# nka77/DAHiTra

Hardware: NVIDIA B200
Metric: image-pairs/sec (higher is better)
Workload: dtype x3 error-compensated f16 products (f16 main + scaled-remainder corrections; decoder: 3xTF32), fp32 accumulate

## Files before the change

### dahitra_b200/_lib.py

```python
from __future__ import annotations

import ctypes as C
import os
import subprocess
import threading

_HERE = os.path.dirname(os.path.abspath(__file__))
_CSRC = os.path.join(_HERE, "csrc")
LIB_PATH = os.path.join(_HERE, "libdahitra_b200.so")
SOURCES = ["conv_ffma.cu", "conv_tc.cu", "conv_tc2.cu", "conv_tc3.cu", "split.cu", "tokens.cu", "decoder.cu", "decoder_tc.cu", "stem_tc.cu", "classifier.cu", "train_decoder.cu", "train_tokens.cu", "prepare.cu", "aux.cu", "forward.cu"]
NVCC_FLAGS = ["-gencode", "arch=compute_100a,code=sm_100a", "-O3", "-lineinfo", "-std=c++17",
              "-Xcompiler", "-fPIC", "-shared"]

_lock = threading.Lock()
_lib = None


def _sources():
    return [os.path.join(_CSRC, s) for s in SOURCES if os.path.exists(os.path.join(_CSRC, s))]


STAMP_PATH = LIB_PATH + ".stamp"


def _deps():
    deps = _sources() + [os.path.join(_HERE, "..", "include", "dahitra_b200.h")]
    deps += [os.path.join(_CSRC, f) for f in sorted(os.listdir(_CSRC)) if f.endswith(".cuh")]
    return [d for d in deps if os.path.exists(d)]


def _source_hash() -> str:
    import hashlib
    h = hashlib.sha256(" ".join(NVCC_FLAGS + [os.environ.get("DAHITRA_DEBUG_BUILD", "0")]).encode())
    for d in _deps():
        h.update(os.path.basename(d).encode() + b"\0")
        with open(d, "rb") as f:
            h.update(f.read())
    return h.hexdigest()


def needs_build() -> bool:
    if not os.path.exists(LIB_PATH):
        return True
    if os.path.exists(STAMP_PATH):
        with open(STAMP_PATH) as f:
            return f.read().strip() != _source_hash()
    t = os.path.getmtime(LIB_PATH)
    if any(os.path.getmtime(d) > t for d in _deps()):
        return True
    _write_stamp()
    return False


def _write_stamp():
    try:
        with open(STAMP_PATH + ".tmp", "w") as f:
            f.write(_source_hash() + "\n")
        os.replace(STAMP_PATH + ".tmp", STAMP_PATH)
    except OSError:
        pass


def build(force: bool = False, verbose: bool = False) -> str:
    if not force and not needs_build():
        return LIB_PATH
    import tempfile
    from concurrent.futures import ThreadPoolExecutor
    nvcc = os.environ.get("NVCC", "nvcc")
    cflags = [f for f in NVCC_FLAGS if f != "-shared"]
    if os.environ.get("DAHITRA_DEBUG_BUILD") == "1":
        cflags.append("-DDH_MBAR_TIMEOUT")
    with tempfile.TemporaryDirectory(prefix="_build_", dir=_HERE) as tmp:
        def compile_one(src):
            obj = os.path.join(tmp, os.path.basename(src) + ".o")
            cmd = [nvcc] + cflags + ["-c", src, "-o", obj]
            if verbose:
                print(" ".join(cmd), flush=True)
            r = subprocess.run(cmd, capture_output=True, text=True)
            if r.returncode != 0:
                raise RuntimeError("nvcc failed on %s:\n%s%s" % (src, r.stdout, r.stderr))
            return obj
        with ThreadPoolExecutor(max_workers=min(8, os.cpu_count() or 1)) as ex:
            objs = list(ex.map(compile_one, _sources()))
        cmd = [nvcc] + NVCC_FLAGS + objs + ["-o", LIB_PATH + ".tmp"]
        if verbose:
            print(" ".join(cmd), flush=True)
        r = subprocess.run(cmd, capture_output=True, text=True)
        if r.returncode != 0:
            raise RuntimeError("nvcc link failed:\n" + r.stdout + r.stderr)
    os.replace(LIB_PATH + ".tmp", LIB_PATH)
    _write_stamp()
    return LIB_PATH


EXAMPLE_SRC = os.path.join(_HERE, "..", "examples", "dahitra_infer.c")
EXAMPLE_BIN = os.path.join(_HERE, "..", "examples", "bin", "dahitra_infer")


def build_example(force: bool = False, verbose: bool = False) -> str:
    src, out = os.path.abspath(EXAMPLE_SRC), os.path.abspath(EXAMPLE_BIN)
    deps = [src, LIB_PATH, os.path.join(_HERE, "..", "include", "dahitra_b200.h")]
    if not force and os.path.exists(out) and all(os.path.getmtime(d) <= os.path.getmtime(out) for d in deps):
        return out
    cuda = os.environ.get("CUDA_HOME", "/usr/local/cuda")
    os.makedirs(os.path.dirname(out), exist_ok=True)
    cmd = [os.environ.get("CC", "gcc"), "-std=c99", "-O2", "-Wall", "-Wextra", "-Werror", "-I", os.path.join(_HERE, "..", "include"),
           "-I", os.path.join(cuda, "include"), src, "-L", _HERE, "-ldahitra_b200", "-L", os.path.join(cuda, "lib64"),
           "-l:libcudart_static.a", "-ldl", "-lpthread", "-lrt", "-Wl,-rpath,$ORIGIN/../../dahitra_b200", "-o", out + ".tmp"]
    if verbose:
        print(" ".join(cmd), flush=True)
    r = subprocess.run(cmd, capture_output=True, text=True)
    if r.returncode != 0:
        raise RuntimeError("building examples/dahitra_infer.c failed:\n" + r.stdout + r.stderr)
    os.replace(out + ".tmp", out)
    return out


_P, _I, _LL, _SZ = C.c_void_p, C.c_int, C.c_longlong, C.c_size_t
SIGNATURES = {
    "dahitra_version": (_I, []),
    "dahitra_error_string": (C.c_char_p, [_I]),
    "dahitra_weight_slot_name": (C.c_char_p, [_I]),
    "dahitra_workspace_bytes": (_SZ, [_I, _I, _I, _I, _I, _I]),
    "dahitra_prepare_weights": (_LL, [_P, _I, _I, _I, _P, _LL, _P]),
    "dahitra_forward": (_I, [_P, _I, _P, _P, _LL, _P, _P, _P, _SZ, _I, _I, _I, _I, _I, _I, _P]),
    "dahitra_forward_profiled": (_I, [_P, _I, _P, _P, _LL, _P, _P, _P, _SZ, _I, _I, _I, _I, _I, _I, _P,
                                      _I, _P, _P, _P, _P]),
    "dahitra_conv2d": (_I, [_P, _P, _I, _I, _I, _I, _I, _I, _I, _I, _I, _I, _I, _P, _P, _P, _P, _I, _P, _I, _P]),
    "dahitra_conv2d_up2_tc": (_I, [_P, _I, _I, _I, _P, _P, _I, _P, _I, _P]),
    "dahitra_stem": (_I, [_P, _LL, _I, _I, _I, _P, _P, _P, _P]),
    "dahitra_stem_tc": (_I, [_P, _LL, _I, _I, _I, _P, _P, _P, _I, _P]),
    "dahitra_maxpool3x3s2": (_I, [_P, _I, _I, _I, _I, _P, _P]),
    "dahitra_squeeze_tokens": (_I, [_P, _I, _I, _I, _P, _P, _P, _P, _P]),
    "dahitra_token_encoder": (_I, [_P, _I, _I, _P, _I, _I, _P, _P]),
    "dahitra_decoder_tables": (_I, [_P, _I, _I, _I, _P, _I, _I, _P, _P]),
    "dahitra_pixel_decoder": (_I, [_P, _P, _P, _P, _I, _I, _I, _I, _I, _P, _I, _P, _P]),
    "dahitra_decoder_tables_tc": (_I, [_P, _I, _I, _I, _P, _I, _I, _P, _P]),
    "dahitra_pixel_decoder_tc": (_I, [_P, _P, _P, _P, _I, _I, _I, _I, _I, _P, _I, _I, _P, _P]),
    "dahitra_confusion_matrix": (_I, [_P, _P, _LL, _I, _P, _P]),
    "dahitra_prepare_input_u8": (_I, [_P, _I, _I, _I, _I, _I, _P, _P]),
    "dahitra_classifier": (_I, [_P, _I, _I, _I, _I, _P, _P, _P, _P, _P]),
    "dahitra_split_pack": (_I, [_P, _LL, _P, _P]),
    "dahitra_split_unpack": (_I, [_P, _LL, _P, _P]),
    "dahitra_maxpool3x3s2_split": (_I, [_P, _I, _I, _I, _I, _P, _P]),
    "dahitra_pixel_decoder_train_blocks": (_I, [_I]),
    "dahitra_pixel_decoder_train_fwd": (_I, [_P, _P, _P, _P, _I, _I, _I, _I, _I, _P]),
    "dahitra_pixel_decoder_train_bwd": (_I, [_P, _P, _P, _P, _P, _I, _I, _I, _I, _I, _P]),
    "dahitra_tokenizer_train_chunks": (_I, [_I]),
    "dahitra_tokenizer_train_fwd": (_I, [_P, _P, _P, _P, _P, _I, _I, _I, _P]),
    "dahitra_tokenizer_train_bwd": (_I, [_P, _P, _P, _P, _P, _P, _P, _I, _I, _I, _P]),
    "dahitra_pixel_decoder_train_fwd_ex": (_I, [_P, _P, _P, _P, _I, _I, _I, _I, _I, _I, _P]),
    "dahitra_pixel_decoder_train_bwd_ex": (_I, [_P, _P, _P, _P, _P, _I, _I, _I, _I, _I, _I, _P]),
    "dahitra_tokenizer_train_fwd_ex": (_I, [_P, _P, _P, _P, _P, _I, _I, _I, _I, _P]),
    "dahitra_tokenizer_train_bwd_ex": (_I, [_P, _P, _P, _P, _P, _P, _P, _I, _I, _I, _I, _P]),
    "dahitra_conv2d_split": (_I, [_P, _P, _I, _I, _LL, _LL, _I, _I, _I, _I, _I, _I, _P, _P, _P, _I, _I, _P, _I, _I, _P, _P, _P]),
    "dahitra_maxpool3x3s2_h16": (_I, [_P, _I, _I, _I, _I, _P, _P]),
    "dahitra_classifier_h16": (_I, [_P, _I, _I, _I, _I, _P, _P, _P, _P, _P]),
}


class DhTensor(C.Structure):
    _fields_ = [("name", C.c_char_p), ("data", C.c_void_p), ("dtype", C.c_int), ("ndim", C.c_int), ("shape", C.c_longlong * 4)]


def load():
    global _lib
    with _lock:
        if _lib is None:
            if not os.path.exists(LIB_PATH):
                raise RuntimeError(
                    f"dahitra_b200: {LIB_PATH} is missing — run `python -c 'import __graft_entry__ as g; g.build()'` "
                    "(nvcc, sm_100a). There is no fallback path.")
            lib = C.CDLL(LIB_PATH)
            for name, (res, args) in SIGNATURES.items():
                fn = getattr(lib, name)
                fn.restype, fn.argtypes = res, args
            _lib = lib
        return _lib


def check(rc: int, what: str = "dahitra"):
    if rc != 0:
        msg = load().dahitra_error_string(rc)
        raise RuntimeError(f"{what} failed with code {rc}: {msg.decode() if msg else '?'}")
```

### dahitra_b200/csrc/common.cuh

```cuda
#pragma once
#include <cuda_runtime.h>
#include <stdint.h>
#include <stddef.h>
#include "../../include/dahitra_b200.h"

#ifndef __CUDA_ARCH_LIST__
#endif

#define DH_CHECK_LAUNCH()                                   \
  do {                                                      \
    cudaError_t e__ = cudaGetLastError();                   \
    if (e__ != cudaSuccess) return (int)e__;                \
  } while (0)

#define DH_REQUIRE(cond, code) \
  do {                         \
    if (!(cond)) return (code);\
  } while (0)

static inline bool dh_aligned16(const void* p) { return (reinterpret_cast<uintptr_t>(p) & 15u) == 0; }
static inline int dh_cdiv(int a, int b) { return (a + b - 1) / b; }

__device__ __forceinline__ float4 ldg4(const float* p) { return __ldg(reinterpret_cast<const float4*>(p)); }
__device__ __forceinline__ void st4(float* p, float4 v) { *reinterpret_cast<float4*>(p) = v; }

__device__ __forceinline__ float warp_sum(float v) {
#pragma unroll
  for (int o = 16; o > 0; o >>= 1) v += __shfl_xor_sync(0xffffffffu, v, o);
  return v;
}
__device__ __forceinline__ float warp_max(float v) {
#pragma unroll
  for (int o = 16; o > 0; o >>= 1) v = fmaxf(v, __shfl_xor_sync(0xffffffffu, v, o));
  return v;
}

__device__ __forceinline__ float gelu_erf(float x) { return 0.5f * x * (1.0f + erff(x * 0.70710678118654752440f)); }

struct ConvArgs {
  const float* in0; const float* in1; int C0, C1;
  int N, inH, inW, up;
  int KH, KW, stride, pad, Cout;
  const float* w;
  const float* wt;
  const float* bias; const float* res; int relu;
  float* out;
  int ps = 0;
  int flat = 0;
};
struct Conv3Args {
  const void* in0; const void* in1; int C0, C1;
  int N, inH, inW;
  long long in0_plane = 0, in1_plane = 0;
  long long res_plane = 0, out_plane = 0;
  int K, stride, Cout;
  const void* wt16;
  long long wt_plane_bytes;
  const float* bias; const void* res; int res_split;
  int relu;
  void* out; int out_split;
  int ps = 0;
  int tok = 0;
  const float* wtok = nullptr; float* partials = nullptr;
  int force_stream = 0;
  int cg = 0;
  int h16 = 0;
};
bool dh_conv_tc3_eligible(const Conv3Args& a);
int dh_launch_conv_tc3(const Conv3Args& a, cudaStream_t s);
int dh_conv_tc3_tok_chunks(int H, int W);
int dh_launch_split_pack(const float* in, size_t n, void* out, cudaStream_t s);
int dh_launch_split_unpack(const void* in, size_t n, float* out, cudaStream_t s);
int dh_launch_maxpool_split(const void* in, int N, int H, int W, int C, void* out, cudaStream_t s);
int dh_launch_maxpool_h16(const void* in, int N, int H, int W, int C, void* out, cudaStream_t s);
int dh_pdl_attr(cudaLaunchAttribute* at);
void dh_set_pdl(int on);
template <typename... KArgs, typename... Args>
static inline int dh_launch(void (*kern)(KArgs...), dim3 grid, dim3 block, size_t smem, cudaStream_t s, Args... args) {
  cudaLaunchConfig_t cfg = {};
  cfg.gridDim = grid; cfg.blockDim = block; cfg.dynamicSmemBytes = smem; cfg.stream = s;
  cudaLaunchAttribute at[1];
  cfg.attrs = at; cfg.numAttrs = dh_pdl_attr(at);
  const cudaError_t e = cudaLaunchKernelEx(&cfg, kern, KArgs(args)...);
  if (e != cudaSuccess) return (int)e;
  DH_CHECK_LAUNCH();
  return 0;
}
#ifdef __CUDACC__
__device__ __forceinline__ void dh_pdl_wait() { asm volatile("griddepcontrol.wait;" ::: "memory"); }
__device__ __forceinline__ void dh_pdl_launch_dependents() { asm volatile("griddepcontrol.launch_dependents;" ::: "memory"); }
#endif
int dh_launch_conv_ffma(const ConvArgs& a, cudaStream_t s);
bool dh_conv_tc_eligible(const ConvArgs& a);
int dh_launch_conv_tc(const ConvArgs& a, cudaStream_t s);
bool dh_conv_tc2_eligible(const ConvArgs& a);
int dh_launch_conv_tc2(const ConvArgs& a, int xm, int cg, cudaStream_t s);
int dh_launch_stem(const float* x, long long xbs, int N, int H, int W, const float* w, const float* b, float* out, cudaStream_t s);
int dh_launch_stem_tc(const float* x, long long xbs, int N, int H, int W, const float* wtc, const float* b, float* out, int x3,
                      cudaStream_t s, long long split_plane_pitch = 0, const float* x_second = nullptr);
int dh_launch_maxpool(const float* in, int N, int H, int W, int C, float* out, cudaStream_t s);
int dh_launch_classifier(const float* in, int N, int H, int W, int nc, const float* w, const float* b,
                         float* logits, unsigned char* amax, cudaStream_t s);
int dh_launch_classifier_tma(const float* in, int N, int H, int W, int nc, const float* w, const float* b,
                             float* logits, unsigned char* amax, cudaStream_t s);
int dh_launch_classifier_h16(const void* in, int N, int H, int W, int nc, const float* w, const float* b,
                             float* logits, unsigned char* amax, cudaStream_t s);
int dh_launch_squeeze_tokens(const float* feat, int N, int npix, int Cin, const float* wsq, const float* wtok,
                             float* xs, float* partials, cudaStream_t s);
int dh_launch_token_encoder(const float* partials, int B, int nchunk, const float* enc, int heads, int add_pos,
                            float* mem, cudaStream_t s);
int dh_launch_decoder_tables(const float* mem, int B, int first_call, int ncalls, const float* dec, int heads, int depth,
                             float* tables, cudaStream_t s);
int dh_launch_decoder_tables_tc(const float* mem, int B, int first_call, int ncalls, const float* dec, int heads, int depth,
                                float* tables, cudaStream_t s);
int dh_launch_pixel_decoder_tc(const float* x, const float* pos, const float* tables, const float* pack, int nimg, int h,
                               int w, int heads, int depth, const float* skip, int skip_up, int x3, float* out,
                               cudaStream_t s);
int dh_launch_pixel_decoder(const float* x, const float* pos, const float* tables, const float* dec,
                            int nimg, int h, int w, int heads, int depth, const float* skip, int skip_up, float* out,
                            cudaStream_t s);
```

### dahitra_b200/csrc/conv_tc3.cu

```cuda
#include "tc_common.cuh"
#include <cstdlib>
#include <mutex>
#include <unordered_map>

using namespace dhtc;

namespace {

constexpr int T3_TH = 16, T3_TW = 8;
constexpr int T3_HW = T3_TW + 2, T3_HH = T3_TH + 2;
constexpr uint32_t T3_PLANE = 11776;
constexpr uint32_t T3_HALO = 2 * T3_PLANE;
constexpr int T3_MAX_HB = 4;
enum { EPI_F32 = 0, EPI_SPLIT = 1, EPI_TOK = 2 };

struct T3Args {
  const float* bias;
  const void* res; void* out;
  const float* wtok; float* partials;
  long long res_plane, out_plane;
  int OH, OW, Cout, relu, tilesX, tilesY, cchunks0, cchunks, Cin, ps, N, ncout_tiles, ntiles;
  int res_split, out_split, tiles_per_img;
  int hb;
  uint32_t halo_plane_bytes;
};

template <int NT, bool RES, int CG = 1, bool P1 = false> struct T3Cfg {
  static constexpr int TPS = NT == 128 ? 1 : 3;
  static constexpr int STAGES = RES ? 1 : (NT == 128 ? 6 : (NT == 64 ? 4 : 8)) * CG;
  static constexpr uint32_t HALO = P1 ? T3_PLANE : T3_HALO;
  static constexpr uint32_t B_TAP = (P1 ? 1u : 2u) * NT * 64u / CG;
  static constexpr uint32_t B_STAGE = B_TAP * TPS;
  static constexpr uint32_t RING_BYTES = RES ? 0u : STAGES * B_STAGE;
  static constexpr int THREADS = 352;
  static constexpr uint32_t IDESC_WIDE = umma_idesc_f16(128, 2 * NT);
  static constexpr uint32_t IDESC_NARROW = umma_idesc_f16(128 * CG, NT);
  static constexpr int ACC_COLS = P1 ? NT : 2 * NT;
  static constexpr uint32_t TMEM_COLS = 2 * ACC_COLS < 32 ? 32 : 2 * ACC_COLS;
};

template <int KS, int SD> struct Tap3 {
  static constexpr int NPH = (KS == 3 && SD == 2) ? 4 : 1;
  static constexpr int NTAPS = KS * KS;
  __host__ __device__ static constexpr int tap(int i) {
    return (KS == 3 && SD == 2) ? (int)((0x862071534ULL >> (4 * i)) & 0xF) : i;
  }
  __host__ __device__ static constexpr int first(int ph) {
    return (KS == 3 && SD == 2) ? (int)((0x95310u >> (4 * ph)) & 0xF) : (ph == 0 ? 0 : NTAPS);
  }
  __host__ __device__ static constexpr int shift_px(int t, int halo_w) {
    return KS == 1 ? 0 : (SD == 2 ? ((t / 3 != 0) ? halo_w : 0) + ((t % 3 != 0) ? 1 : 0) : (t / 3) * halo_w + t % 3);
  }
};

struct Tile3 { int n, oy0, ox0, ct; };
__device__ __forceinline__ Tile3 tile3(int tile, const T3Args& e, int CG = 1, int rank = 0) {
  Tile3 t;
  t.ct = tile % e.ncout_tiles; tile /= e.ncout_tiles;
  if (CG == 2) tile = 2 * tile + rank;
  const int tx = tile % e.tilesX; tile /= e.tilesX;
  const int ty = tile % e.tilesY;
  t.n = tile / e.tilesY; t.oy0 = ty * T3_TH; t.ox0 = tx * T3_TW;
  return t;
}

__device__ __forceinline__ void tma_load_3d_2sm(uint32_t dst, const CUtensorMap* tm, uint32_t cluster_bar, int c0, int c1, int c2) {
  asm volatile(
      "cp.async.bulk.tensor.3d.cta_group::2.shared::cluster.global.tile.mbarrier::complete_tx::bytes [%0], [%1, {%3, %4, %5}], [%2];"
      ::"r"(dst), "l"(tm), "r"(cluster_bar), "r"(c0), "r"(c1), "r"(c2) : "memory");
}
__device__ __forceinline__ void tma_load_3d(uint32_t dst, const CUtensorMap* tm, uint32_t bar, int c0, int c1, int c2) {
  asm volatile(
      "cp.async.bulk.tensor.3d.shared::cluster.global.tile.mbarrier::complete_tx::bytes [%0], [%1, {%3, %4, %5}], [%2];"
      ::"r"(dst), "l"(tm), "r"(bar), "r"(c0), "r"(c1), "r"(c2) : "memory");
}
__device__ __forceinline__ void split8(const float4& a, const float4& b, uint4& hi, uint4& lo) {
  hi.x = pack_f16x2_sat(a.x, a.y); hi.y = pack_f16x2_sat(a.z, a.w); hi.z = pack_f16x2_sat(b.x, b.y); hi.w = pack_f16x2_sat(b.z, b.w);
  lo.x = pack_f16x2_sat((a.x - f16_lo(hi.x)) * 2048.f, (a.y - f16_hi(hi.x)) * 2048.f);
  lo.y = pack_f16x2_sat((a.z - f16_lo(hi.y)) * 2048.f, (a.w - f16_hi(hi.y)) * 2048.f);
  lo.z = pack_f16x2_sat((b.x - f16_lo(hi.z)) * 2048.f, (b.y - f16_hi(hi.z)) * 2048.f);
  lo.w = pack_f16x2_sat((b.z - f16_lo(hi.w)) * 2048.f, (b.w - f16_hi(hi.w)) * 2048.f);
}
__device__ __forceinline__ void join8(const uint4& hi, const uint4& lo, float4& a, float4& b) {
  constexpr float S = 1.0f / 2048.0f;
  a = make_float4(fmaf(f16_lo(lo.x), S, f16_lo(hi.x)), fmaf(f16_hi(lo.x), S, f16_hi(hi.x)),
                  fmaf(f16_lo(lo.y), S, f16_lo(hi.y)), fmaf(f16_hi(lo.y), S, f16_hi(hi.y)));
  b = make_float4(fmaf(f16_lo(lo.z), S, f16_lo(hi.z)), fmaf(f16_hi(lo.z), S, f16_hi(hi.z)),
                  fmaf(f16_lo(lo.w), S, f16_lo(hi.w)), fmaf(f16_hi(lo.w), S, f16_hi(hi.w)));
}
__device__ __forceinline__ void half8(const uint4& h, float4& a, float4& b) {
  a = make_float4(f16_lo(h.x), f16_hi(h.x), f16_lo(h.y), f16_hi(h.y));
  b = make_float4(f16_lo(h.z), f16_hi(h.z), f16_lo(h.w), f16_hi(h.w));
}
__device__ __forceinline__ uint4 ldg16(const void* p) { return __ldg(reinterpret_cast<const uint4*>(p)); }
__device__ __forceinline__ float4 as_f4(const uint4& u) { return make_float4(__uint_as_float(u.x), __uint_as_float(u.y), __uint_as_float(u.z), __uint_as_float(u.w)); }

template <int NT, int KS, int SD, int EPI, bool RES, int CG, bool P1>
__global__ void __launch_bounds__(T3Cfg<NT, RES, CG, P1>::THREADS, 1)
conv_tc3_kernel(const __grid_constant__ CUtensorMap tmA0h, const __grid_constant__ CUtensorMap tmA0l,
                const __grid_constant__ CUtensorMap tmA1h, const __grid_constant__ CUtensorMap tmA1l,
                const __grid_constant__ CUtensorMap tmB, const T3Args e) {
  using Cfg = T3Cfg<NT, RES, CG, P1>;
  constexpr int STAGES = Cfg::STAGES;
  extern __shared__ uint8_t t3_raw[];
  __shared__ __align__(8) uint64_t halo_full[T3_MAX_HB], halo_empty[T3_MAX_HB], b_full[STAGES], b_empty[STAGES], acc_full[2], acc_empty[2];
  __shared__ uint32_t tmem_slot;

  const int warp = threadIdx.x >> 5, lane = threadIdx.x & 31;
  const uint32_t base = (smem_u32(t3_raw) + 1023u) & ~1023u;
  uint8_t* base_ptr = t3_raw + (base - smem_u32(t3_raw));
  const int HB = e.hb;
  const uint32_t b_ring = base + (uint32_t)HB * Cfg::HALO;
  const int rank = CG == 2 ? (int)cluster_ctarank() : 0;
  const int w0 = CG == 2 ? (int)(blockIdx.x >> 1) : (int)blockIdx.x;
  const int wstep = CG == 2 ? (int)(gridDim.x >> 1) : (int)gridDim.x;
  constexpr int pad = (KS == 3) ? 1 : 0;
  using Sched = Tap3<KS, SD>;
  constexpr int NPH = Sched::NPH;
  constexpr int NTAPS = KS * KS;
  constexpr int TPS = (SD == 1 && NTAPS % Cfg::TPS == 0) ? Cfg::TPS : 1;
  constexpr int HALO_W = (KS == 3) ? T3_HW : T3_TW;
  const uint32_t w_bytes = RES ? (uint32_t)(e.ncout_tiles * e.cchunks * NTAPS) * Cfg::B_TAP : Cfg::RING_BYTES;
  const uint32_t epi_off = (uint32_t)HB * Cfg::HALO + w_bytes;

  if (threadIdx.x == 0) {
    for (int i = 0; i < T3_MAX_HB; ++i) { mbar_init(smem_u32(&halo_full[i]), 1); mbar_init(smem_u32(&halo_empty[i]), 1); }
    for (int i = 0; i < 2; ++i) { mbar_init(smem_u32(&acc_full[i]), 1); mbar_init(smem_u32(&acc_empty[i]), 128 * CG); }
    for (int s = 0; s < STAGES; ++s) { mbar_init(smem_u32(&b_full[s]), 1); mbar_init(smem_u32(&b_empty[s]), 1); }
    mbar_fence_init();
    asm volatile("prefetch.tensormap [%0];" ::"l"(&tmA0h) : "memory");
    asm volatile("prefetch.tensormap [%0];" ::"l"(&tmA0l) : "memory");
    asm volatile("prefetch.tensormap [%0];" ::"l"(&tmB) : "memory");
  }
  if (warp == 1) {
    if (CG == 2) tmem_alloc_2sm(smem_u32(&tmem_slot), Cfg::TMEM_COLS);
    else         tmem_alloc(smem_u32(&tmem_slot), Cfg::TMEM_COLS);
  }
  if (EPI == EPI_TOK && threadIdx.x >= 64 && threadIdx.x < 96)
    reinterpret_cast<float4*>(base_ptr + epi_off + 8 * 4096)[threadIdx.x - 64] = __ldg(reinterpret_cast<const float4*>(e.wtok) + (threadIdx.x - 64));
  tc_fence_before();
  __syncthreads();
  if (CG == 2) cluster_sync_all();
  tc_fence_after();
  const uint32_t tmem_base = tmem_slot;
  if (RES && warp == 6 && lane == 0) {
    const uint32_t bar = smem_u32(&b_full[0]);
    if (rank == 0) mbar_expect_tx(bar, (uint32_t)CG * w_bytes);
    const uint32_t lbar = (CG == 2 && rank == 1) ? mapa_u32(bar, 0) : bar;
    uint32_t dst = b_ring;
    for (int ct = 0; ct < e.ncout_tiles; ++ct)
      for (int cc = 0; cc < e.cchunks; ++cc)
#pragma unroll
        for (int i = 0; i < NTAPS; ++i, dst += Cfg::B_TAP) {
          if (CG == 2) tma_load_3d_2sm(dst, &tmB, lbar, Sched::tap(i) * e.Cin + cc * 32, ct * NT + rank * (NT / 2), 0);
          else         tma_load_3d(dst, &tmB, bar, Sched::tap(i) * e.Cin + cc * 32, ct * NT, 0);
        }
  }
  pdl_wait();
  pdl_launch_dependents();

  if (warp == 0) {
    if (lane == 0) {
      int hb = 0;
      uint32_t ephase = 1;
      for (int tile = w0; tile < e.ntiles; tile += wstep) {
        const Tile3 t = tile3(tile, e, CG, rank);
        for (int cc = 0; cc < e.cchunks; ++cc) {
#pragma unroll
          for (int ph = 0; ph < NPH; ++ph) {
            mbar_wait(smem_u32(&halo_empty[hb]), ephase);
            const uint32_t bar = smem_u32(&halo_full[hb]);
            if (rank == 0) mbar_expect_tx(bar, (uint32_t)CG * (P1 ? 1u : 2u) * e.halo_plane_bytes);
            const uint32_t dst = base + (uint32_t)hb * Cfg::HALO;
            const int cx = SD == 1 ? t.ox0 - pad : 2 * (t.ox0 - pad) + (ph & 1);
            const int cy = SD == 1 ? t.oy0 - pad : 2 * (t.oy0 - pad) + (ph >> 1);
            const bool first = cc < e.cchunks0;
            const int c0 = (first ? cc : cc - e.cchunks0) * 32;
            if (CG == 2 && rank == 1) {
              const uint32_t lbar = mapa_u32(bar, 0);
              tma_load_4d_2sm(dst, first ? &tmA0h : &tmA1h, lbar, c0, cx, cy, t.n);
              tma_load_4d_2sm(dst + T3_PLANE, first ? &tmA0l : &tmA1l, lbar, c0, cx, cy, t.n);
            } else {
              tma_load_4d(dst, first ? &tmA0h : &tmA1h, bar, c0, cx, cy, t.n);
              if (!P1) tma_load_4d(dst + T3_PLANE, first ? &tmA0l : &tmA1l, bar, c0, cx, cy, t.n);
            }
            if (++hb == HB) { hb = 0; ephase ^= 1u; }
          }
        }
      }
    }
  } else if (warp == 6) {
    if (!RES && lane == 0) {
      int step = 0;
      for (int tile = w0; tile < e.ntiles; tile += wstep) {
        const Tile3 t = tile3(tile, e, CG, rank);
        for (int cc = 0; cc < e.cchunks; ++cc) {
#pragma unroll
          for (int i0 = 0; i0 < NTAPS; i0 += TPS, ++step) {
            const int st = step % STAGES, round = step / STAGES;
            mbar_wait(smem_u32(&b_empty[st]), (uint32_t)((round & 1) ^ 1));
            const uint32_t bar = smem_u32(&b_full[st]);
            if (rank == 0) mbar_expect_tx(bar, (uint32_t)(CG * TPS) * Cfg::B_TAP);
            const uint32_t lbar = (CG == 2 && rank == 1) ? mapa_u32(bar, 0) : bar;
#pragma unroll
            for (int tt = 0; tt < TPS; ++tt) {
              const uint32_t dst = b_ring + (uint32_t)st * Cfg::B_STAGE + (uint32_t)tt * Cfg::B_TAP;
              const int kcol = Sched::tap(i0 + tt) * e.Cin + cc * 32;
              if (CG == 2) tma_load_3d_2sm(dst, &tmB, lbar, kcol, t.ct * NT + rank * (NT / 2), 0);
              else         tma_load_3d(dst, &tmB, bar, kcol, t.ct * NT, 0);
            }
          }
        }
      }
    }
  } else if (warp == 1) {
    if (lane == 0 && rank == 0) {
      constexpr uint32_t SBO = (uint32_t)HALO_W * 64u;
      int hb = 0, st = 0, it = 0;
      uint32_t hphase = 0, bphase = 0;
      if (RES) { mbar_wait(smem_u32(&b_full[0]), 0); tc_fence_after(); }
      for (int tile = w0; tile < e.ntiles; tile += wstep, ++it) {
        const int ab = it & 1;
        if (CG == 2) mbar_wait_cluster(smem_u32(&acc_empty[ab]), (uint32_t)(((it >> 1) & 1) ^ 1));
        else         mbar_wait(smem_u32(&acc_empty[ab]), (uint32_t)(((it >> 1) & 1) ^ 1));
        tc_fence_after();
        const uint32_t d_main = tmem_base + (uint32_t)ab * Cfg::ACC_COLS, d_corr = d_main + NT;
        const uint32_t w_tile = RES ? b_ring + (uint32_t)((tile % e.ncout_tiles) * e.cchunks * NTAPS) * Cfg::B_TAP : 0u;
        for (int cc = 0; cc < e.cchunks; ++cc) {
#pragma unroll
          for (int ph = 0; ph < NPH; ++ph) {
            mbar_wait(smem_u32(&halo_full[hb]), hphase);
            tc_fence_after();
            const uint32_t h_hi = base + (uint32_t)hb * Cfg::HALO, h_lo = h_hi + T3_PLANE;
#pragma unroll
            for (int i0 = Sched::first(ph); i0 < Sched::first(ph + 1); i0 += TPS) {
              uint32_t b_stage;
              if (RES) {
                b_stage = w_tile + (uint32_t)(cc * NTAPS + i0) * Cfg::B_TAP;
              } else {
                mbar_wait(smem_u32(&b_full[st]), bphase);
                tc_fence_after();
                b_stage = b_ring + (uint32_t)st * Cfg::B_STAGE;
              }
#pragma unroll
              for (int tt = 0; tt < TPS; ++tt) {
                const int i = i0 + tt;
                const uint32_t px = (uint32_t)Sched::shift_px(Sched::tap(i), HALO_W) * 64u;
                const uint64_t a_h = umma_desc_sw64(h_hi + px, SBO), a_l = umma_desc_sw64(h_lo + px, SBO);
                const uint64_t b_w = umma_desc_sw64(b_stage + (uint32_t)tt * Cfg::B_TAP, 512u);
                if (CG == 2) {
                  const uint64_t b_l = umma_desc_sw64(b_stage + (uint32_t)tt * Cfg::B_TAP + (NT / 2) * 64u, 512u);
#pragma unroll
                  for (int k = 0; k < 2; ++k) umma_bf16_2sm(d_main, a_h + (uint64_t)(2 * k), b_w + (uint64_t)(2 * k), Cfg::IDESC_NARROW, (cc | i | k) ? 1u : 0u);
#pragma unroll
                  for (int k = 0; k < 2; ++k) umma_bf16_2sm(d_corr, a_h + (uint64_t)(2 * k), b_l + (uint64_t)(2 * k), Cfg::IDESC_NARROW, (cc | i | k) ? 1u : 0u);
#pragma unroll
                  for (int k = 0; k < 2; ++k) umma_bf16_2sm(d_corr, a_l + (uint64_t)(2 * k), b_w + (uint64_t)(2 * k), Cfg::IDESC_NARROW, 1u);
                } else if (P1) {
#pragma unroll
                  for (int k = 0; k < 2; ++k) umma_bf16(d_main, a_h + (uint64_t)(2 * k), b_w + (uint64_t)(2 * k), Cfg::IDESC_NARROW, (cc | i | k) ? 1u : 0u);
                } else {
#pragma unroll
                  for (int k = 0; k < 2; ++k) umma_bf16(d_main, a_h + (uint64_t)(2 * k), b_w + (uint64_t)(2 * k), Cfg::IDESC_WIDE, (cc | i | k) ? 1u : 0u);
#pragma unroll
                  for (int k = 0; k < 2; ++k) umma_bf16(d_corr, a_l + (uint64_t)(2 * k), b_w + (uint64_t)(2 * k), Cfg::IDESC_NARROW, 1u);
                }
              }
              if (!RES) {
                if (CG == 2) umma_commit_2sm(smem_u32(&b_empty[st])); else umma_commit(smem_u32(&b_empty[st]));
                if (++st == STAGES) { st = 0; bphase ^= 1u; }
              }
            }
            if (CG == 2) umma_commit_2sm(smem_u32(&halo_empty[hb])); else umma_commit(smem_u32(&halo_empty[hb]));
            if (++hb == HB) { hb = 0; hphase ^= 1u; }
          }
        }
        if (CG == 2) umma_commit_2sm(smem_u32(&acc_full[ab])); else umma_commit(smem_u32(&acc_full[ab]));
      }
    }
  } else {
    const int q = warp & 3, grp = warp >= 7 ? 1 : 0;
    float* stage = reinterpret_cast<float*>(base_ptr + epi_off + (size_t)(grp * 4 + q) * 4096);
    const float* wtok_s = reinterpret_cast<const float*>(base_ptr + epi_off + 8 * 4096);
    float* tokred = reinterpret_cast<float*>(base_ptr + epi_off + 8 * 4096 + 512 + grp * 2176);
    const int c4 = lane & 3, r4 = lane >> 2;
    constexpr int NSLAB = NT / 32;
    const char* resb = reinterpret_cast<const char*>(e.res);
    int it = 0;
    for (int tile = w0; tile < e.ntiles; tile += wstep, ++it) {
      if ((it & 1) != grp) continue;
      const Tile3 t = tile3(tile, e, CG, rank);
      const int n0 = t.ct * NT;
      size_t rowoff[4];
      bool ok[4];
#pragma unroll
      for (int g = 0; g < 4; ++g) {
        const int mm = q * 32 + g * 8 + r4;
        const int oy = t.oy0 + mm / T3_TW, ox = t.ox0 + mm % T3_TW;
        ok[g] = (oy < e.OH) && (ox < e.OW) && (t.n < e.N);
        rowoff[g] = e.ps ? ((size_t)(t.n * 2 * e.OH + 2 * oy) * (2 * e.OW) + 2 * ox) * 32 + c4 * 8
                         : ((size_t)(t.n * e.OH + oy) * e.OW + ox) * e.Cout + n0 + c4 * 8;
      }
      uint4 ra[4], rb[4];
      auto load_res = [&](int j) {
#pragma unroll
        for (int g = 0; g < 4; ++g) {
          ra[g] = make_uint4(0u, 0u, 0u, 0u); rb[g] = ra[g];
          if (ok[g]) {
            const size_t o = rowoff[g] + (size_t)j * 32;
            if (e.res_split) { ra[g] = ldg16(resb + o * 2); if (!P1) rb[g] = ldg16(resb + (o + (size_t)e.res_plane) * 2); }
            else             { ra[g] = ldg16(resb + o * 4); rb[g] = ldg16(resb + o * 4 + 16); }
          }
        }
      };
      if (e.res) load_res(0);
      const int ab = it & 1;
      mbar_wait(smem_u32(&acc_full[ab]), (uint32_t)((it >> 1) & 1));
      tc_fence_after();
#pragma unroll 1
      for (int j = 0; j < NSLAB; ++j) {
        float4 bia0 = make_float4(0.f, 0.f, 0.f, 0.f), bia1 = bia0;
        if (e.bias) { bia0 = ldg4(e.bias + n0 + j * 32 + c4 * 8); bia1 = ldg4(e.bias + n0 + j * 32 + c4 * 8 + 4); }
        uint32_t v[32], u[32];
        tmem_ld32(tmem_base + ((uint32_t)(q * 32) << 16) + (uint32_t)(ab * Cfg::ACC_COLS + j * 32), v);
        if (!P1) tmem_ld32(tmem_base + ((uint32_t)(q * 32) << 16) + (uint32_t)(ab * Cfg::ACC_COLS + NT + j * 32), u);
        if (j == NSLAB - 1) {
          tc_fence_before();
          if (CG == 2) mbar_arrive_cluster(mapa_u32(smem_u32(&acc_empty[ab]), 0));
          else         mbar_arrive_local(smem_u32(&acc_empty[ab]));
        }
        float tl[4] = {0.f, 0.f, 0.f, 0.f};
#pragma unroll
        for (int c = 0; c < 32; ++c) {
          float x = P1 ? __uint_as_float(v[c]) : fmaf(__uint_as_float(u[c]), 1.0f / 2048.0f, __uint_as_float(v[c]));
          if (EPI == EPI_TOK) {
            x = fmaxf(x, 0.f);
            const float4 wt = *reinterpret_cast<const float4*>(wtok_s + c * 4);
            tl[0] = fmaf(x, wt.x, tl[0]); tl[1] = fmaf(x, wt.y, tl[1]); tl[2] = fmaf(x, wt.z, tl[2]); tl[3] = fmaf(x, wt.w, tl[3]);
          }
          v[c] = __float_as_uint(x);
        }
#pragma unroll
        for (int k4 = 0; k4 < 8; ++k4)
          *reinterpret_cast<float4*>(stage + lane * 32 + ((k4 ^ (lane & 7)) << 2)) =
              make_float4(__uint_as_float(v[k4 * 4]), __uint_as_float(v[k4 * 4 + 1]), __uint_as_float(v[k4 * 4 + 2]), __uint_as_float(v[k4 * 4 + 3]));
        __syncwarp();
#pragma unroll
        for (int g = 0; g < 4; ++g) {
          const int r = g * 8 + r4;
          float4 o0 = *reinterpret_cast<const float4*>(stage + r * 32 + (((2 * c4) ^ (r & 7)) << 2));
          float4 o1 = *reinterpret_cast<const float4*>(stage + r * 32 + (((2 * c4 + 1) ^ (r & 7)) << 2));
          o0.x += bia0.x; o0.y += bia0.y; o0.z += bia0.z; o0.w += bia0.w;
          o1.x += bia1.x; o1.y += bia1.y; o1.z += bia1.z; o1.w += bia1.w;
          if (e.res) {
            float4 x0, x1;
            if (e.res_split) { if (P1) half8(ra[g], x0, x1); else join8(ra[g], rb[g], x0, x1); }
            else { x0 = as_f4(ra[g]); x1 = as_f4(rb[g]); }
            o0.x += x0.x; o0.y += x0.y; o0.z += x0.z; o0.w += x0.w;
            o1.x += x1.x; o1.y += x1.y; o1.z += x1.z; o1.w += x1.w;
          }
          if (e.relu) {
            o0.x = fmaxf(o0.x, 0.f); o0.y = fmaxf(o0.y, 0.f); o0.z = fmaxf(o0.z, 0.f); o0.w = fmaxf(o0.w, 0.f);
            o1.x = fmaxf(o1.x, 0.f); o1.y = fmaxf(o1.y, 0.f); o1.z = fmaxf(o1.z, 0.f); o1.w = fmaxf(o1.w, 0.f);
          }
          if (ok[g]) {
            if (P1 && e.out_split) {
              uint16_t* o16 = reinterpret_cast<uint16_t*>(e.out);
              const size_t off = rowoff[g] + (e.ps ? ((size_t)(j >> 1) * (2 * e.OW) + (j & 1)) * 32 : (size_t)j * 32);
              *reinterpret_cast<uint4*>(o16 + off) = make_uint4(pack_f16x2_sat(o0.x, o0.y), pack_f16x2_sat(o0.z, o0.w),
                                                                pack_f16x2_sat(o1.x, o1.y), pack_f16x2_sat(o1.z, o1.w));
            } else if (!P1 && (EPI == EPI_SPLIT || (EPI == EPI_TOK && e.out_split))) {
              uint4 h, l;
              split8(o0, o1, h, l);
              uint16_t* o16 = reinterpret_cast<uint16_t*>(e.out);
              const size_t off = rowoff[g] + (size_t)j * 32;
              *reinterpret_cast<uint4*>(o16 + off) = h;
              *reinterpret_cast<uint4*>(o16 + off + (size_t)e.out_plane) = l;
            } else {
              float* ob = reinterpret_cast<float*>(e.out);
              float* op = e.ps ? ob + rowoff[g] + ((size_t)(j >> 1) * (2 * e.OW) + (j & 1)) * 32 : ob + rowoff[g] + (size_t)j * 32;
              st4(op, o0); st4(op + 4, o1);
            }
          }
        }
        if (e.res && j + 1 < NSLAB) load_res(j + 1);
        if (EPI == EPI_TOK) {
          const int mm = q * 32 + lane;
          const bool valid = (t.oy0 + mm / T3_TW < e.OH) && (t.ox0 + mm % T3_TW < e.OW) && (t.n < e.N);
          float ew[4];
#pragma unroll
          for (int l = 0; l < 4; ++l) {
            const float a = valid ? tl[l] : -INFINITY;
            const float mx = warp_max(a);
            ew[l] = valid ? expf(a - mx) : 0.f;
            const float sw = warp_sum(ew[l]);
            if (lane == 0) { tokred[(q * 4 + l) * 34] = mx; tokred[(q * 4 + l) * 34 + 1] = sw; }
          }
          float ts[4] = {0.f, 0.f, 0.f, 0.f};
#pragma unroll 8
          for (int r = 0; r < 32; ++r) {
            const float xv = stage[r * 32 + ((((lane >> 2) ^ (r & 7)) << 2) | (lane & 3))];
#pragma unroll
            for (int l = 0; l < 4; ++l) ts[l] = fmaf(__shfl_sync(0xffffffffu, ew[l], r), xv, ts[l]);
          }
#pragma unroll
          for (int l = 0; l < 4; ++l) tokred[(q * 4 + l) * 34 + 2 + lane] = ts[l];
          asm volatile("bar.sync %0, 128;" ::"r"(1 + grp) : "memory");
          {
            const int l = q;
            float m4[4], M = -INFINITY;
#pragma unroll
            for (int w4 = 0; w4 < 4; ++w4) { m4[w4] = tokred[(w4 * 4 + l) * 34]; M = fmaxf(M, m4[w4]); }
            float S = 0.f, T = 0.f;
#pragma unroll
            for (int w4 = 0; w4 < 4; ++w4) {
              const float sc = (m4[w4] == -INFINITY) ? 0.f : expf(m4[w4] - M);
              S = fmaf(tokred[(w4 * 4 + l) * 34 + 1], sc, S);
              T = fmaf(tokred[(w4 * 4 + l) * 34 + 2 + lane], sc, T);
            }
            const int mtile = CG == 2 ? 2 * (tile / e.ncout_tiles) + rank : tile / e.ncout_tiles;
            float* pp = e.partials + (((size_t)t.n * e.tiles_per_img + mtile % e.tiles_per_img) * 4 + l) * 34;
            if (t.n < e.N) {
              if (lane == 0) { pp[0] = M; pp[1] = S; }
              pp[2 + lane] = T;
            }
          }
          asm volatile("bar.sync %0, 128;" ::"r"(1 + grp) : "memory");
        }
        __syncwarp();
      }
    }
  }
  tc_fence_before();
  __syncthreads();
  if (CG == 2) cluster_sync_all();
  if (warp == 1) {
    tc_fence_after();
    if (CG == 2) tmem_dealloc_2sm(tmem_base, Cfg::TMEM_COLS);
    else         tmem_dealloc(tmem_base, Cfg::TMEM_COLS);
  }
}

typedef CUresult (*EncodeTiledFn3)(CUtensorMap*, CUtensorMapDataType, cuuint32_t, void*, const cuuint64_t*, const cuuint64_t*,
                                   const cuuint32_t*, const cuuint32_t*, CUtensorMapInterleave, CUtensorMapSwizzle,
                                   CUtensorMapL2promotion, CUtensorMapFloatOOBfill);
EncodeTiledFn3 get_encode3() {
  static EncodeTiledFn3 fn = nullptr;
  static std::once_flag once;
  std::call_once(once, [] {
    void* p = nullptr;
    cudaDriverEntryPointQueryResult q;
    if (cudaGetDriverEntryPoint("cuTensorMapEncodeTiled", &p, cudaEnableDefault, &q) == cudaSuccess && q == cudaDriverEntryPointSuccess)
      fn = (EncodeTiledFn3)p;
  });
  return fn;
}
struct Key3 {
  const void* ptr; long long d[5];
  bool operator==(const Key3& o) const { return ptr == o.ptr && d[0] == o.d[0] && d[1] == o.d[1] && d[2] == o.d[2] && d[3] == o.d[3] && d[4] == o.d[4]; }
};
struct Key3Hash {
  size_t operator()(const Key3& k) const {
    size_t h = (size_t)k.ptr;
    for (long long v : k.d) h = h * 1000003u ^ (size_t)v;
    return h;
  }
};
std::mutex g_mu3;
std::unordered_map<Key3, CUtensorMap, Key3Hash> g_maps3;

int act_map(CUtensorMap* out, const void* ptr, int C, int W, int H, int N, int bw, int bh, int es) {
  Key3 key{ptr, {C, W, H, ((long long)N << 8) | es, ((long long)bw << 16) | bh}};
  {
    std::lock_guard<std::mutex> lk(g_mu3);
    auto it = g_maps3.find(key);
    if (it != g_maps3.end()) { *out = it->second; return 0; }
  }
  EncodeTiledFn3 enc = get_encode3();
  if (!enc) return DH_E_VARIANT;
  cuuint64_t dims[4] = {(cuuint64_t)C, (cuuint64_t)W, (cuuint64_t)H, (cuuint64_t)N};
  cuuint64_t strides[3] = {(cuuint64_t)C * 2, (cuuint64_t)C * W * 2, (cuuint64_t)C * W * H * 2};
  cuuint32_t box[4] = {32, (cuuint32_t)(bw * es), (cuuint32_t)(bh * es), 1};
  cuuint32_t estr[4] = {1, (cuuint32_t)es, (cuuint32_t)es, 1};
  CUtensorMap m;
  const CUresult r = enc(&m, CU_TENSOR_MAP_DATA_TYPE_FLOAT16, 4, const_cast<void*>(ptr), dims, strides, box, estr,
                         CU_TENSOR_MAP_INTERLEAVE_NONE, CU_TENSOR_MAP_SWIZZLE_64B, CU_TENSOR_MAP_L2_PROMOTION_L2_256B,
                         CU_TENSOR_MAP_FLOAT_OOB_FILL_NONE);
  if (r != CUDA_SUCCESS) return DH_E_SHAPE;
  {
    std::lock_guard<std::mutex> lk(g_mu3);
    if (g_maps3.size() > 4096) g_maps3.clear();
    g_maps3[key] = m;
  }
  *out = m;
  return 0;
}
int filt_map(CUtensorMap* out, const void* ptr, int K, int Cout, long long plane_bytes, int NT, int planes) {
  Key3 key{ptr, {K, Cout, plane_bytes, NT, -1 - planes}};
  {
    std::lock_guard<std::mutex> lk(g_mu3);
    auto it = g_maps3.find(key);
    if (it != g_maps3.end()) { *out = it->second; return 0; }
  }
  EncodeTiledFn3 enc = get_encode3();
  if (!enc) return DH_E_VARIANT;
  cuuint64_t dims[3] = {(cuuint64_t)K, (cuuint64_t)Cout, (cuuint64_t)planes};
  cuuint64_t strides[2] = {(cuuint64_t)K * 2, (cuuint64_t)plane_bytes};
  cuuint32_t box[3] = {32, (cuuint32_t)NT, (cuuint32_t)planes};
  cuuint32_t estr[3] = {1, 1, 1};
  CUtensorMap m;
  const CUresult r = enc(&m, CU_TENSOR_MAP_DATA_TYPE_FLOAT16, 3, const_cast<void*>(ptr), dims, strides, box, estr,
                         CU_TENSOR_MAP_INTERLEAVE_NONE, CU_TENSOR_MAP_SWIZZLE_64B, CU_TENSOR_MAP_L2_PROMOTION_L2_256B,
                         CU_TENSOR_MAP_FLOAT_OOB_FILL_NONE);
  if (r != CUDA_SUCCESS) return DH_E_SHAPE;
  {
    std::lock_guard<std::mutex> lk(g_mu3);
    g_maps3[key] = m;
  }
  *out = m;
  return 0;
}

constexpr uint32_t T3_SMEM_MAX = 232448 - 1024;

template <int NT, int KS, int SD, int EPI, bool RES, int CG, bool P1>
int launch3k(const CUtensorMap* A, const CUtensorMap& Bm, const T3Args& e, uint32_t smem, dim3 grid, cudaStream_t s) {
  using Cfg = T3Cfg<NT, RES, CG, P1>;
  auto kern = conv_tc3_kernel<NT, KS, SD, EPI, RES, CG, P1>;
  cudaError_t err = cudaFuncSetAttribute(kern, cudaFuncAttributeMaxDynamicSharedMemorySize, (int)T3_SMEM_MAX);
  if (err != cudaSuccess) return (int)err;
  cudaLaunchConfig_t cfg = {};
  cfg.gridDim = grid; cfg.blockDim = dim3(Cfg::THREADS, 1, 1); cfg.dynamicSmemBytes = smem; cfg.stream = s;
  cudaLaunchAttribute at[2];
  int na = dh_pdl_attr(at);
  if (CG == 2) {
    at[na].id = cudaLaunchAttributeClusterDimension;
    at[na].val.clusterDim.x = 2; at[na].val.clusterDim.y = 1; at[na].val.clusterDim.z = 1;
    ++na;
  }
  cfg.attrs = at; cfg.numAttrs = na;
  err = cudaLaunchKernelEx(&cfg, kern, A[0], A[1], A[2], A[3], Bm, e);
  if (err != cudaSuccess) return (int)err;
  DH_CHECK_LAUNCH();
  return 0;
}
template <int NT, bool RES, int CG, bool P1>
int launch3(const CUtensorMap* A, const CUtensorMap& Bm, const T3Args& e, int ks, int stride, int epi, uint32_t smem, dim3 grid, cudaStream_t s) {
  if (epi == EPI_TOK) {
    if constexpr (NT == 32 && CG == 1) return launch3k<32, 1, 1, EPI_TOK, RES, 1, P1>(A, Bm, e, smem, grid, s);
    return DH_E_SHAPE;
  }
  if constexpr (P1) {
    if (stride == 2) return ks == 3 ? launch3k<NT, 3, 2, EPI_SPLIT, RES, CG, true>(A, Bm, e, smem, grid, s) : launch3k<NT, 1, 2, EPI_SPLIT, RES, CG, true>(A, Bm, e, smem, grid, s);
    return ks == 3 ? launch3k<NT, 3, 1, EPI_SPLIT, RES, CG, true>(A, Bm, e, smem, grid, s) : launch3k<NT, 1, 1, EPI_SPLIT, RES, CG, true>(A, Bm, e, smem, grid, s);
  } else {
    if (stride == 2) {
      if (epi == EPI_SPLIT) return ks == 3 ? launch3k<NT, 3, 2, EPI_SPLIT, RES, CG, false>(A, Bm, e, smem, grid, s) : launch3k<NT, 1, 2, EPI_SPLIT, RES, CG, false>(A, Bm, e, smem, grid, s);
      return ks == 3 ? launch3k<NT, 3, 2, EPI_F32, RES, CG, false>(A, Bm, e, smem, grid, s) : launch3k<NT, 1, 2, EPI_F32, RES, CG, false>(A, Bm, e, smem, grid, s);
    }
    if (epi == EPI_SPLIT) return ks == 3 ? launch3k<NT, 3, 1, EPI_SPLIT, RES, CG, false>(A, Bm, e, smem, grid, s) : launch3k<NT, 1, 1, EPI_SPLIT, RES, CG, false>(A, Bm, e, smem, grid, s);
    return ks == 3 ? launch3k<NT, 3, 1, EPI_F32, RES, CG, false>(A, Bm, e, smem, grid, s) : launch3k<NT, 1, 1, EPI_F32, RES, CG, false>(A, Bm, e, smem, grid, s);
  }
}
template <bool RES, int CG, bool P1>
int launch3n(int NT, const CUtensorMap* A, const CUtensorMap& Bm, const T3Args& e, int ks, int stride, int epi, uint32_t smem, dim3 grid, cudaStream_t s) {
  switch (NT) {
    case 128: return launch3<128, RES, CG, P1>(A, Bm, e, ks, stride, epi, smem, grid, s);
    case 64: return launch3<64, RES, CG, P1>(A, Bm, e, ks, stride, epi, smem, grid, s);
    default: return launch3<32, RES, CG, P1>(A, Bm, e, ks, stride, epi, smem, grid, s);
  }
}
template <bool RES>
int launch3c(int cg, bool p1, int NT, const CUtensorMap* A, const CUtensorMap& Bm, const T3Args& e, int ks, int stride, int epi, uint32_t smem,
             dim3 grid, cudaStream_t s) {
  if (p1) return launch3n<RES, 1, true>(NT, A, Bm, e, ks, stride, epi, smem, grid, s);
  return cg == 2 ? launch3n<RES, 2, false>(NT, A, Bm, e, ks, stride, epi, smem, grid, s)
                 : launch3n<RES, 1, false>(NT, A, Bm, e, ks, stride, epi, smem, grid, s);
}
}

bool dh_conv_tc3_eligible(const Conv3Args& a) {
  const bool base = a.in0 && a.wt16 && a.out && (a.stride == 1 || (a.stride == 2 && a.inH % 2 == 0 && a.inW % 2 == 0 && !a.ps)) &&
                    (a.K == 1 || a.K == 3) && a.C0 > 0 && a.C0 % 32 == 0 && a.C1 % 32 == 0 && (a.C1 == 0 || a.in1) &&
                    (a.Cout == 32 || a.Cout == 64 || a.Cout == 128 || a.Cout == 256) && a.inH >= 1 && a.inW >= 1 && a.N >= 1;
  if (!base) return false;
  if (a.ps) return a.Cout == 128 && a.res == nullptr && (!a.out_split || a.h16) && a.K == 3;
  if (a.tok) return a.Cout == 32 && a.K == 1 && a.stride == 1 && a.wtok && a.partials && !a.res && !a.bias;
  return true;
}

int dh_conv_tc3_tok_chunks(int H, int W) { return dh_cdiv(H, T3_TH) * dh_cdiv(W, T3_TW); }

int dh_launch_conv_tc3(const Conv3Args& a, cudaStream_t s) {
  DH_REQUIRE(dh_conv_tc3_eligible(a), DH_E_SHAPE);
  DH_REQUIRE(dh_aligned16(a.in0) && dh_aligned16(a.in1) && dh_aligned16(a.wt16) && dh_aligned16(a.out) &&
             dh_aligned16(a.bias) && dh_aligned16(a.res) && dh_aligned16(a.wtok), DH_E_ALIGN);
  const int Cin = a.C0 + a.C1, K = a.K * a.K * Cin;
  int sms_ = 148, dev_ = 0;
  cudaGetDevice(&dev_);
  cudaDeviceGetAttribute(&sms_, cudaDevAttrMultiProcessorCount, dev_);
  int NT = a.Cout >= 128 ? 128 : a.Cout;
  if (NT == 128 && !a.ps) {
    const int mt = dh_cdiv(a.inW / a.stride, T3_TW) * dh_cdiv(a.inH / a.stride, T3_TH) * a.N;
    if (mt * (a.Cout / 128) < sms_) NT = 64;
  }
  const int hw = (a.K == 3) ? T3_HW : T3_TW, hh = (a.K == 3) ? T3_HH : T3_TH;
  CUtensorMap A[4], Bm;
  const size_t plane0 = a.in0_plane ? (size_t)a.in0_plane : (size_t)a.N * a.inH * a.inW * a.C0;
  const size_t plane1 = a.in1_plane ? (size_t)a.in1_plane : (size_t)a.N * a.inH * a.inW * a.C1;
  int rc = act_map(&A[0], a.in0, a.C0, a.inW, a.inH, a.N, hw, hh, a.stride);
  if (rc) return rc;
  A[1] = A[0];
  if (!a.h16) rc = act_map(&A[1], reinterpret_cast<const uint16_t*>(a.in0) + plane0, a.C0, a.inW, a.inH, a.N, hw, hh, a.stride);
  if (rc) return rc;
  if (a.C1) {
    rc = act_map(&A[2], a.in1, a.C1, a.inW, a.inH, a.N, hw, hh, a.stride);
    A[3] = A[2];
    if (!rc && !a.h16) rc = act_map(&A[3], reinterpret_cast<const uint16_t*>(a.in1) + plane1, a.C1, a.inW, a.inH, a.N, hw, hh, a.stride);
    if (rc) return rc;
  } else { A[2] = A[0]; A[3] = A[1]; }
  static const int env_cg = [] { const char* v = getenv("DAHITRA_TC3_CG"); return v ? atoi(v) : 0; }();
  static const bool env_stream = [] { const char* v = getenv("DAHITRA_TC3_STREAM"); return v && v[0] == '1'; }();
  const int mtiles = dh_cdiv(a.inW / a.stride, T3_TW) * dh_cdiv(a.inH / a.stride, T3_TH) * a.N;
  int cg = a.tok ? 1 : (a.cg ? a.cg : (env_cg == 2 ? 2 : (env_cg == 1 && (NT == 128 || (a.Cout == 32 && K >= 1152)) ? 2 : 1)));
  DH_REQUIRE(!(a.h16 && cg == 2), DH_E_VARIANT);
  if (mtiles < 2) cg = 1;
  rc = filt_map(&Bm, a.wt16, K, a.Cout, a.wt_plane_bytes, NT / cg, a.h16 ? 1 : 2);
  if (rc) return rc;
  T3Args e;
  e.bias = a.bias; e.res = a.res; e.out = a.out; e.wtok = a.wtok; e.partials = a.partials;
  e.OH = a.inH / a.stride; e.OW = a.inW / a.stride; e.Cout = a.Cout; e.relu = a.relu;
  e.tilesX = dh_cdiv(e.OW, T3_TW); e.tilesY = dh_cdiv(e.OH, T3_TH);
  e.cchunks0 = a.C0 / 32; e.cchunks = Cin / 32; e.Cin = Cin; e.ps = a.ps; e.N = a.N;
  e.ncout_tiles = a.Cout / NT;
  e.tiles_per_img = e.tilesX * e.tilesY;
  e.ntiles = (cg == 2 ? (mtiles + 1) / 2 : mtiles) * e.ncout_tiles;
  e.res_split = a.res_split; e.out_split = a.out_split;
  e.res_plane = a.res_plane ? a.res_plane : (long long)a.N * e.OH * e.OW * a.Cout;
  e.out_plane = a.out_plane ? a.out_plane : (long long)a.N * e.OH * e.OW * a.Cout;
  e.halo_plane_bytes = (uint32_t)(hw * hh * 64);
  const int epi = a.tok ? EPI_TOK : ((a.out_split || a.h16) ? EPI_SPLIT : EPI_F32);
  int dev = 0, sms = 148;
  cudaGetDevice(&dev);
  cudaDeviceGetAttribute(&sms, cudaDevAttrMultiProcessorCount, dev);
  const int slots = sms / cg;
  const int nwork = e.ntiles < slots ? e.ntiles : slots;
  dim3 grid((unsigned)(nwork * cg), 1, 1);
  const uint32_t w_bytes = (uint32_t)K * (uint32_t)a.Cout * (a.h16 ? 2u : 4u) / (uint32_t)cg;
  const uint32_t halo = a.h16 ? T3_PLANE : T3_HALO;
  const uint32_t fixed = 8 * 4096 + 1024 + (a.tok ? 512 + 2 * 2176 : 0);
  const bool res_ok = w_bytes + 2 * halo + fixed <= T3_SMEM_MAX && !a.force_stream && !env_stream && e.ntiles >= 2 * nwork;
  if (res_ok) {
    int hb = (int)((T3_SMEM_MAX - fixed - w_bytes) / halo);
    e.hb = hb > T3_MAX_HB ? T3_MAX_HB : hb;
    const uint32_t smem = (uint32_t)e.hb * halo + w_bytes + fixed;
    return launch3c<true>(cg, a.h16, NT, A, Bm, e, a.K, a.stride, epi, smem, grid, s);
  }
  e.hb = T3_MAX_HB;
  const uint32_t ring = a.h16 ? (NT == 128 ? T3Cfg<128, false, 1, true>::RING_BYTES : (NT == 64 ? T3Cfg<64, false, 1, true>::RING_BYTES : T3Cfg<32, false, 1, true>::RING_BYTES))
                              : (NT == 128 ? T3Cfg<128, false>::RING_BYTES : (NT == 64 ? T3Cfg<64, false>::RING_BYTES : T3Cfg<32, false>::RING_BYTES));
  const uint32_t smem = T3_MAX_HB * halo + ring + fixed;
  return launch3c<false>(cg, a.h16, NT, A, Bm, e, a.K, a.stride, epi, smem, grid, s);
}
```

### dahitra_b200/csrc/forward.cu

```cuda
#include "common.cuh"
#include <string.h>

namespace {

struct Level {
  int cin, heads, depth, h, w;
  size_t xs, xd, dx, out, part, mem, tab;
  int nchunk, nchunk3;
};

struct Plan {
  int B, H, W, nc, variant;
  size_t f2, p2, t4a, t4b, f4, t8a, t8b, t8c, f8, p8, t16a, t16b, t16c, f16;
  Level lv[3];
  size_t c4, c3, y20, o2, c2;
  size_t total_floats;
};

struct Bump {
  size_t off = 0;
  size_t take(size_t nfloats) {
    const size_t o = off;
    off += (nfloats + 63) & ~(size_t)63;
    return o;
  }
};

bool make_plan(Plan& p, int variant, int B, int H, int W, int nc, int flags) {
  if (B < 1 || H < 32 || W < 32 || (H % 32) || (W % 32) || nc < 1 || nc > 8) return false;
  if (variant != DH_VARIANT_LEVIR && variant != DH_VARIANT_XBD) return false;
  p.B = B; p.H = H; p.W = W; p.nc = nc; p.variant = variant;
  const size_t N2 = 2 * (size_t)B;
  const size_t s2 = (size_t)(H / 2) * (W / 2), s4 = s2 / 4, s8 = s4 / 4, s16 = s8 / 4;
  Bump b;
  p.f2 = b.take(N2 * s2 * 64);
  p.p2 = b.take(N2 * s4 * 64);
  p.t4a = b.take(N2 * s4 * 64); p.t4b = b.take(N2 * s4 * 64); p.f4 = b.take(N2 * s4 * 64);
  p.t8a = b.take(N2 * s8 * 128); p.t8b = b.take(N2 * s8 * 128); p.t8c = b.take(N2 * s8 * 128); p.f8 = b.take(N2 * s8 * 128);
  p.p8 = b.take(N2 * s16 * 128);
  p.t16a = b.take(N2 * s16 * 256); p.t16b = b.take(N2 * s16 * 256); p.t16c = b.take(N2 * s16 * 256); p.f16 = b.take(N2 * s16 * 256);
  const int cins[3] = {256, 128, 64}, heads[3] = {4, 4, 8}, depths[3] = {4, 4, 8}, div[3] = {16, 8, 4};
  for (int i = 0; i < 3; ++i) {
    Level& L = p.lv[i];
    L.cin = cins[i]; L.heads = heads[i]; L.depth = depths[i]; L.h = H / div[i]; L.w = W / div[i];
    const size_t n = (size_t)L.h * L.w;
    L.nchunk = (int)((n + 255) / 256);
    L.nchunk3 = dh_conv_tc3_tok_chunks(L.h, L.w);
    L.xs = b.take(N2 * n * 32);
    L.xd = b.take(N2 * n * 32);
    L.dx = b.take((size_t)B * n * 32);
    L.out = b.take((size_t)B * n * 32);
    L.part = b.take(N2 * (size_t)(L.nchunk3 > L.nchunk ? L.nchunk3 : L.nchunk) * 4 * 34);
    L.mem = b.take((size_t)B * 3 * 128);
    L.tab = b.take((size_t)3 * B * L.depth * (DH_TAB_FLOATS(L.heads) > DH_TABTC_FLOATS ? DH_TAB_FLOATS(L.heads) : DH_TABTC_FLOATS));
  }
  p.c4 = b.take((size_t)B * s4 * 32);
  const size_t n_c3 = (size_t)B * s2 * 32, n_y20 = (size_t)B * s2 * 128, n_c2 = (size_t)B * H * W * 32;
  const bool early_head = (flags & DH_FLAG_EARLY_HEAD) != 0;
  p.c3 = (p.t8c - p.t8a >= n_c3) ? p.t8a : b.take(n_c3);
  p.o2 = (p.p8 - p.t8c >= n_c3) ? p.t8c : b.take(n_c3);
  p.y20 = (!early_head && p.t8a - p.p2 >= n_y20) ? p.p2 : b.take(n_y20);
  p.c2 = (p.p2 - p.f2 >= n_c2) ? p.f2 : b.take(n_c2);
  p.total_floats = b.off;
  return true;
}

const char* kSlotNames[DH_W_COUNT] = {
  "DH_W_STEM_W", "DH_W_STEM_B",
  "DH_W_L1_0_C1_W", "DH_W_L1_0_C1_B", "DH_W_L1_0_C2_W", "DH_W_L1_0_C2_B",
  "DH_W_L1_1_C1_W", "DH_W_L1_1_C1_B", "DH_W_L1_1_C2_W", "DH_W_L1_1_C2_B",
  "DH_W_L2_0_C1_W", "DH_W_L2_0_C1_B", "DH_W_L2_0_C2_W", "DH_W_L2_0_C2_B", "DH_W_L2_0_DS_W", "DH_W_L2_0_DS_B",
  "DH_W_L2_1_C1_W", "DH_W_L2_1_C1_B", "DH_W_L2_1_C2_W", "DH_W_L2_1_C2_B",
  "DH_W_L3_0_C1_W", "DH_W_L3_0_C1_B", "DH_W_L3_0_C2_W", "DH_W_L3_0_C2_B", "DH_W_L3_0_DS_W", "DH_W_L3_0_DS_B",
  "DH_W_L3_1_C1_W", "DH_W_L3_1_C1_B", "DH_W_L3_1_C2_W", "DH_W_L3_1_C2_B",
  "DH_W_LV5_SQ", "DH_W_LV5_TOK", "DH_W_LV5_ENC", "DH_W_LV5_DEC", "DH_W_LV5_POS", "DH_W_LV5_DECODE",
  "DH_W_LV4_SQ", "DH_W_LV4_TOK", "DH_W_LV4_ENC", "DH_W_LV4_DEC", "DH_W_LV4_POS", "DH_W_LV4_DECODE",
  "DH_W_LV3_SQ", "DH_W_LV3_TOK", "DH_W_LV3_ENC", "DH_W_LV3_DEC", "DH_W_LV3_POS", "DH_W_LV3_DECODE",
  "DH_W_CL4_W", "DH_W_CL4_B", "DH_W_CL3_W", "DH_W_CL3_B", "DH_W_CL2_W", "DH_W_CL2_B",
  "DH_W_CL20A_W", "DH_W_CL20A_B", "DH_W_CL20B_W", "DH_W_CL20B_B", "DH_W_CLS_W", "DH_W_CLS_B",
  "DH_W_L1_0_C1_WT", "DH_W_L1_0_C2_WT", "DH_W_L1_1_C1_WT", "DH_W_L1_1_C2_WT",
  "DH_W_L2_0_C2_WT", "DH_W_L2_1_C1_WT", "DH_W_L2_1_C2_WT",
  "DH_W_L3_0_C1_WT", "DH_W_L3_0_C2_WT", "DH_W_L3_0_DS_WT", "DH_W_L3_1_C1_WT", "DH_W_L3_1_C2_WT",
  "DH_W_LV5_DECODE_WT", "DH_W_LV4_DECODE_WT", "DH_W_LV3_DECODE_WT", "DH_W_CL20A_WT", "DH_W_CL20B_WT",
  "DH_W_L2_0_C1_WT", "DH_W_L2_0_DS_WT",
  "DH_W_CL4_PSWT", "DH_W_CL4_PSB", "DH_W_CL3_PSWT", "DH_W_CL3_PSB", "DH_W_CL2_PSWT", "DH_W_CL2_PSB",
  "DH_W_LV5_DECTC", "DH_W_LV4_DECTC", "DH_W_LV3_DECTC", "DH_W_STEM_WTC",
  "DH_W_LV5_SQ_WT", "DH_W_LV4_SQ_WT", "DH_W_LV3_SQ_WT"};

int wt_slot_of(int wslot) {
  switch (wslot) {
    case DH_W_L1_0_C1_W: return DH_W_L1_0_C1_WT; case DH_W_L1_0_C2_W: return DH_W_L1_0_C2_WT;
    case DH_W_L1_1_C1_W: return DH_W_L1_1_C1_WT; case DH_W_L1_1_C2_W: return DH_W_L1_1_C2_WT;
    case DH_W_L2_0_C2_W: return DH_W_L2_0_C2_WT; case DH_W_L2_1_C1_W: return DH_W_L2_1_C1_WT;
    case DH_W_L2_1_C2_W: return DH_W_L2_1_C2_WT;
    case DH_W_L3_0_C1_W: return DH_W_L3_0_C1_WT; case DH_W_L3_0_C2_W: return DH_W_L3_0_C2_WT;
    case DH_W_L3_0_DS_W: return DH_W_L3_0_DS_WT; case DH_W_L3_1_C1_W: return DH_W_L3_1_C1_WT;
    case DH_W_L3_1_C2_W: return DH_W_L3_1_C2_WT;
    case DH_W_LV5_DECODE: return DH_W_LV5_DECODE_WT; case DH_W_LV4_DECODE: return DH_W_LV4_DECODE_WT;
    case DH_W_LV3_DECODE: return DH_W_LV3_DECODE_WT;
    case DH_W_CL20A_W: return DH_W_CL20A_WT; case DH_W_CL20B_W: return DH_W_CL20B_WT;
    case DH_W_L2_0_C1_W: return DH_W_L2_0_C1_WT; case DH_W_L2_0_DS_W: return DH_W_L2_0_DS_WT;
    default: return -1;
  }
}

}

extern "C" int dahitra_version(void) { return DAHITRA_ABI_VERSION; }

extern "C" const char* dahitra_error_string(int code) {
  switch (code) {
    case 0: return "ok";
    case DH_E_NULL: return "dahitra: required pointer is NULL";
    case DH_E_SHAPE: return "dahitra: unsupported shape";
    case DH_E_ALIGN: return "dahitra: pointer not 16-byte aligned";
    case DH_E_WORKSPACE: return "dahitra: workspace too small";
    case DH_E_VARIANT: return "dahitra: unknown variant or flags";
    case DH_E_WEIGHTS: return "dahitra: malformed weight table";
    default: return code > 0 ? cudaGetErrorString((cudaError_t)code) : "dahitra: unknown error";
  }
}

extern "C" const char* dahitra_weight_slot_name(int slot) {
  return (slot >= 0 && slot < DH_W_COUNT) ? kSlotNames[slot] : nullptr;
}

extern "C" size_t dahitra_workspace_bytes(int variant, int B, int H, int W, int output_nc, int flags) {
  Plan p;
  if (!make_plan(p, variant, B, H, W, output_nc, flags)) return 0;
  return p.total_floats * sizeof(float);
}

static int conv_dispatch(const ConvArgs& a, int flags, cudaStream_t s) {
  if (flags & DH_FLAG_CONV_TC) {
    const bool stride_ok = a.stride == 1 || (flags & DH_FLAG_TC_STRIDE2);
    if (stride_ok && !(flags & DH_FLAG_CONV_TC_V1) && dh_conv_tc2_eligible(a))
      return dh_launch_conv_tc2(a, (flags & DH_FLAG_TC_BF16) ? 3 : (flags & DH_FLAG_TC_3XTF32) ? ((flags & DH_FLAG_TC_MAIN_F16) ? ((flags & DH_FLAG_TC_FOLD) ? 6 : 4) : (flags & DH_FLAG_TC_X3_BF16) ? 2 : 1)
                                                            : ((flags & DH_FLAG_TC_MAIN_F16) ? 5 : 0),
                                (flags & DH_FLAG_CONV_TC_2CTA) ? 2 : 1, s);
    if (stride_ok && dh_conv_tc_eligible(a)) return dh_launch_conv_tc(a, s);
  }
  return dh_launch_conv_ffma(a, s);
}

extern "C" int dahitra_conv2d(const float* in0, const float* in1, int C0, int C1, int N, int inH, int inW, int up,
                              int KH, int KW, int stride, int pad, int Cout, const float* w, const float* wt,
                              const float* bias, const float* res, int relu, float* out, int flags, void* stream) {
  ConvArgs a{in0, in1, C0, C1, N, inH, inW, up, KH, KW, stride, pad, Cout, w, wt, bias, res, relu, out};
  return conv_dispatch(a, flags, (cudaStream_t)stream);
}
extern "C" int dahitra_conv2d_up2_tc(const float* in, int N, int inH, int inW, const float* pswt, const float* psb,
                                     int relu, float* out, int flags, void* stream) {
  ConvArgs a{in, nullptr, 32, 0, N, inH, inW, 1, 3, 3, 1, 1, 128, nullptr, pswt, psb, nullptr, relu, out};
  a.ps = 1;
  DH_REQUIRE(dh_conv_tc_eligible(a), DH_E_SHAPE);
  return conv_dispatch(a, flags | DH_FLAG_CONV_TC, (cudaStream_t)stream);
}
extern "C" int dahitra_stem(const float* x, long long xbs, int N, int H, int W, const float* w, const float* bias,
                            float* out, void* stream) {
  return dh_launch_stem(x, xbs, N, H, W, w, bias, out, (cudaStream_t)stream);
}
extern "C" int dahitra_stem_tc(const float* x, long long xbs, int N, int H, int W, const float* wtc, const float* bias,
                               float* out, int x3, void* stream) {
  return dh_launch_stem_tc(x, xbs, N, H, W, wtc, bias, out, x3, (cudaStream_t)stream);
}
extern "C" int dahitra_maxpool3x3s2(const float* in, int N, int H, int W, int C, float* out, void* stream) {
  return dh_launch_maxpool(in, N, H, W, C, out, (cudaStream_t)stream);
}
extern "C" int dahitra_squeeze_tokens(const float* feat, int N, int npix, int Cin, const float* w_sq, const float* w_tok,
                                      float* xs, float* partials, void* stream) {
  return dh_launch_squeeze_tokens(feat, N, npix, Cin, w_sq, w_tok, xs, partials, (cudaStream_t)stream);
}
extern "C" int dahitra_token_encoder(const float* partials, int B, int nchunk, const float* enc_pack, int heads,
                                     int add_pos, float* mem, void* stream) {
  return dh_launch_token_encoder(partials, B, nchunk, enc_pack, heads, add_pos, mem, (cudaStream_t)stream);
}
extern "C" int dahitra_decoder_tables(const float* mem, int B, int first_call, int ncalls, const float* dec_pack,
                                      int heads, int depth, float* tables, void* stream) {
  return dh_launch_decoder_tables(mem, B, first_call, ncalls, dec_pack, heads, depth, tables, (cudaStream_t)stream);
}
extern "C" int dahitra_pixel_decoder(const float* x, const float* pos, const float* tables, const float* dec_pack,
                                     int nimg, int h, int w, int heads, int depth, const float* skip, int skip_up,
                                     float* out, void* stream) {
  return dh_launch_pixel_decoder(x, pos, tables, dec_pack, nimg, h, w, heads, depth, skip, skip_up, out,
                                 (cudaStream_t)stream);
}
extern "C" int dahitra_decoder_tables_tc(const float* mem, int B, int first_call, int ncalls, const float* dec_pack,
                                         int heads, int depth, float* tables, void* stream) {
  return dh_launch_decoder_tables_tc(mem, B, first_call, ncalls, dec_pack, heads, depth, tables, (cudaStream_t)stream);
}
extern "C" int dahitra_pixel_decoder_tc(const float* x, const float* pos, const float* tables, const float* dectc_pack,
                                        int nimg, int h, int w, int heads, int depth, const float* skip, int skip_up,
                                        int x3, float* out, void* stream) {
  return dh_launch_pixel_decoder_tc(x, pos, tables, dectc_pack, nimg, h, w, heads, depth, skip, skip_up, x3, out,
                                    (cudaStream_t)stream);
}
extern "C" int dahitra_split_pack(const float* in, long long n, void* out, void* stream) {
  return dh_launch_split_pack(in, (size_t)n, out, (cudaStream_t)stream);
}
extern "C" int dahitra_split_unpack(const void* in, long long n, float* out, void* stream) {
  return dh_launch_split_unpack(in, (size_t)n, out, (cudaStream_t)stream);
}
extern "C" int dahitra_maxpool3x3s2_split(const void* in, int N, int H, int W, int C, void* out, void* stream) {
  return dh_launch_maxpool_split(in, N, H, W, C, out, (cudaStream_t)stream);
}
extern "C" int dahitra_conv2d_split(const void* in0, const void* in1, int C0, int C1, long long in0_plane, long long in1_plane,
                                    int N, int inH, int inW, int K, int stride, int Cout, const float* wt, const float* bias,
                                    const void* res, int res_split, int relu, void* out, int out_split, int mode,
                                    const float* w_tok, float* partials, void* stream) {
  DH_REQUIRE(wt, DH_E_NULL);
  const int h16 = (mode & 128) ? 1 : 0;
  const int sched = mode & ~(3 | 128);
  mode &= 3;
  DH_REQUIRE(mode <= 2 && !(sched & ~(16 | 32 | 64)), DH_E_VARIANT);
  Conv3Args a{};
  a.h16 = h16;
  a.cg = (sched & 32) ? 2 : ((sched & 16) ? 1 : 0);
  a.force_stream = (sched & 64) ? 1 : 0;
  a.in0 = in0; a.in1 = in1; a.C0 = C0; a.C1 = C1; a.N = N; a.inH = inH; a.inW = inW; a.in0_plane = in0_plane; a.in1_plane = in1_plane;
  a.K = K; a.stride = stride; a.Cout = Cout;
  const size_t plane = (size_t)Cout * K * K * (C0 + C1);
  a.wt16 = wt + 3 * plane; a.wt_plane_bytes = (long long)plane * 4;
  a.bias = bias; a.res = res; a.res_split = res_split; a.relu = relu; a.out = out; a.out_split = out_split;
  a.ps = mode == 1; a.tok = mode == 2; a.wtok = w_tok; a.partials = partials;
  return dh_launch_conv_tc3(a, (cudaStream_t)stream);
}
extern "C" int dahitra_classifier(const float* in, int N, int H, int W, int nc, const float* w, const float* bias,
                                  float* logits, unsigned char* argmax_u8, void* stream) {
  return dh_launch_classifier(in, N, H, W, nc, w, bias, logits, argmax_u8, (cudaStream_t)stream);
}
extern "C" int dahitra_maxpool3x3s2_h16(const void* in, int N, int H, int W, int C, void* out, void* stream) {
  return dh_launch_maxpool_h16(in, N, H, W, C, out, (cudaStream_t)stream);
}
extern "C" int dahitra_classifier_h16(const void* in, int N, int H, int W, int nc, const float* w, const float* bias,
                                      float* logits, unsigned char* argmax_u8, void* stream) {
  return dh_launch_classifier_h16(in, N, H, W, nc, w, bias, logits, argmax_u8, (cudaStream_t)stream);
}

namespace { thread_local int g_pdl = 0; }
void dh_set_pdl(int on) { g_pdl = on; }
int dh_pdl_attr(cudaLaunchAttribute* at) {
  if (!g_pdl) return 0;
  at[0].id = cudaLaunchAttributeProgrammaticStreamSerialization;
  at[0].val.programmaticStreamSerializationAllowed = 1;
  return 1;
}

namespace {
constexpr int PROF_MAX = 160;
struct ProfRec { const char* name; double flops, bytes; };
struct Profiler {
  bool on = false, created = false;
  int n = 0;
  cudaEvent_t ev[PROF_MAX + 1];
  ProfRec rec[PROF_MAX];
};
thread_local Profiler g_prof;

inline void prof_mark(cudaStream_t s, const char* name, double flops, double bytes) {
  if (!g_prof.on || g_prof.n >= PROF_MAX) return;
  g_prof.rec[g_prof.n] = {name, flops, bytes};
  ++g_prof.n;
  cudaEventRecord(g_prof.ev[g_prof.n], s);
}
}

namespace {
struct AuxStreams {
  bool ok = false;
  cudaStream_t st[2], low;
  cudaEvent_t fork, join[2], fork_low, join_low;
};
AuxStreams* aux_streams() {
  thread_local AuxStreams per_dev[16];
  int dev = 0;
  if (cudaGetDevice(&dev) != cudaSuccess || dev < 0 || dev >= 16) return nullptr;
  AuxStreams& a = per_dev[dev];
  if (!a.ok) {
    bool good = cudaEventCreateWithFlags(&a.fork, cudaEventDisableTiming) == cudaSuccess;
    for (int i = 0; i < 2 && good; ++i)
      good = cudaStreamCreateWithFlags(&a.st[i], cudaStreamNonBlocking) == cudaSuccess &&
             cudaEventCreateWithFlags(&a.join[i], cudaEventDisableTiming) == cudaSuccess;
    if (good) {
      int lo = 0, hi = 0;
      cudaDeviceGetStreamPriorityRange(&lo, &hi);
      good = cudaStreamCreateWithPriority(&a.low, cudaStreamNonBlocking, lo) == cudaSuccess &&
             cudaEventCreateWithFlags(&a.fork_low, cudaEventDisableTiming) == cudaSuccess &&
             cudaEventCreateWithFlags(&a.join_low, cudaEventDisableTiming) == cudaSuccess;
    }
    if (!good) { cudaGetLastError(); return nullptr; }
    a.ok = true;
  }
  return &a;
}
}

#define DH_STEP(name, fl, by, expr)        \
  do {                                     \
    const int rc__ = (expr);               \
    if (rc__ != 0) return rc__;            \
    prof_mark(s, name, (fl), (by));        \
  } while (0)

namespace {
int forward_split(const Plan& p, const void* const* weights, const float* x1, const float* x2, long long x_batch_stride,
                  float* logits, unsigned char* argmax_u8, float* ws, int variant, int B, int H, int W, int output_nc, int flags,
                  cudaStream_t s_main) {
  cudaStream_t s = s_main;
  auto Wt = [&](int slot) { return (const float*)weights[slot]; };
  const int N2 = 2 * B;
  const int h2 = H / 2, w2 = W / 2, h4 = H / 4, w4 = W / 4, h8 = H / 8, w8 = W / 8, h16 = H / 16, w16 = W / 16;
  const bool one = (flags & DH_FLAG_ACT_H16) != 0;
  const double eb = one ? 2.0 : 4.0;
  auto conv3 = [&](const char* name, const float* in0, const float* in1, int C0, int C1, long long in_plane, int N, int inH, int inW,
                   int K, int stride, int Cout, int wts, int bslot, const float* res, int res_split, int relu, float* out,
                   int out_split, int ps) -> int {
    Conv3Args a{};
    a.in0 = in0; a.in1 = in1; a.C0 = C0; a.C1 = C1; a.N = N; a.inH = inH; a.inW = inW; a.in0_plane = in_plane; a.in1_plane = in_plane;
    a.K = K; a.stride = stride; a.Cout = Cout;
    const size_t plane = (size_t)Cout * K * K * (C0 + C1);
    a.wt16 = Wt(wts) + 3 * plane; a.wt_plane_bytes = (long long)plane * 4;
    a.bias = bslot >= 0 ? Wt(bslot) : nullptr; a.res = res; a.res_split = one ? 1 : res_split; a.relu = relu; a.out = out;
    a.out_split = one ? 1 : out_split;
    a.ps = ps; a.h16 = one;
    const int rc = dh_launch_conv_tc3(a, s);
    if (rc != 0) return rc;
    const double OH = (double)inH / stride, OW = (double)inW / stride, Cin = C0 + C1;
    const double cout_alg = ps ? 32.0 : Cout, up = ps ? 2.0 : 1.0;
    const double fl = 2.0 * N * OH * up * OW * up * cout_alg * K * K * Cin;
    const double by = eb * ((double)N * inH * inW * Cin + (double)N * OH * up * OW * up * cout_alg * (res ? 2 : 1) + (double)K * K * Cin * cout_alg);
    prof_mark(s, name, fl, by);
    return 0;
  };
#define DH_CONV3(...)                     \
  do {                                    \
    const int rc__ = conv3(__VA_ARGS__);  \
    if (rc__ != 0) return rc__;           \
  } while (0)

  auto H16 = [](float* p) { return reinterpret_cast<uint16_t*>(p); };
  float* F2 = ws + p.f2;
  const size_t f2_half = (size_t)B * h2 * w2 * 64;
  const long long f2_plane = (long long)N2 * h2 * w2 * 64;
  float* F2post = reinterpret_cast<float*>(H16(F2) + f2_half);
  const double stem_fl = 2.0 * B * h2 * w2 * 64 * 147;
  const double stem_by = one ? B * (4.0 * 3 * H * W + 2.0 * h2 * w2 * 64) : 4.0 * B * ((double)3 * H * W + (double)h2 * w2 * 64);
  const int stem_mode = one ? 3 | 512 : ((flags & DH_FLAG_TC_3XTF32) ? 2 : 3) | 256;
  DH_STEP("stem", 2.0 * stem_fl, 2.0 * stem_by,
          dh_launch_stem_tc(x1, x_batch_stride, B, H, W, Wt(DH_W_STEM_WTC), Wt(DH_W_STEM_B), F2, stem_mode, s, f2_plane, x2));
  float* P2 = ws + p.p2;
  auto maxpool = [&](const float* in, int hh, int ww, int C, float* out) {
    return one ? dh_launch_maxpool_h16(in, N2, hh, ww, C, out, s) : dh_launch_maxpool_split(in, N2, hh, ww, C, out, s);
  };
  DH_STEP("maxpool_2", 0.0, eb * N2 * 64 * ((double)h2 * w2 + (double)h4 * w4), maxpool(F2, h2, w2, 64, P2));
  float *T4a = ws + p.t4a, *T4b = ws + p.t4b, *F4 = ws + p.f4;
  DH_CONV3("layer1.0.conv1", P2, nullptr, 64, 0, 0, N2, h4, w4, 3, 1, 64, DH_W_L1_0_C1_WT, DH_W_L1_0_C1_B, nullptr, 0, 1, T4a, 1, 0);
  DH_CONV3("layer1.0.conv2", T4a, nullptr, 64, 0, 0, N2, h4, w4, 3, 1, 64, DH_W_L1_0_C2_WT, DH_W_L1_0_C2_B, P2, 1, 1, T4b, 1, 0);
  DH_CONV3("layer1.1.conv1", T4b, nullptr, 64, 0, 0, N2, h4, w4, 3, 1, 64, DH_W_L1_1_C1_WT, DH_W_L1_1_C1_B, nullptr, 0, 1, T4a, 1, 0);
  DH_CONV3("layer1.1.conv2", T4a, nullptr, 64, 0, 0, N2, h4, w4, 3, 1, 64, DH_W_L1_1_C2_WT, DH_W_L1_1_C2_B, T4b, 1, 1, F4, 1, 0);
  float *T8a = ws + p.t8a, *T8b = ws + p.t8b, *T8c = ws + p.t8c, *F8 = ws + p.f8;
  DH_CONV3("layer2.0.conv1", F4, nullptr, 64, 0, 0, N2, h4, w4, 3, 2, 128, DH_W_L2_0_C1_WT, DH_W_L2_0_C1_B, nullptr, 0, 1, T8a, 1, 0);
  DH_CONV3("layer2.0.down", F4, nullptr, 64, 0, 0, N2, h4, w4, 1, 2, 128, DH_W_L2_0_DS_WT, DH_W_L2_0_DS_B, nullptr, 0, 0, T8b, 1, 0);
  DH_CONV3("layer2.0.conv2", T8a, nullptr, 128, 0, 0, N2, h8, w8, 3, 1, 128, DH_W_L2_0_C2_WT, DH_W_L2_0_C2_B, T8b, 1, 1, T8c, 1, 0);
  DH_CONV3("layer2.1.conv1", T8c, nullptr, 128, 0, 0, N2, h8, w8, 3, 1, 128, DH_W_L2_1_C1_WT, DH_W_L2_1_C1_B, nullptr, 0, 1, T8a, 1, 0);
  DH_CONV3("layer2.1.conv2", T8a, nullptr, 128, 0, 0, N2, h8, w8, 3, 1, 128, DH_W_L2_1_C2_WT, DH_W_L2_1_C2_B, T8c, 1, 1, F8, 1, 0);
  float* P8 = ws + p.p8;
  DH_STEP("maxpool_8", 0.0, eb * N2 * 128 * ((double)h8 * w8 + (double)h16 * w16), maxpool(F8, h8, w8, 128, P8));
  float *T16a = ws + p.t16a, *T16b = ws + p.t16b, *T16c = ws + p.t16c, *F16 = ws + p.f16;
  DH_CONV3("layer3.0.conv1", P8, nullptr, 128, 0, 0, N2, h16, w16, 3, 1, 256, DH_W_L3_0_C1_WT, DH_W_L3_0_C1_B, nullptr, 0, 1, T16a, 1, 0);
  DH_CONV3("layer3.0.down", P8, nullptr, 128, 0, 0, N2, h16, w16, 1, 1, 256, DH_W_L3_0_DS_WT, DH_W_L3_0_DS_B, nullptr, 0, 0, T16b, 1, 0);
  DH_CONV3("layer3.0.conv2", T16a, nullptr, 256, 0, 0, N2, h16, w16, 3, 1, 256, DH_W_L3_0_C2_WT, DH_W_L3_0_C2_B, T16b, 1, 1, T16c, 1, 0);
  DH_CONV3("layer3.1.conv1", T16c, nullptr, 256, 0, 0, N2, h16, w16, 3, 1, 256, DH_W_L3_1_C1_WT, DH_W_L3_1_C1_B, nullptr, 0, 1, T16a, 1, 0);
  DH_CONV3("layer3.1.conv2", T16a, nullptr, 256, 0, 0, N2, h16, w16, 3, 1, 256, DH_W_L3_1_C2_WT, DH_W_L3_1_C2_B, T16c, 1, 1, F16, 1, 0);

  float* feats[3] = {F16, F8, F4};
  const int base[3] = {DH_W_LV5_SQ, DH_W_LV4_SQ, DH_W_LV3_SQ};
  static const char* const nm[3][7] = {
      {"squeeze_tok_5", "token_enc_5", "dec_tables_5", "decoder_5_x12", "conv_decode_5", "decoder_5_diff", "conv_layer4"},
      {"squeeze_tok_4", "token_enc_4", "dec_tables_4", "decoder_4_x12", "conv_decode_4", "decoder_4_diff", "conv_layer4"},
      {"squeeze_tok_3", "token_enc_3", "dec_tables_3", "decoder_3_x12", "conv_decode_3", "decoder_3_diff", "conv_layer4"}};
  float* C4 = ws + p.c4;
  const int x3 = (flags & DH_FLAG_DEC_TC_X3) ? 1 : 0;
  auto dec_bytes_px = [&](const float* pos) { return one ? 32.0 * (2 + 2 + (pos ? 4 : 0)) : 4.0 * 32 * (pos ? 3 : 2); };
  auto level_pre = [&](int i) -> int {
    const Level& L = p.lv[i];
    const int npix = L.h * L.w;
    const float *wtok = Wt(base[i] + 1), *enc = Wt(base[i] + 2), *dec = Wt(base[i] + 3), *pos = Wt(base[i] + 4);
    float *XS = ws + L.xs, *XD = ws + L.xd, *DX = ws + L.dx, *PART = ws + L.part, *MEM = ws + L.mem, *TAB = ws + L.tab;
    const double inner = 64.0 * L.heads;
    const double dec_fl_px = L.depth * 2.0 * (32 * inner + 4 * inner + 4 * inner + inner * 32 + 2 * 32 * 32);
    const double dec_by_px = dec_bytes_px(pos);
    const bool levir = variant == DH_VARIANT_LEVIR;
    {
      Conv3Args a{};
      a.in0 = feats[i]; a.C0 = L.cin; a.N = N2; a.inH = L.h; a.inW = L.w; a.K = 1; a.stride = 1; a.Cout = 32;
      const size_t plane = (size_t)32 * L.cin;
      a.wt16 = Wt(DH_W_LV5_SQ_WT + i) + 3 * plane; a.wt_plane_bytes = (long long)plane * 4;
      a.out = XS; a.out_split = (levir && !one) ? 0 : 1; a.tok = 1; a.wtok = wtok; a.partials = PART; a.h16 = one;
      DH_STEP(nm[i][0], 2.0 * N2 * npix * 32 * (L.cin + 4 + 4), eb * N2 * npix * (L.cin + 32.0), dh_launch_conv_tc3(a, s));
    }
    const int add_tok_pos = levir ? 1 : (i == 0 ? 1 : 0);
    DH_STEP(nm[i][1], 0.0, 4.0 * N2 * L.nchunk3 * 136.0, dh_launch_token_encoder(PART, B, L.nchunk3, enc, L.heads, add_tok_pos, MEM, s));
    const size_t half = (size_t)B * npix * 32;
    const long long plane2 = (long long)N2 * npix * 32;
    const float* dectc = Wt(DH_W_LV5_DECTC + i);
    if (levir) {
      DH_STEP(nm[i][2], 0.0, 4.0 * 3 * B * L.depth * (double)DH_TABTC_FLOATS, dh_launch_decoder_tables_tc(MEM, B, 0, 3, dec, L.heads, L.depth, TAB, s));
      DH_STEP(nm[i][3], dec_fl_px * N2 * npix, dec_by_px * N2 * npix,
              dh_launch_pixel_decoder_tc(XS, pos, TAB, dectc, N2, L.h, L.w, L.heads, L.depth, nullptr, 1, x3 | (one ? 512 : 256), XD, s));
      DH_CONV3(nm[i][4], XD, reinterpret_cast<float*>(H16(XD) + half), 32, 32, plane2, B, L.h, L.w, 3, 1, 32, DH_W_LV5_DECODE_WT + i, -1,
               nullptr, 0, 0, DX, 0, 0);
    } else {
      DH_STEP(nm[i][2], 0.0, 4.0 * B * L.depth * (double)DH_TABTC_FLOATS, dh_launch_decoder_tables_tc(MEM, B, 2, 1, dec, L.heads, L.depth, TAB, s));
      DH_CONV3(nm[i][4], XS, reinterpret_cast<float*>(H16(XS) + half), 32, 32, plane2, B, L.h, L.w, 3, 1, 32, DH_W_LV5_DECODE_WT + i, -1,
               nullptr, 0, 0, DX, 0, 0);
    }
    return 0;
  };
  auto level_post = [&](int i) -> int {
    const Level& L = p.lv[i];
    const int npix = L.h * L.w;
    const float* pos = Wt(base[i] + 4);
    float *DX = ws + L.dx, *OUT = ws + L.out, *TAB = ws + L.tab;
    const float* skip = (i == 0) ? nullptr : (i == 1 ? ws + p.lv[0].out : C4);
    const int skip_up = (i == 1) ? 2 : 1;
    const double inner = 64.0 * L.heads;
    const double dec_fl_px = L.depth * 2.0 * (32 * inner + 4 * inner + 4 * inner + inner * 32 + 2 * 32 * 32);
    const double dec_by_px = dec_bytes_px(pos);
    const float* dectc = Wt(DH_W_LV5_DECTC + i);
    const float* tab2 = (variant == DH_VARIANT_LEVIR) ? TAB + (size_t)2 * B * L.depth * DH_TABTC_FLOATS : TAB;
    const int out_split = one ? 512 : (i == 0 ? 0 : 256);
    DH_STEP(nm[i][5], dec_fl_px * B * npix, (dec_by_px + (skip ? 32.0 * eb / (skip_up * skip_up) : 0.0)) * B * npix,
            dh_launch_pixel_decoder_tc(DX, pos, tab2, dectc, B, L.h, L.w, L.heads, L.depth, skip, skip_up, x3 | out_split, OUT, s));
    if (i == 1)
      DH_CONV3(nm[i][6], OUT, nullptr, 32, 0, 0, B, L.h, L.w, 3, 1, 128, DH_W_CL4_PSWT, DH_W_CL4_PSB, nullptr, 0, 1, C4, 0, 1);
    return 0;
  };
  AuxStreams* aux = (g_prof.on || (flags & DH_FLAG_SERIAL)) ? nullptr : aux_streams();
  if (aux) {
    if (cudaEventRecord(aux->fork, s_main) != cudaSuccess) return (int)cudaGetLastError();
    for (int i = 1; i <= 2; ++i) {
      s = aux->st[i - 1];
      if (cudaStreamWaitEvent(s, aux->fork, 0) != cudaSuccess) return (int)cudaGetLastError();
      const int rc = level_pre(i);
      if (rc == 0 && cudaEventRecord(aux->join[i - 1], s) != cudaSuccess) { s = s_main; return (int)cudaGetLastError(); }
      s = s_main;
      if (rc != 0) return rc;
    }
  }
  for (int i = 0; i < 3; ++i) {
    int rc = 0;
    if (i == 0 || !aux) rc = level_pre(i);
    else if (cudaStreamWaitEvent(s_main, aux->join[i - 1], 0) != cudaSuccess) rc = (int)cudaGetLastError();
    if (rc == 0) rc = level_post(i);
    if (rc != 0) return rc;
  }
  float *C3 = ws + p.c3, *Y20 = ws + p.y20, *O2 = ws + p.o2, *C2 = ws + p.c2;
  float* OUT3 = ws + p.lv[2].out;
  DH_CONV3("conv_layer3", OUT3, nullptr, 32, 0, 0, B, h4, w4, 3, 1, 128, DH_W_CL3_PSWT, DH_W_CL3_PSB, nullptr, 0, 1, C3, 0, 1);
  DH_CONV3("conv_layer2_0.0", F2, F2post, 64, 64, f2_plane, B, h2, w2, 3, 1, 128, DH_W_CL20A_WT, DH_W_CL20A_B, nullptr, 0, 1, Y20, 1, 0);
  DH_CONV3("conv_layer2_0.3", Y20, nullptr, 128, 0, 0, B, h2, w2, 3, 1, 32, DH_W_CL20B_WT, DH_W_CL20B_B, C3, 0, 0, O2, 1, 0);
  DH_CONV3("conv_layer2", O2, nullptr, 32, 0, 0, B, h2, w2, 3, 1, 128, DH_W_CL2_PSWT, DH_W_CL2_PSB, nullptr, 0, 1, C2, 0, 1);
  DH_STEP("classifier", 2.0 * B * H * W * 9 * 32 * output_nc,
          (one ? B * H * W * (2.0 * 32 + 4.0 * output_nc) : 4.0 * B * H * W * (32.0 + output_nc)) + (argmax_u8 ? (double)B * H * W : 0.0),
          one ? dh_launch_classifier_h16(C2, B, H, W, output_nc, Wt(DH_W_CLS_W), Wt(DH_W_CLS_B), logits, argmax_u8, s)
              : dh_launch_classifier(C2, B, H, W, output_nc, Wt(DH_W_CLS_W), Wt(DH_W_CLS_B), logits, argmax_u8, s));
  return 0;
}
}


extern "C" int dahitra_forward(const void* const* weights, int n_weights, const float* x1, const float* x2,
                               long long x_batch_stride, float* logits, unsigned char* argmax_u8, void* workspace,
                               size_t workspace_bytes, int variant, int B, int H, int W, int output_nc, int flags,
                               void* stream) {
  DH_REQUIRE(weights && x1 && x2 && logits && workspace, DH_E_NULL);
  DH_REQUIRE(n_weights == DH_W_COUNT, DH_E_WEIGHTS);
  Plan p;
  DH_REQUIRE(variant == DH_VARIANT_LEVIR || variant == DH_VARIANT_XBD, DH_E_VARIANT);
  if (flags & DH_FLAG_ACT_H16) {
    constexpr int need = DH_FLAG_CONV_TC | DH_FLAG_TC_MAIN_F16 | DH_FLAG_TC_STRIDE2 | DH_FLAG_STEM_TC | DH_FLAG_DEC_TC;
    DH_REQUIRE((flags & need) == need &&
               !(flags & (DH_FLAG_ACT_SPLIT | DH_FLAG_TC_3XTF32 | DH_FLAG_TC_BF16 | DH_FLAG_CONV_TC_V1)), DH_E_VARIANT);
  }
  DH_REQUIRE(make_plan(p, variant, B, H, W, output_nc, flags), DH_E_SHAPE);
  DH_REQUIRE(workspace_bytes >= p.total_floats * sizeof(float), DH_E_WORKSPACE);
  DH_REQUIRE(dh_aligned16(workspace), DH_E_ALIGN);
  for (int i = 0; i < DH_W_COUNT; ++i) {
    const bool optional = (i == DH_W_LV5_POS || i == DH_W_LV4_POS || i == DH_W_LV3_POS);
    DH_REQUIRE(weights[i] || optional, DH_E_WEIGHTS);
    DH_REQUIRE(dh_aligned16(weights[i]), DH_E_ALIGN);
  }
  const cudaStream_t s_main = (cudaStream_t)stream;
  cudaStream_t s = s_main;
  float* ws = (float*)workspace;
  dh_set_pdl((flags & DH_FLAG_PDL) ? 1 : 0);
  if (flags & DH_FLAG_ACT_SPLIT) {
    constexpr int need = DH_FLAG_CONV_TC | DH_FLAG_TC_MAIN_F16 | DH_FLAG_TC_STRIDE2 | DH_FLAG_STEM_TC | DH_FLAG_DEC_TC;
    DH_REQUIRE((flags & need) == need && !(flags & (DH_FLAG_TC_BF16 | DH_FLAG_CONV_TC_V1)), DH_E_VARIANT);
    return forward_split(p, weights, x1, x2, x_batch_stride, logits, argmax_u8, ws, variant, B, H, W, output_nc, flags, s_main);
  }
  if (flags & DH_FLAG_ACT_H16)
    return forward_split(p, weights, x1, x2, x_batch_stride, logits, argmax_u8, ws, variant, B, H, W, output_nc, flags, s_main);
  auto Wt = [&](int slot) { return (const float*)weights[slot]; };
  const int N2 = 2 * B;
  const int h2 = H / 2, w2 = W / 2, h4 = H / 4, w4 = W / 4, h8 = H / 8, w8 = W / 8, h16 = H / 16, w16 = W / 16;

  int conv_flat = 0;
  auto conv = [&](const char* name, const float* in0, const float* in1, int C0, int C1, int N, int inH, int inW, int up,
                  int K, int stride, int Cout, int wslot, int bslot, const float* res, int relu, float* out) -> int {
    const int wts = wt_slot_of(wslot);
    ConvArgs a{in0, in1, C0, C1, N, inH, inW, up, K, K, stride, K / 2, Cout, Wt(wslot), wts >= 0 ? Wt(wts) : nullptr,
               bslot >= 0 ? Wt(bslot) : nullptr, res, relu, out};
    const int psw = (wslot == DH_W_CL4_W) ? DH_W_CL4_PSWT : (wslot == DH_W_CL3_W) ? DH_W_CL3_PSWT
                  : (wslot == DH_W_CL2_W) ? DH_W_CL2_PSWT : -1;
    a.flat = conv_flat;
    if (up == 2 && psw >= 0 && (flags & DH_FLAG_CONV_TC)) {
      a.up = 1; a.Cout = 128; a.w = nullptr; a.wt = Wt(psw); a.bias = Wt(psw + 1); a.ps = 1;
    }
    const int rc = conv_dispatch(a, flags, s);
    if (rc != 0) return rc;
    const double OH = (double)(inH * up) / stride, OW = (double)(inW * up) / stride, Cin = C0 + C1;
    const double fl = 2.0 * N * OH * OW * Cout * K * K * Cin;
    const double by = 4.0 * ((double)N * inH * inW * Cin + (double)N * OH * OW * Cout * (res ? 2 : 1) + (double)K * K * Cin * Cout);
    prof_mark(s, name, fl, by);
    return 0;
  };
#define DH_CONV(...)                     \
  do {                                   \
    const int rc__ = conv(__VA_ARGS__);  \
    if (rc__ != 0) return rc__;          \
  } while (0)

  float* F2 = ws + p.f2;
  const double stem_fl = 2.0 * B * h2 * w2 * 64 * 147, stem_by = 4.0 * B * ((double)3 * H * W + (double)h2 * w2 * 64);
  const int stem_mode = !(flags & DH_FLAG_TC_3XTF32)
                            ? ((flags & (DH_FLAG_TC_MAIN_F16 | DH_FLAG_TC_BF16)) ? 3 : 0)
                            : ((flags & DH_FLAG_TC_FOLD) && (flags & DH_FLAG_TC_MAIN_F16) && (flags & DH_FLAG_TC_X3_BF16)) ? 2 : 1;
  auto stem = [&](const float* xin, float* o) -> int {
    return (flags & DH_FLAG_STEM_TC) ? dh_launch_stem_tc(xin, x_batch_stride, B, H, W, Wt(DH_W_STEM_WTC), Wt(DH_W_STEM_B), o,
                                                         stem_mode, s)
                                     : dh_launch_stem(xin, x_batch_stride, B, H, W, Wt(DH_W_STEM_W), Wt(DH_W_STEM_B), o, s);
  };
  DH_STEP("stem_pre", stem_fl, stem_by, stem(x1, F2));
  DH_STEP("stem_post", stem_fl, stem_by, stem(x2, F2 + (size_t)B * h2 * w2 * 64));
  AuxStreams* aux_head = (!g_prof.on && !(flags & DH_FLAG_SERIAL) && (flags & DH_FLAG_EARLY_HEAD) && (flags & DH_FLAG_CONV_TC))
                             ? aux_streams() : nullptr;
  float* Y20 = ws + p.y20;
  if (aux_head) {
    if (cudaEventRecord(aux_head->fork_low, s_main) != cudaSuccess ||
        cudaStreamWaitEvent(aux_head->low, aux_head->fork_low, 0) != cudaSuccess) return (int)cudaGetLastError();
    s = aux_head->low; conv_flat = 1;
    const int rc = conv("conv_layer2_0.0", F2, F2 + (size_t)B * h2 * w2 * 64, 64, 64, B, h2, w2, 1, 3, 1, 128, DH_W_CL20A_W, DH_W_CL20A_B,
                        nullptr, 1, Y20);
    conv_flat = 0;
    const bool ok = rc == 0 && cudaEventRecord(aux_head->join_low, s) == cudaSuccess;
    s = s_main;
    if (!ok) return rc != 0 ? rc : (int)cudaGetLastError();
  }
  float* P2 = ws + p.p2;
  DH_STEP("maxpool_2", 0.0, 4.0 * N2 * 64 * ((double)h2 * w2 + (double)h4 * w4), dh_launch_maxpool(F2, N2, h2, w2, 64, P2, s));
  float *T4a = ws + p.t4a, *T4b = ws + p.t4b, *F4 = ws + p.f4;
  DH_CONV("layer1.0.conv1", P2, nullptr, 64, 0, N2, h4, w4, 1, 3, 1, 64, DH_W_L1_0_C1_W, DH_W_L1_0_C1_B, nullptr, 1, T4a);
  DH_CONV("layer1.0.conv2", T4a, nullptr, 64, 0, N2, h4, w4, 1, 3, 1, 64, DH_W_L1_0_C2_W, DH_W_L1_0_C2_B, P2, 1, T4b);
  DH_CONV("layer1.1.conv1", T4b, nullptr, 64, 0, N2, h4, w4, 1, 3, 1, 64, DH_W_L1_1_C1_W, DH_W_L1_1_C1_B, nullptr, 1, T4a);
  DH_CONV("layer1.1.conv2", T4a, nullptr, 64, 0, N2, h4, w4, 1, 3, 1, 64, DH_W_L1_1_C2_W, DH_W_L1_1_C2_B, T4b, 1, F4);
  float *T8a = ws + p.t8a, *T8b = ws + p.t8b, *T8c = ws + p.t8c, *F8 = ws + p.f8;
  DH_CONV("layer2.0.conv1", F4, nullptr, 64, 0, N2, h4, w4, 1, 3, 2, 128, DH_W_L2_0_C1_W, DH_W_L2_0_C1_B, nullptr, 1, T8a);
  DH_CONV("layer2.0.down", F4, nullptr, 64, 0, N2, h4, w4, 1, 1, 2, 128, DH_W_L2_0_DS_W, DH_W_L2_0_DS_B, nullptr, 0, T8b);
  DH_CONV("layer2.0.conv2", T8a, nullptr, 128, 0, N2, h8, w8, 1, 3, 1, 128, DH_W_L2_0_C2_W, DH_W_L2_0_C2_B, T8b, 1, T8c);
  DH_CONV("layer2.1.conv1", T8c, nullptr, 128, 0, N2, h8, w8, 1, 3, 1, 128, DH_W_L2_1_C1_W, DH_W_L2_1_C1_B, nullptr, 1, T8a);
  DH_CONV("layer2.1.conv2", T8a, nullptr, 128, 0, N2, h8, w8, 1, 3, 1, 128, DH_W_L2_1_C2_W, DH_W_L2_1_C2_B, T8c, 1, F8);
  float* P8 = ws + p.p8;
  DH_STEP("maxpool_8", 0.0, 4.0 * N2 * 128 * ((double)h8 * w8 + (double)h16 * w16), dh_launch_maxpool(F8, N2, h8, w8, 128, P8, s));
  float *T16a = ws + p.t16a, *T16b = ws + p.t16b, *T16c = ws + p.t16c, *F16 = ws + p.f16;
  DH_CONV("layer3.0.conv1", P8, nullptr, 128, 0, N2, h16, w16, 1, 3, 1, 256, DH_W_L3_0_C1_W, DH_W_L3_0_C1_B, nullptr, 1, T16a);
  DH_CONV("layer3.0.down", P8, nullptr, 128, 0, N2, h16, w16, 1, 1, 1, 256, DH_W_L3_0_DS_W, DH_W_L3_0_DS_B, nullptr, 0, T16b);
  DH_CONV("layer3.0.conv2", T16a, nullptr, 256, 0, N2, h16, w16, 1, 3, 1, 256, DH_W_L3_0_C2_W, DH_W_L3_0_C2_B, T16b, 1, T16c);
  DH_CONV("layer3.1.conv1", T16c, nullptr, 256, 0, N2, h16, w16, 1, 3, 1, 256, DH_W_L3_1_C1_W, DH_W_L3_1_C1_B, nullptr, 1, T16a);
  DH_CONV("layer3.1.conv2", T16a, nullptr, 256, 0, N2, h16, w16, 1, 3, 1, 256, DH_W_L3_1_C2_W, DH_W_L3_1_C2_B, T16c, 1, F16);

  const float* feats[3] = {F16, F8, F4};
  const int base[3] = {DH_W_LV5_SQ, DH_W_LV4_SQ, DH_W_LV3_SQ};
  static const char* const nm[3][7] = {
      {"squeeze_tok_5", "token_enc_5", "dec_tables_5", "decoder_5_x12", "conv_decode_5", "decoder_5_diff", "conv_layer4"},
      {"squeeze_tok_4", "token_enc_4", "dec_tables_4", "decoder_4_x12", "conv_decode_4", "decoder_4_diff", "conv_layer4"},
      {"squeeze_tok_3", "token_enc_3", "dec_tables_3", "decoder_3_x12", "conv_decode_3", "decoder_3_diff", "conv_layer4"}};
  float* C4 = ws + p.c4;
  auto level_pre = [&](int i) -> int {
    const Level& L = p.lv[i];
    const int npix = L.h * L.w;
    const float *wsq = Wt(base[i] + 0), *wtok = Wt(base[i] + 1), *enc = Wt(base[i] + 2), *dec = Wt(base[i] + 3),
                *pos = Wt(base[i] + 4);
    float *XS = ws + L.xs, *XD = ws + L.xd, *DX = ws + L.dx, *PART = ws + L.part, *MEM = ws + L.mem, *TAB = ws + L.tab;
    const double inner = 64.0 * L.heads;
    const double dec_fl_px = L.depth * 2.0 * (32 * inner + 4 * inner + 4 * inner + inner * 32 + 2 * 32 * 32);
    const double dec_by_px = 4.0 * 32 * (pos ? 3 : 2);
    DH_STEP(nm[i][0], 2.0 * N2 * npix * 32 * (L.cin + 4 + 4), 4.0 * N2 * npix * (L.cin + 32.0),
            dh_launch_squeeze_tokens(feats[i], N2, npix, L.cin, wsq, wtok, XS, PART, s));
    const int add_tok_pos = (variant == DH_VARIANT_LEVIR) ? 1 : (i == 0 ? 1 : 0);
    DH_STEP(nm[i][1], 0.0, 4.0 * N2 * L.nchunk * 136.0, dh_launch_token_encoder(PART, B, L.nchunk, enc, L.heads, add_tok_pos, MEM, s));
    const size_t half = (size_t)B * npix * 32;
    const bool dtc = (flags & DH_FLAG_DEC_TC) != 0;
    const float* dectc = Wt(DH_W_LV5_DECTC + i);
    const size_t tabf = dtc ? (size_t)DH_TABTC_FLOATS : (size_t)DH_TAB_FLOATS(L.heads);
    auto tables = [&](int first, int ncalls) -> int {
      return dtc ? dh_launch_decoder_tables_tc(MEM, B, first, ncalls, dec, L.heads, L.depth, TAB, s)
                 : dh_launch_decoder_tables(MEM, B, first, ncalls, dec, L.heads, L.depth, TAB, s);
    };
    if (variant == DH_VARIANT_LEVIR) {
      DH_STEP(nm[i][2], 0.0, 4.0 * 3 * B * L.depth * tabf, tables(0, 3));
      DH_STEP(nm[i][3], dec_fl_px * N2 * npix, dec_by_px * N2 * npix,
              (dtc ? dh_launch_pixel_decoder_tc(XS, pos, TAB, dectc, N2, L.h, L.w, L.heads, L.depth, nullptr, 1,
                                                (flags & DH_FLAG_DEC_TC_X3) ? 1 : 0, XD, s)
                   : dh_launch_pixel_decoder(XS, pos, TAB, dec, N2, L.h, L.w, L.heads, L.depth, nullptr, 1, XD, s)));
      DH_CONV(nm[i][4], XD, XD + half, 32, 32, B, L.h, L.w, 1, 3, 1, 32, base[i] + 5, -1, nullptr, 0, DX);
    } else {
      DH_STEP(nm[i][2], 0.0, 4.0 * B * L.depth * tabf, tables(2, 1));
      DH_CONV(nm[i][4], XS, XS + half, 32, 32, B, L.h, L.w, 1, 3, 1, 32, base[i] + 5, -1, nullptr, 0, DX);
    }
    return 0;
  };
  auto level_post = [&](int i) -> int {
    const Level& L = p.lv[i];
    const int npix = L.h * L.w;
    const float *dec = Wt(base[i] + 3), *pos = Wt(base[i] + 4);
    float *DX = ws + L.dx, *OUT = ws + L.out, *TAB = ws + L.tab;
    const float* skip = (i == 0) ? nullptr : (i == 1 ? ws + p.lv[0].out : C4);
    const int skip_up = (i == 1) ? 2 : 1;
    const double inner = 64.0 * L.heads;
    const double dec_fl_px = L.depth * 2.0 * (32 * inner + 4 * inner + 4 * inner + inner * 32 + 2 * 32 * 32);
    const double dec_by_px = 4.0 * 32 * (pos ? 3 : 2);
    const bool dtc = (flags & DH_FLAG_DEC_TC) != 0;
    const float* dectc = Wt(DH_W_LV5_DECTC + i);
    const size_t tabf = dtc ? (size_t)DH_TABTC_FLOATS : (size_t)DH_TAB_FLOATS(L.heads);
    const float* tab2 = (variant == DH_VARIANT_LEVIR) ? TAB + (size_t)2 * B * L.depth * tabf : TAB;
    DH_STEP(nm[i][5], dec_fl_px * B * npix, (dec_by_px + (skip ? 128.0 / (skip_up * skip_up) : 0.0)) * B * npix,
            (dtc ? dh_launch_pixel_decoder_tc(DX, pos, tab2, dectc, B, L.h, L.w, L.heads, L.depth, skip, skip_up,
                                              (flags & DH_FLAG_DEC_TC_X3) ? 1 : 0, OUT, s)
                 : dh_launch_pixel_decoder(DX, pos, tab2, dec, B, L.h, L.w, L.heads, L.depth, skip, skip_up, OUT, s)));
    if (i == 1)
      DH_CONV(nm[i][6], OUT, nullptr, 32, 0, B, L.h, L.w, 2, 3, 1, 32, DH_W_CL4_W, DH_W_CL4_B, nullptr, 1, C4);
    return 0;
  };
  AuxStreams* aux = (g_prof.on || (flags & DH_FLAG_SERIAL)) ? nullptr : aux_streams();
  if (aux) {
    if (cudaEventRecord(aux->fork, s_main) != cudaSuccess) return (int)cudaGetLastError();
    for (int i = 1; i <= 2; ++i) {
      s = aux->st[i - 1];
      if (cudaStreamWaitEvent(s, aux->fork, 0) != cudaSuccess) return (int)cudaGetLastError();
      const int rc = level_pre(i);
      if (rc == 0 && cudaEventRecord(aux->join[i - 1], s) != cudaSuccess) { s = s_main; return (int)cudaGetLastError(); }
      s = s_main;
      if (rc != 0) return rc;
    }
  }
  for (int i = 0; i < 3; ++i) {
    int rc = 0;
    if (i == 0 || !aux) rc = level_pre(i);
    else if (cudaStreamWaitEvent(s_main, aux->join[i - 1], 0) != cudaSuccess) rc = (int)cudaGetLastError();
    if (rc == 0) rc = level_post(i);
    if (rc != 0) return rc;
  }
  float *C3 = ws + p.c3, *O2 = ws + p.o2, *C2 = ws + p.c2;
  const float* OUT3 = ws + p.lv[2].out;
  DH_CONV("conv_layer3", OUT3, nullptr, 32, 0, B, h4, w4, 2, 3, 1, 32, DH_W_CL3_W, DH_W_CL3_B, nullptr, 1, C3);
  const float* A128 = F2;
  const float* B128 = F2 + (size_t)B * h2 * w2 * 64;
  if (aux_head) {
    if (cudaStreamWaitEvent(s_main, aux_head->join_low, 0) != cudaSuccess) return (int)cudaGetLastError();
  } else {
    DH_CONV("conv_layer2_0.0", A128, B128, 64, 64, B, h2, w2, 1, 3, 1, 128, DH_W_CL20A_W, DH_W_CL20A_B, nullptr, 1, Y20);
  }
  DH_CONV("conv_layer2_0.3", Y20, nullptr, 128, 0, B, h2, w2, 1, 3, 1, 32, DH_W_CL20B_W, DH_W_CL20B_B, C3, 0, O2);
  DH_CONV("conv_layer2", O2, nullptr, 32, 0, B, h2, w2, 2, 3, 1, 32, DH_W_CL2_W, DH_W_CL2_B, nullptr, 1, C2);
  DH_STEP("classifier", 2.0 * B * H * W * 9 * 32 * output_nc, 4.0 * B * H * W * (32.0 + output_nc) + (argmax_u8 ? (double)B * H * W : 0.0),
          dh_launch_classifier(C2, B, H, W, output_nc, Wt(DH_W_CLS_W), Wt(DH_W_CLS_B), logits, argmax_u8, s));
  return 0;
}

extern "C" int dahitra_forward_profiled(const void* const* weights, int n_weights, const float* x1, const float* x2,
                                        long long x_batch_stride, float* logits, unsigned char* argmax_u8,
                                        void* workspace, size_t workspace_bytes, int variant, int B, int H, int W,
                                        int output_nc, int flags, void* stream, int cap, float* ms, double* flops,
                                        double* bytes, const char** names) {
  DH_REQUIRE(ms && flops && bytes && names && cap > 0, DH_E_NULL);
  cudaStream_t s = (cudaStream_t)stream;
  if (!g_prof.created) {
    for (int i = 0; i <= PROF_MAX; ++i)
      if (cudaEventCreate(&g_prof.ev[i]) != cudaSuccess) return -(int)cudaGetLastError() - 1000;
    g_prof.created = true;
  }
  g_prof.n = 0;
  g_prof.on = true;
  cudaEventRecord(g_prof.ev[0], s);
  const int rc = dahitra_forward(weights, n_weights, x1, x2, x_batch_stride, logits, argmax_u8, workspace, workspace_bytes,
                                 variant, B, H, W, output_nc, flags, stream);
  g_prof.on = false;
  if (rc != 0) return rc > 0 ? -rc - 1000 : rc;
  const cudaError_t e = cudaStreamSynchronize(s);
  if (e != cudaSuccess) return -(int)e - 1000;
  const int n = g_prof.n < cap ? g_prof.n : cap;
  for (int i = 0; i < n; ++i) {
    cudaEventElapsedTime(&ms[i], g_prof.ev[i], g_prof.ev[i + 1]);
    flops[i] = g_prof.rec[i].flops;
    bytes[i] = g_prof.rec[i].bytes;
    names[i] = g_prof.rec[i].name;
  }
  return n;
}
```

### dahitra_b200/csrc/split.cu

```cuda
#include "tc_common.cuh"
#include <cuda_fp16.h>

using namespace dhtc;

namespace {

__device__ __forceinline__ void sp_split8(const float (&v)[8], uint4& hi, uint4& lo) {
  hi.x = pack_f16x2_sat(v[0], v[1]); hi.y = pack_f16x2_sat(v[2], v[3]); hi.z = pack_f16x2_sat(v[4], v[5]); hi.w = pack_f16x2_sat(v[6], v[7]);
  lo.x = pack_f16x2_sat((v[0] - f16_lo(hi.x)) * 2048.f, (v[1] - f16_hi(hi.x)) * 2048.f);
  lo.y = pack_f16x2_sat((v[2] - f16_lo(hi.y)) * 2048.f, (v[3] - f16_hi(hi.y)) * 2048.f);
  lo.z = pack_f16x2_sat((v[4] - f16_lo(hi.z)) * 2048.f, (v[5] - f16_hi(hi.z)) * 2048.f);
  lo.w = pack_f16x2_sat((v[6] - f16_lo(hi.w)) * 2048.f, (v[7] - f16_hi(hi.w)) * 2048.f);
}
__device__ __forceinline__ void sp_join8(uint4 hi, uint4 lo, float (&v)[8]) {
  constexpr float S = 1.0f / 2048.0f;
  v[0] = fmaf(f16_lo(lo.x), S, f16_lo(hi.x)); v[1] = fmaf(f16_hi(lo.x), S, f16_hi(hi.x));
  v[2] = fmaf(f16_lo(lo.y), S, f16_lo(hi.y)); v[3] = fmaf(f16_hi(lo.y), S, f16_hi(hi.y));
  v[4] = fmaf(f16_lo(lo.z), S, f16_lo(hi.z)); v[5] = fmaf(f16_hi(lo.z), S, f16_hi(hi.z));
  v[6] = fmaf(f16_lo(lo.w), S, f16_lo(hi.w)); v[7] = fmaf(f16_hi(lo.w), S, f16_hi(hi.w));
}

__global__ void __launch_bounds__(256) split_pack_kernel(const float* __restrict__ in, size_t n8, size_t n, uint16_t* __restrict__ out) {
  for (size_t i = (size_t)blockIdx.x * blockDim.x + threadIdx.x; i < n8; i += (size_t)gridDim.x * blockDim.x) {
    const float4 a = ldg4(in + i * 8), b = ldg4(in + i * 8 + 4);
    const float v[8] = {a.x, a.y, a.z, a.w, b.x, b.y, b.z, b.w};
    uint4 hi, lo;
    sp_split8(v, hi, lo);
    *reinterpret_cast<uint4*>(out + i * 8) = hi;
    *reinterpret_cast<uint4*>(out + n + i * 8) = lo;
  }
}
__global__ void __launch_bounds__(256) split_unpack_kernel(const uint16_t* __restrict__ in, size_t n8, size_t n, float* __restrict__ out) {
  for (size_t i = (size_t)blockIdx.x * blockDim.x + threadIdx.x; i < n8; i += (size_t)gridDim.x * blockDim.x) {
    const uint4 hi = __ldg(reinterpret_cast<const uint4*>(in + i * 8)), lo = __ldg(reinterpret_cast<const uint4*>(in + n + i * 8));
    float v[8];
    sp_join8(hi, lo, v);
    st4(out + i * 8, make_float4(v[0], v[1], v[2], v[3]));
    st4(out + i * 8 + 4, make_float4(v[4], v[5], v[6], v[7]));
  }
}

__device__ __forceinline__ void lexmax2(uint32_t& mh, uint32_t& ml, uint32_t h, uint32_t l) {
  const __half2 a = *reinterpret_cast<const __half2*>(&h), m = *reinterpret_cast<const __half2*>(&mh);
  const uint32_t gt = __hgt2_mask(a, m), eq = __heq2_mask(a, m);
  const __half2 lm = __hmax2(*reinterpret_cast<const __half2*>(&l), *reinterpret_cast<const __half2*>(&ml));
  ml = (gt & l) | (eq & *reinterpret_cast<const uint32_t*>(&lm)) | (~(gt | eq) & ml);
  mh = (gt & h) | (~gt & mh);
}

__global__ void __launch_bounds__(256)
maxpool_split_kernel(const uint16_t* __restrict__ in, int N, int H, int W, int C, uint16_t* __restrict__ out) {
  const int OH = H / 2, OW = W / 2, C8 = C / 8;
  const size_t total = (size_t)N * OH * OW * C8, plane_in = (size_t)N * H * W * C, plane_out = (size_t)N * OH * OW * C;
  pdl_wait();
  pdl_launch_dependents();
  const size_t i = (size_t)blockIdx.x * blockDim.x + threadIdx.x;
  if (i >= total) return;
  const int c8 = (int)(i % C8);
  size_t p = i / C8;
  const int ox = (int)(p % OW); p /= OW;
  const int oy = (int)(p % OH);
  const int n = (int)(p / OH);
  uint4 mh = make_uint4(0xFC00FC00u, 0xFC00FC00u, 0xFC00FC00u, 0xFC00FC00u), ml = mh;
#pragma unroll
  for (int dy = -1; dy <= 1; ++dy) {
    const int iy = 2 * oy + dy;
    if (iy < 0 || iy >= H) continue;
#pragma unroll
    for (int dx = -1; dx <= 1; ++dx) {
      const int ix = 2 * ox + dx;
      if (ix < 0 || ix >= W) continue;
      const size_t o = (((size_t)n * H + iy) * W + ix) * C + c8 * 8;
      const uint4 hi = __ldg(reinterpret_cast<const uint4*>(in + o)), lo = __ldg(reinterpret_cast<const uint4*>(in + plane_in + o));
      lexmax2(mh.x, ml.x, hi.x, lo.x); lexmax2(mh.y, ml.y, hi.y, lo.y); lexmax2(mh.z, ml.z, hi.z, lo.z); lexmax2(mh.w, ml.w, hi.w, lo.w);
    }
  }
  const size_t o = (((size_t)n * OH + oy) * OW + ox) * C + c8 * 8;
  *reinterpret_cast<uint4*>(out + o) = mh;
  *reinterpret_cast<uint4*>(out + plane_out + o) = ml;
}

__global__ void __launch_bounds__(256)
maxpool_h16_kernel(const uint16_t* __restrict__ in, int N, int H, int W, int C, uint16_t* __restrict__ out) {
  const int OH = H / 2, OW = W / 2, C8 = C / 8;
  const size_t total = (size_t)N * OH * OW * C8;
  pdl_wait();
  pdl_launch_dependents();
  const size_t i = (size_t)blockIdx.x * blockDim.x + threadIdx.x;
  if (i >= total) return;
  const int c8 = (int)(i % C8);
  size_t p = i / C8;
  const int ox = (int)(p % OW); p /= OW;
  const int oy = (int)(p % OH);
  const int n = (int)(p / OH);
  __half2 m[4];
#pragma unroll
  for (int k = 0; k < 4; ++k) m[k] = __half2half2(__ushort_as_half((unsigned short)0xFC00u));
#pragma unroll
  for (int dy = -1; dy <= 1; ++dy) {
    const int iy = 2 * oy + dy;
    if (iy < 0 || iy >= H) continue;
#pragma unroll
    for (int dx = -1; dx <= 1; ++dx) {
      const int ix = 2 * ox + dx;
      if (ix < 0 || ix >= W) continue;
      const uint4 v = __ldg(reinterpret_cast<const uint4*>(in + (((size_t)n * H + iy) * W + ix) * C + c8 * 8));
      const __half2* h = reinterpret_cast<const __half2*>(&v);
#pragma unroll
      for (int k = 0; k < 4; ++k) m[k] = __hmax2(m[k], h[k]);
    }
  }
  *reinterpret_cast<uint4*>(out + (((size_t)n * OH + oy) * OW + ox) * C + c8 * 8) = *reinterpret_cast<const uint4*>(m);
}

int grid_for(size_t items) {
  int dev = 0, sms = 148;
  cudaGetDevice(&dev);
  cudaDeviceGetAttribute(&sms, cudaDevAttrMultiProcessorCount, dev);
  const size_t want = (items + 255) / 256, cap = (size_t)sms * 8;
  return (int)(want < cap ? (want ? want : 1) : cap);
}
}

int dh_launch_split_pack(const float* in, size_t n, void* out, cudaStream_t s) {
  DH_REQUIRE(in && out, DH_E_NULL);
  DH_REQUIRE(n % 8 == 0 && n > 0, DH_E_SHAPE);
  DH_REQUIRE(dh_aligned16(in) && dh_aligned16(out), DH_E_ALIGN);
  split_pack_kernel<<<grid_for(n / 8), 256, 0, s>>>(in, n / 8, n, reinterpret_cast<uint16_t*>(out));
  DH_CHECK_LAUNCH();
  return 0;
}
int dh_launch_split_unpack(const void* in, size_t n, float* out, cudaStream_t s) {
  DH_REQUIRE(in && out, DH_E_NULL);
  DH_REQUIRE(n % 8 == 0 && n > 0, DH_E_SHAPE);
  DH_REQUIRE(dh_aligned16(in) && dh_aligned16(out), DH_E_ALIGN);
  split_unpack_kernel<<<grid_for(n / 8), 256, 0, s>>>(reinterpret_cast<const uint16_t*>(in), n / 8, n, out);
  DH_CHECK_LAUNCH();
  return 0;
}
int dh_launch_maxpool_split(const void* in, int N, int H, int W, int C, void* out, cudaStream_t s) {
  DH_REQUIRE(in && out, DH_E_NULL);
  DH_REQUIRE(N > 0 && H >= 2 && W >= 2 && H % 2 == 0 && W % 2 == 0 && C % 8 == 0, DH_E_SHAPE);
  DH_REQUIRE(dh_aligned16(in) && dh_aligned16(out), DH_E_ALIGN);
  const size_t items = (size_t)N * (H / 2) * (W / 2) * (C / 8);
  cudaLaunchConfig_t cfg = {};
  cfg.gridDim = dim3((unsigned)((items + 255) / 256)); cfg.blockDim = dim3(256); cfg.stream = s;
  cudaLaunchAttribute at[1];
  cfg.attrs = at; cfg.numAttrs = dh_pdl_attr(at);
  const cudaError_t e = cudaLaunchKernelEx(&cfg, maxpool_split_kernel, reinterpret_cast<const uint16_t*>(in), N, H, W, C,
                                           reinterpret_cast<uint16_t*>(out));
  if (e != cudaSuccess) return (int)e;
  DH_CHECK_LAUNCH();
  return 0;
}
int dh_launch_maxpool_h16(const void* in, int N, int H, int W, int C, void* out, cudaStream_t s) {
  DH_REQUIRE(in && out, DH_E_NULL);
  DH_REQUIRE(N > 0 && H >= 2 && W >= 2 && H % 2 == 0 && W % 2 == 0 && C % 8 == 0, DH_E_SHAPE);
  DH_REQUIRE(dh_aligned16(in) && dh_aligned16(out), DH_E_ALIGN);
  const size_t items = (size_t)N * (H / 2) * (W / 2) * (C / 8);
  return dh_launch(maxpool_h16_kernel, dim3((unsigned)((items + 255) / 256)), dim3(256), 0, s,
                   reinterpret_cast<const uint16_t*>(in), N, H, W, C, reinterpret_cast<uint16_t*>(out));
}
```

### dahitra_b200/csrc/tc_common.cuh

```cuda
#pragma once
#include "common.cuh"
#include <cuda.h>
#include <cstdio>

int dh_encode_tiled_f32(CUtensorMap* out, const void* ptr, int rank, const unsigned long long* dims,
                        const unsigned long long* strides, const unsigned* box, bool swizzle128);
int dh_encode_tiled_f32_sw(CUtensorMap* out, const void* ptr, int rank, const unsigned long long* dims,
                           const unsigned long long* strides, const unsigned* box, int swizzle_bytes);
int dh_encode_tiled_f16_sw(CUtensorMap* out, const void* ptr, int rank, const unsigned long long* dims,
                           const unsigned long long* strides, const unsigned* box, int swizzle_bytes);

namespace dhtc {

__device__ __forceinline__ uint32_t smem_u32(const void* p) { return (uint32_t)__cvta_generic_to_shared(p); }

__device__ __forceinline__ void mbar_init(uint32_t bar, uint32_t count) {
  asm volatile("mbarrier.init.shared::cta.b64 [%0], %1;" ::"r"(bar), "r"(count) : "memory");
}
__device__ __forceinline__ void mbar_fence_init() { asm volatile("fence.mbarrier_init.release.cluster;" ::: "memory"); }
__device__ __forceinline__ void mbar_expect_tx(uint32_t bar, uint32_t bytes) {
  asm volatile("mbarrier.arrive.expect_tx.shared::cta.b64 _, [%0], %1;" ::"r"(bar), "r"(bytes) : "memory");
}
__device__ __forceinline__ void pdl_wait() { asm volatile("griddepcontrol.wait;" ::: "memory"); }
__device__ __forceinline__ void pdl_launch_dependents() { asm volatile("griddepcontrol.launch_dependents;" ::: "memory"); }

__device__ __forceinline__ void mbar_wait(uint32_t bar, uint32_t parity) {
  uint32_t done;
#ifdef DH_MBAR_TIMEOUT
  uint32_t spins = 0;
#endif
  do {
    asm volatile(
        "{\n\t.reg .pred p;\n\t"
        "mbarrier.try_wait.parity.shared::cta.b64 p, [%1], %2, %3;\n\t"
        "selp.u32 %0, 1, 0, p;\n\t}"
        : "=r"(done) : "r"(bar), "r"(parity), "r"(10000u) : "memory");
#ifdef DH_MBAR_TIMEOUT
    if (!done && ++spins > (1u << 19)) {
      printf("[mbar timeout] block %d thread %d bar smem+0x%x parity %u\n", blockIdx.x, threadIdx.x, bar, parity);
      __trap();
    }
#endif
  } while (!done);
}
__device__ __forceinline__ uint32_t cluster_ctarank() { uint32_t r; asm volatile("mov.u32 %0, %%cluster_ctarank;" : "=r"(r)); return r; }
__device__ __forceinline__ void cluster_sync_all() {
  asm volatile("barrier.cluster.arrive.release.aligned;" ::: "memory");
  asm volatile("barrier.cluster.wait.acquire.aligned;" ::: "memory");
}
__device__ __forceinline__ uint32_t mapa_u32(uint32_t smem_addr, uint32_t rank) {
  uint32_t r;
  asm volatile("mapa.shared::cluster.u32 %0, %1, %2;" : "=r"(r) : "r"(smem_addr), "r"(rank));
  return r;
}
__device__ __forceinline__ void mbar_arrive_local(uint32_t bar) {
  asm volatile("mbarrier.arrive.shared::cta.b64 _, [%0];" ::"r"(bar) : "memory");
}
__device__ __forceinline__ void mbar_arrive_cluster(uint32_t cluster_bar) {
  asm volatile("mbarrier.arrive.release.cluster.shared::cluster.b64 _, [%0];" ::"r"(cluster_bar) : "memory");
}
__device__ __forceinline__ void mbar_wait_cluster(uint32_t bar, uint32_t parity) {
  uint32_t done;
#ifdef DH_MBAR_TIMEOUT
  uint32_t spins = 0;
#endif
  do {
    asm volatile(
        "{\n\t.reg .pred p;\n\t"
        "mbarrier.try_wait.parity.acquire.cluster.shared::cta.b64 p, [%1], %2, %3;\n\t"
        "selp.u32 %0, 1, 0, p;\n\t}"
        : "=r"(done) : "r"(bar), "r"(parity), "r"(10000u) : "memory");
#ifdef DH_MBAR_TIMEOUT
    if (!done && ++spins > (1u << 19)) __trap();
#endif
  } while (!done);
}
__device__ __forceinline__ void tma_load_4d_2sm(uint32_t dst, const CUtensorMap* tm, uint32_t cluster_bar, int c0, int c1, int c2, int c3) {
  asm volatile(
      "cp.async.bulk.tensor.4d.cta_group::2.shared::cluster.global.tile.mbarrier::complete_tx::bytes [%0], [%1, {%3, %4, %5, %6}], [%2];"
      ::"r"(dst), "l"(tm), "r"(cluster_bar), "r"(c0), "r"(c1), "r"(c2), "r"(c3) : "memory");
}
__device__ __forceinline__ void tma_load_2d_2sm(uint32_t dst, const CUtensorMap* tm, uint32_t cluster_bar, int c0, int c1) {
  asm volatile(
      "cp.async.bulk.tensor.2d.cta_group::2.shared::cluster.global.tile.mbarrier::complete_tx::bytes [%0], [%1, {%3, %4}], [%2];"
      ::"r"(dst), "l"(tm), "r"(cluster_bar), "r"(c0), "r"(c1) : "memory");
}
__device__ __forceinline__ float tf32_round(float v) {
  return __uint_as_float((__float_as_uint(v) + 0x1000u) & 0xFFFFE000u);
}
__device__ __forceinline__ void tma_load_4d(uint32_t dst, const CUtensorMap* tm, uint32_t bar, int c0, int c1, int c2, int c3) {
  asm volatile(
      "cp.async.bulk.tensor.4d.shared::cluster.global.tile.mbarrier::complete_tx::bytes [%0], [%1, {%3, %4, %5, %6}], [%2];"
      ::"r"(dst), "l"(tm), "r"(bar), "r"(c0), "r"(c1), "r"(c2), "r"(c3) : "memory");
}
__device__ __forceinline__ void tma_load_2d(uint32_t dst, const CUtensorMap* tm, uint32_t bar, int c0, int c1) {
  asm volatile(
      "cp.async.bulk.tensor.2d.shared::cluster.global.tile.mbarrier::complete_tx::bytes [%0], [%1, {%3, %4}], [%2];"
      ::"r"(dst), "l"(tm), "r"(bar), "r"(c0), "r"(c1) : "memory");
}
__device__ __forceinline__ void bulk_load_1d(uint32_t dst, const void* src, uint32_t bytes, uint32_t bar) {
  asm volatile("cp.async.bulk.shared::cluster.global.mbarrier::complete_tx::bytes [%0], [%1], %2, [%3];"
               ::"r"(dst), "l"(src), "r"(bytes), "r"(bar) : "memory");
}
__device__ __forceinline__ void fence_async_smem() { asm volatile("fence.proxy.async.shared::cta;" ::: "memory"); }
__device__ __forceinline__ void tc_fence_before() { asm volatile("tcgen05.fence::before_thread_sync;" ::: "memory"); }
__device__ __forceinline__ void tc_fence_after() { asm volatile("tcgen05.fence::after_thread_sync;" ::: "memory"); }

__device__ __forceinline__ uint64_t umma_desc_sw128(uint32_t smem_addr) {
  return (uint64_t)((smem_addr & 0x3FFFF) >> 4) | ((uint64_t)1 << 16) | ((uint64_t)(1024 >> 4) << 32) |
         ((uint64_t)1 << 46) | ((uint64_t)2 << 61);
}
__host__ __device__ constexpr uint32_t umma_idesc_tf32(int M, int N) {
  return (1u << 4) | (2u << 7) | (2u << 10) | ((uint32_t)(N >> 3) << 17) | ((uint32_t)(M >> 4) << 24);
}
__device__ __forceinline__ void umma_tf32(uint32_t tmem_d, uint64_t adesc, uint64_t bdesc, uint32_t idesc, uint32_t accumulate) {
  asm volatile(
      "{\n\t.reg .pred p;\n\t"
      "setp.ne.b32 p, %4, 0;\n\t"
      "tcgen05.mma.cta_group::1.kind::tf32 [%0], %1, %2, %3, p;\n\t}"
      ::"r"(tmem_d), "l"(adesc), "l"(bdesc), "r"(idesc), "r"(accumulate) : "memory");
}
__device__ __forceinline__ uint64_t umma_desc_sw64(uint32_t smem_addr, uint32_t sbo_bytes) {
  return (uint64_t)((smem_addr & 0x3FFFF) >> 4) | ((uint64_t)1 << 16) | ((uint64_t)(sbo_bytes >> 4) << 32) |
         ((uint64_t)1 << 46) | ((uint64_t)4 << 61);
}
__host__ __device__ constexpr uint32_t umma_idesc_bf16(int M, int N) {
  return (1u << 4) | (1u << 7) | (1u << 10) | ((uint32_t)(N >> 3) << 17) | ((uint32_t)(M >> 4) << 24);
}
__device__ __forceinline__ void umma_bf16(uint32_t tmem_d, uint64_t adesc, uint64_t bdesc, uint32_t idesc, uint32_t accumulate) {
  asm volatile(
      "{\n\t.reg .pred p;\n\t"
      "setp.ne.b32 p, %4, 0;\n\t"
      "tcgen05.mma.cta_group::1.kind::f16 [%0], %1, %2, %3, p;\n\t}"
      ::"r"(tmem_d), "l"(adesc), "l"(bdesc), "r"(idesc), "r"(accumulate) : "memory");
}
__host__ __device__ constexpr uint32_t umma_idesc_f16(int M, int N) {
  return (1u << 4) | ((uint32_t)(N >> 3) << 17) | ((uint32_t)(M >> 4) << 24);
}
__device__ __forceinline__ uint32_t pack_f16x2_sat(float lo, float hi) {
  uint32_t r;
  asm("cvt.rn.satfinite.f16x2.f32 %0, %1, %2;" : "=r"(r) : "f"(hi), "f"(lo));
  return r;
}
__device__ __forceinline__ float f16_lo(uint32_t p) { float f; asm("{ .reg .b16 l, h; mov.b32 {l, h}, %1; cvt.f32.f16 %0, l; }" : "=f"(f) : "r"(p)); return f; }
__device__ __forceinline__ float f16_hi(uint32_t p) { float f; asm("{ .reg .b16 l, h; mov.b32 {l, h}, %1; cvt.f32.f16 %0, h; }" : "=f"(f) : "r"(p)); return f; }
__device__ __forceinline__ uint32_t pack_bf16x2(float lo, float hi) {
  uint32_t r;
  asm("cvt.rn.bf16x2.f32 %0, %1, %2;" : "=r"(r) : "f"(hi), "f"(lo));
  return r;
}
__device__ __forceinline__ void umma_tf32_ts(uint32_t tmem_d, uint32_t tmem_a, uint64_t bdesc, uint32_t idesc, uint32_t accumulate) {
  asm volatile(
      "{\n\t.reg .pred p;\n\t"
      "setp.ne.b32 p, %4, 0;\n\t"
      "tcgen05.mma.cta_group::1.kind::tf32 [%0], [%1], %2, %3, p;\n\t}"
      ::"r"(tmem_d), "r"(tmem_a), "l"(bdesc), "r"(idesc), "r"(accumulate) : "memory");
}
__device__ __forceinline__ void umma_tf32_2sm(uint32_t tmem_d, uint64_t adesc, uint64_t bdesc, uint32_t idesc, uint32_t accumulate) {
  asm volatile(
      "{\n\t.reg .pred p;\n\t"
      "setp.ne.b32 p, %4, 0;\n\t"
      "tcgen05.mma.cta_group::2.kind::tf32 [%0], %1, %2, %3, p;\n\t}"
      ::"r"(tmem_d), "l"(adesc), "l"(bdesc), "r"(idesc), "r"(accumulate) : "memory");
}
__device__ __forceinline__ void umma_bf16_2sm(uint32_t tmem_d, uint64_t adesc, uint64_t bdesc, uint32_t idesc, uint32_t accumulate) {
  asm volatile(
      "{\n\t.reg .pred p;\n\t"
      "setp.ne.b32 p, %4, 0;\n\t"
      "tcgen05.mma.cta_group::2.kind::f16 [%0], %1, %2, %3, p;\n\t}"
      ::"r"(tmem_d), "l"(adesc), "l"(bdesc), "r"(idesc), "r"(accumulate) : "memory");
}
__device__ __forceinline__ void umma_commit_2sm(uint32_t bar) {
  asm volatile("tcgen05.commit.cta_group::2.mbarrier::arrive::one.shared::cluster.multicast::cluster.b64 [%0], %1;"
               ::"r"(bar), "h"((uint16_t)3) : "memory");
}
__device__ __forceinline__ void tmem_alloc_2sm(uint32_t slot_smem_addr, uint32_t ncols) {
  asm volatile("tcgen05.alloc.cta_group::2.sync.aligned.shared::cta.b32 [%0], %1;" ::"r"(slot_smem_addr), "r"(ncols) : "memory");
  asm volatile("tcgen05.relinquish_alloc_permit.cta_group::2.sync.aligned;" ::: "memory");
}
__device__ __forceinline__ void tmem_dealloc_2sm(uint32_t taddr, uint32_t ncols) {
  asm volatile("tcgen05.dealloc.cta_group::2.sync.aligned.b32 %0, %1;" ::"r"(taddr), "r"(ncols) : "memory");
}
__device__ __forceinline__ void umma_commit(uint32_t bar) {
  asm volatile("tcgen05.commit.cta_group::1.mbarrier::arrive::one.shared::cluster.b64 [%0];" ::"r"(bar) : "memory");
}
__device__ __forceinline__ void tmem_alloc(uint32_t slot_smem_addr, uint32_t ncols) {
  asm volatile("tcgen05.alloc.cta_group::1.sync.aligned.shared::cta.b32 [%0], %1;" ::"r"(slot_smem_addr), "r"(ncols) : "memory");
  asm volatile("tcgen05.relinquish_alloc_permit.cta_group::1.sync.aligned;" ::: "memory");
}
__device__ __forceinline__ void tmem_dealloc(uint32_t taddr, uint32_t ncols) {
  asm volatile("tcgen05.dealloc.cta_group::1.sync.aligned.b32 %0, %1;" ::"r"(taddr), "r"(ncols) : "memory");
}
__device__ __forceinline__ void tmem_ld32(uint32_t taddr, uint32_t (&v)[32]) {
  asm volatile(
      "tcgen05.ld.sync.aligned.32x32b.x32.b32 "
      "{%0, %1, %2, %3, %4, %5, %6, %7, %8, %9, %10, %11, %12, %13, %14, %15, "
      "%16, %17, %18, %19, %20, %21, %22, %23, %24, %25, %26, %27, %28, %29, %30, %31}, [%32];"
      : "=r"(v[0]), "=r"(v[1]), "=r"(v[2]), "=r"(v[3]), "=r"(v[4]), "=r"(v[5]), "=r"(v[6]), "=r"(v[7]),
        "=r"(v[8]), "=r"(v[9]), "=r"(v[10]), "=r"(v[11]), "=r"(v[12]), "=r"(v[13]), "=r"(v[14]), "=r"(v[15]),
        "=r"(v[16]), "=r"(v[17]), "=r"(v[18]), "=r"(v[19]), "=r"(v[20]), "=r"(v[21]), "=r"(v[22]), "=r"(v[23]),
        "=r"(v[24]), "=r"(v[25]), "=r"(v[26]), "=r"(v[27]), "=r"(v[28]), "=r"(v[29]), "=r"(v[30]), "=r"(v[31])
      : "r"(taddr) : "memory");
  asm volatile("tcgen05.wait::ld.sync.aligned;" ::: "memory");
}
__device__ __forceinline__ void tmem_ld16(uint32_t taddr, uint32_t (&v)[16]) {
  asm volatile(
      "tcgen05.ld.sync.aligned.32x32b.x16.b32 "
      "{%0, %1, %2, %3, %4, %5, %6, %7, %8, %9, %10, %11, %12, %13, %14, %15}, [%16];"
      : "=r"(v[0]), "=r"(v[1]), "=r"(v[2]), "=r"(v[3]), "=r"(v[4]), "=r"(v[5]), "=r"(v[6]), "=r"(v[7]),
        "=r"(v[8]), "=r"(v[9]), "=r"(v[10]), "=r"(v[11]), "=r"(v[12]), "=r"(v[13]), "=r"(v[14]), "=r"(v[15])
      : "r"(taddr) : "memory");
  asm volatile("tcgen05.wait::ld.sync.aligned;" ::: "memory");
}
__device__ __forceinline__ void tmem_st32(uint32_t taddr, const uint32_t (&v)[32]) {
  asm volatile(
      "tcgen05.st.sync.aligned.32x32b.x32.b32 [%0], "
      "{%1, %2, %3, %4, %5, %6, %7, %8, %9, %10, %11, %12, %13, %14, %15, %16, "
      "%17, %18, %19, %20, %21, %22, %23, %24, %25, %26, %27, %28, %29, %30, %31, %32};"
      ::"r"(taddr), "r"(v[0]), "r"(v[1]), "r"(v[2]), "r"(v[3]), "r"(v[4]), "r"(v[5]), "r"(v[6]), "r"(v[7]),
        "r"(v[8]), "r"(v[9]), "r"(v[10]), "r"(v[11]), "r"(v[12]), "r"(v[13]), "r"(v[14]), "r"(v[15]),
        "r"(v[16]), "r"(v[17]), "r"(v[18]), "r"(v[19]), "r"(v[20]), "r"(v[21]), "r"(v[22]), "r"(v[23]),
        "r"(v[24]), "r"(v[25]), "r"(v[26]), "r"(v[27]), "r"(v[28]), "r"(v[29]), "r"(v[30]), "r"(v[31])
      : "memory");
  asm volatile("tcgen05.wait::st.sync.aligned;" ::: "memory");
}

__device__ __forceinline__ unsigned long long f2_pack(float2 a) { unsigned long long r; asm("mov.b64 %0, {%1, %2};" : "=l"(r) : "f"(a.x), "f"(a.y)); return r; }
__device__ __forceinline__ float2 f2_unpack(unsigned long long r) { float2 d; asm("mov.b64 {%0, %1}, %2;" : "=f"(d.x), "=f"(d.y) : "l"(r)); return d; }
__device__ __forceinline__ float2 ffma2(float2 a, float2 b, float2 c) {
  unsigned long long d; asm("fma.rn.f32x2 %0, %1, %2, %3;" : "=l"(d) : "l"(f2_pack(a)), "l"(f2_pack(b)), "l"(f2_pack(c))); return f2_unpack(d);
}
__device__ __forceinline__ float2 fadd2(float2 a, float2 b) { unsigned long long d; asm("add.rn.f32x2 %0, %1, %2;" : "=l"(d) : "l"(f2_pack(a)), "l"(f2_pack(b))); return f2_unpack(d); }
__device__ __forceinline__ float2 fsub2(float2 a, float2 b) { unsigned long long d; asm("sub.rn.f32x2 %0, %1, %2;" : "=l"(d) : "l"(f2_pack(a)), "l"(f2_pack(b))); return f2_unpack(d); }
__device__ __forceinline__ float2 fmul2(float2 a, float2 b) { unsigned long long d; asm("mul.rn.f32x2 %0, %1, %2;" : "=l"(d) : "l"(f2_pack(a)), "l"(f2_pack(b))); return f2_unpack(d); }
__device__ __forceinline__ float2 f2_bcast(float s) { return make_float2(s, s); }

__host__ __device__ __forceinline__ int sw128_idx(int r, int k) { return r * 32 + ((((k >> 2) ^ (r & 7)) << 2) | (k & 3)); }

}
```

### dahitra_b200/engine.py

```python
from __future__ import annotations

import ctypes as C
import os

import torch

from . import _lib

BN_EPS = 1e-5
SCALE = 32 ** -0.5
LEVELS = ((5, 256, 4, 4), (4, 128, 4, 4), (3, 64, 8, 8))

DH_VARIANT_LEVIR, DH_VARIANT_XBD = 0, 1
DH_FLAG_CONV_TC, DH_FLAG_TC_3XTF32, DH_FLAG_TC_STRIDE2, DH_FLAG_DEC_TC, DH_FLAG_STEM_TC, DH_FLAG_DEC_TC_X3 = 1, 2, 4, 8, 16, 32
DH_FLAG_CONV_TC_V1, DH_FLAG_CONV_TC_2CTA, DH_FLAG_SERIAL, DH_FLAG_TC_X3_BF16, DH_FLAG_TC_BF16 = 64, 128, 256, 512, 1024
DH_FLAG_TC_MAIN_F16, DH_FLAG_TC_FOLD, DH_FLAG_EARLY_HEAD, DH_FLAG_ACT_SPLIT, DH_FLAG_PDL = 2048, 4096, 8192, 16384, 32768
DH_FLAG_ACT_H16 = 65536
MODES = {
    "fp32": 0,
    "fp32_tcdec": DH_FLAG_DEC_TC | DH_FLAG_DEC_TC_X3,
    "tf32x3": DH_FLAG_CONV_TC | DH_FLAG_TC_3XTF32 | DH_FLAG_TC_X3_BF16 | DH_FLAG_TC_MAIN_F16 | DH_FLAG_TC_FOLD | DH_FLAG_TC_STRIDE2
              | DH_FLAG_STEM_TC | DH_FLAG_DEC_TC | DH_FLAG_DEC_TC_X3 | DH_FLAG_ACT_SPLIT | DH_FLAG_PDL,
    "tf32x3_fp32act": DH_FLAG_CONV_TC | DH_FLAG_TC_3XTF32 | DH_FLAG_TC_X3_BF16 | DH_FLAG_TC_MAIN_F16 | DH_FLAG_TC_FOLD | DH_FLAG_TC_STRIDE2
                      | DH_FLAG_STEM_TC | DH_FLAG_DEC_TC | DH_FLAG_DEC_TC_X3,
    "tf32x3_unfolded": DH_FLAG_CONV_TC | DH_FLAG_TC_3XTF32 | DH_FLAG_TC_X3_BF16 | DH_FLAG_TC_MAIN_F16 | DH_FLAG_TC_STRIDE2 | DH_FLAG_STEM_TC
                       | DH_FLAG_DEC_TC | DH_FLAG_DEC_TC_X3,
    "tf32x3_tf32main": DH_FLAG_CONV_TC | DH_FLAG_TC_3XTF32 | DH_FLAG_TC_X3_BF16 | DH_FLAG_TC_STRIDE2 | DH_FLAG_STEM_TC | DH_FLAG_DEC_TC
                       | DH_FLAG_DEC_TC_X3,
    "tf32x3_pure": DH_FLAG_CONV_TC | DH_FLAG_TC_3XTF32 | DH_FLAG_TC_STRIDE2 | DH_FLAG_STEM_TC | DH_FLAG_DEC_TC | DH_FLAG_DEC_TC_X3,
    "tf32": DH_FLAG_CONV_TC | DH_FLAG_TC_STRIDE2 | DH_FLAG_STEM_TC | DH_FLAG_DEC_TC | DH_FLAG_DEC_TC_X3,
    "f16": DH_FLAG_CONV_TC | DH_FLAG_TC_MAIN_F16 | DH_FLAG_TC_STRIDE2 | DH_FLAG_STEM_TC | DH_FLAG_DEC_TC | DH_FLAG_DEC_TC_X3,
    "bf16": DH_FLAG_CONV_TC | DH_FLAG_TC_BF16 | DH_FLAG_TC_STRIDE2 | DH_FLAG_STEM_TC | DH_FLAG_DEC_TC | DH_FLAG_DEC_TC_X3,
    "h16": DH_FLAG_CONV_TC | DH_FLAG_TC_MAIN_F16 | DH_FLAG_TC_STRIDE2 | DH_FLAG_STEM_TC | DH_FLAG_DEC_TC | DH_FLAG_DEC_TC_X3
           | DH_FLAG_ACT_H16 | DH_FLAG_PDL,
    "tf32_fast": DH_FLAG_CONV_TC | DH_FLAG_TC_STRIDE2 | DH_FLAG_STEM_TC | DH_FLAG_DEC_TC,
}

DEFAULT_MODE = "tf32x3"


def resolve_mode(mode):
    if isinstance(mode, int):
        return mode
    if mode not in MODES:
        raise ValueError(f"dahitra_b200: unknown precision mode {mode!r}; choose from {sorted(MODES)}")
    return MODES[mode]


def slot_names():
    lib = _lib.load()
    out, i = [], 0
    while True:
        s = lib.dahitra_weight_slot_name(i)
        if s is None:
            return out
        out.append(s.decode())
        i += 1


def _fold_conv_bn(sd, conv, bn):
    w = sd[conv + ".weight"].double()
    if bn is None:
        return w, (sd[conv + ".bias"].double() if (conv + ".bias") in sd else None)
    g, b = sd[bn + ".weight"].double(), sd[bn + ".bias"].double()
    mu, var = sd[bn + ".running_mean"].double(), sd[bn + ".running_var"].double()
    k = g / torch.sqrt(var + BN_EPS)
    return w * k[:, None, None, None], b - mu * k


def _khwc(w):
    o, i, kh, kw = w.shape
    return w.permute(2, 3, 1, 0).reshape(kh * kw * i, o)


def upsample_phase_filter(w, b):
    cout, cin = w.shape[:2]
    rows = {0: {-1: [0], 0: [1, 2]}, 1: {0: [0, 1], 1: [2]}}
    W3 = torch.zeros(4, cout, 3, 3, cin, dtype=w.dtype)
    for py in (0, 1):
        for px in (0, 1):
            for u, rs in rows[py].items():
                for v, ss in rows[px].items():
                    acc = torch.zeros(cout, cin, dtype=w.dtype)
                    for r in rs:
                        for s in ss:
                            acc += w[:, :, r, s]
                    W3[py * 2 + px, :, u + 1, v + 1, :] = acc
    return W3.reshape(4 * cout, 9 * cin), b.repeat(4)


def tf32_round(x):
    b = x.to(torch.float32).contiguous().view(torch.int32)
    return ((b + 0x1000) & ~0x1FFF).view(torch.float32)


def tf32_split(x):
    hi = tf32_round(x).double()
    lo = tf32_round(x - hi).double()
    return hi, lo


def kmajor_split(wt):
    wt = wt.contiguous().double()
    hi, lo = tf32_split(wt)
    b16 = torch.stack([wt, wt - hi]).to(torch.float32).to(torch.bfloat16).contiguous()
    packed = b16.view(torch.int16).reshape(-1).view(torch.float32).reshape(wt.shape)
    h16 = wt.clamp(-65504.0, 65504.0).to(torch.float32).to(torch.float16)
    r16 = (wt - h16.double()).to(torch.float32).to(torch.bfloat16)
    packed_f = torch.cat([h16.contiguous().view(torch.int16).reshape(-1), r16.contiguous().view(torch.int16).reshape(-1)]) \
        .view(torch.float32).reshape(wt.shape)
    s16 = ((wt - h16.double()) * 2048.0).clamp(-65504.0, 65504.0).to(torch.float32).to(torch.float16)
    packed_s = torch.cat([s16.contiguous().view(torch.int16).reshape(-1), torch.zeros(s16.numel(), dtype=torch.int16)]) \
        .view(torch.float32).reshape(wt.shape)
    return torch.cat([torch.stack([hi, lo]).to(torch.float32), packed[None], packed_f[None], packed_s[None]])


def stem_tc_image(w147):
    w = w147.double().reshape(7, 7, 3, 64)
    wk = torch.zeros(24, 8, 64, dtype=torch.float64)
    wk[:21, 1:8] = w.permute(2, 0, 1, 3).reshape(21, 7, 64)
    wk = wk.reshape(192, 64)
    hi, lo = tf32_split(wk)
    img = lambda m: torch.cat([swizzle128(m[kt * 32:(kt + 1) * 32].T.contiguous()) for kt in range(6)])
    h16 = wk.clamp(-65504.0, 65504.0).to(torch.float32).to(torch.float16)
    s16 = ((wk - h16.double()) * 2048.0).clamp(-65504.0, 65504.0).to(torch.float32).to(torch.float16)
    main = torch.cat([h16, s16], dim=1).view(torch.int16)
    corr = wk.to(torch.float32).to(torch.bfloat16).view(torch.int16)
    img16 = lambda m: torch.cat([swizzle128_16(m[kt * 64:(kt + 1) * 64].T.contiguous()) for kt in range(3)]).view(torch.float32)
    return torch.cat([img(hi).to(torch.float32), img(lo).to(torch.float32), img16(main), img16(corr)])


def swizzle128_16(m):
    rows = m.shape[0]
    n = torch.arange(rows)[:, None].expand(rows, 64)
    k = torch.arange(64)[None, :].expand(rows, 64)
    idx = n * 64 + ((((k >> 3) ^ (n & 7)) << 3) | (k & 7))
    out = torch.empty(rows * 64, dtype=m.dtype)
    out[idx.reshape(-1)] = m.reshape(-1)
    return out


def swizzle128(m):
    rows = m.shape[0]
    n = torch.arange(rows)[:, None].expand(rows, 32)
    k = torch.arange(32)[None, :].expand(rows, 32)
    idx = n * 32 + ((((k >> 2) ^ (n & 7)) << 2) | (k & 3))
    out = torch.empty(rows * 32, dtype=m.dtype)
    out[idx.reshape(-1)] = m.reshape(-1)
    return out


def _heads(w, h):
    return w.reshape(h, -1, w.shape[-1])


def prepare_weights(sd: dict, variant: int, out_nc: int) -> dict:
    sd = {k: v.detach().cpu() for k, v in sd.items()}
    P = {}

    tc_slots = {"DH_W_L1_0_C1", "DH_W_L1_0_C2", "DH_W_L1_1_C1", "DH_W_L1_1_C2", "DH_W_L2_0_C2", "DH_W_L2_1_C1",
                "DH_W_L2_1_C2", "DH_W_L3_0_C1", "DH_W_L3_0_C2", "DH_W_L3_0_DS", "DH_W_L3_1_C1", "DH_W_L3_1_C2",
                "DH_W_CL20A", "DH_W_CL20B", "DH_W_L2_0_C1", "DH_W_L2_0_DS"}

    def put_conv(slot, conv, bn):
        w, b = _fold_conv_bn(sd, conv, bn)
        P[slot + "_W"] = _khwc(w)
        P[slot + "_B"] = b
        if slot in tc_slots:
            P[slot + "_WT"] = kmajor_split(_khwc(w).T)

    put_conv("DH_W_STEM", "resnet.conv1", "resnet.bn1")
    P["DH_W_STEM_WTC"] = stem_tc_image(P["DH_W_STEM_W"])
    for li in (1, 2, 3):
        for bi in (0, 1):
            p = f"resnet.layer{li}.{bi}"
            put_conv(f"DH_W_L{li}_{bi}_C1", p + ".conv1", p + ".bn1")
            put_conv(f"DH_W_L{li}_{bi}_C2", p + ".conv2", p + ".bn2")
            if (p + ".downsample.0.weight") in sd:
                put_conv(f"DH_W_L{li}_{bi}_DS", p + ".downsample.0", p + ".downsample.1")
    for k, cin, heads, depth in LEVELS:
        s = f"DH_W_LV{k}_"
        P[s + "SQ"] = sd[f"conv_squeeze_{k}.0.weight"].double()[:, :, 0, 0].T
        P[s + "TOK"] = sd[f"conv_token_{k}.weight"].double()[:, :, 0, 0].T
        P[s + "SQ_WT"] = kmajor_split(P[s + "SQ"].T)
        P[s + "DECODE"] = _khwc(sd[f"conv_decode_{k}.weight"].double())
        P[s + "DECODE_WT"] = kmajor_split(P[s + "DECODE"].T)
        t = f"transformer_{k}.layers.0"
        if variant == DH_VARIANT_LEVIR:
            pos = sd[f"pos_embedding_{k}"].double().reshape(-1) if f"pos_embedding_{k}" in sd \
                else torch.zeros(256, dtype=torch.float64)
        else:
            pos = sd["pos_embedding_3"].double().reshape(-1) if (k == 5 and "pos_embedding_3" in sd) \
                else torch.zeros(256, dtype=torch.float64)
        wqkv = sd[t + ".0.fn.fn.to_qkv.weight"].double()
        inner = heads * 64
        wq, wk, wv = (_heads(wqkv[i * inner:(i + 1) * inner], heads) for i in range(3))
        wo = sd[t + ".0.fn.fn.to_out.0.weight"].double().reshape(32, heads, 64).permute(1, 0, 2)
        mqk = SCALE * torch.einsum("hdc,hde->hce", wq, wk)
        mvoT = torch.einsum("hcd,hde->hec", wo, wv)
        P[s + "ENC"] = torch.cat([
            pos, sd[t + ".0.fn.norm.weight"].double(), sd[t + ".0.fn.norm.bias"].double(),
            mqk.reshape(-1), mvoT.reshape(-1), sd[t + ".0.fn.fn.to_out.0.bias"].double(),
            sd[t + ".1.fn.norm.weight"].double(), sd[t + ".1.fn.norm.bias"].double(),
            sd[t + ".1.fn.fn.net.0.weight"].double().T.reshape(-1), sd[t + ".1.fn.fn.net.0.bias"].double(),
            sd[t + ".1.fn.fn.net.3.weight"].double().T.reshape(-1), sd[t + ".1.fn.fn.net.3.bias"].double()])
        layers = []
        for l in range(depth):
            d = f"transformer_decoder_{k}.layers.{l}"
            wq = _heads(sd[d + ".0.fn.fn.to_q.weight"].double(), heads)
            wk = _heads(sd[d + ".0.fn.fn.to_k.weight"].double(), heads)
            wv = _heads(sd[d + ".0.fn.fn.to_v.weight"].double(), heads)
            wo = sd[d + ".0.fn.fn.to_out.0.weight"].double().reshape(32, heads, 64).permute(1, 0, 2)
            mqkT = SCALE * torch.einsum("hdc,hde->hec", wq, wk)
            movT = torch.einsum("hcd,hde->hec", wo, wv)
            g2, b2n = sd[d + ".1.fn.norm.weight"].double(), sd[d + ".1.fn.norm.bias"].double()
            w1, b1 = sd[d + ".1.fn.fn.net.0.weight"].double(), sd[d + ".1.fn.fn.net.0.bias"].double()
            w2, b2 = sd[d + ".1.fn.fn.net.3.weight"].double(), sd[d + ".1.fn.fn.net.3.bias"].double()
            layers += [sd[d + ".0.fn.norm.weight"].double(), sd[d + ".0.fn.norm.bias"].double(),
                       mqkT.reshape(-1), movT.reshape(-1), sd[d + ".0.fn.fn.to_out.0.bias"].double(),
                       (w1 * g2[None, :]).T.reshape(-1), b1 + w1 @ b2n, w2.T.reshape(-1), b2]
        P[s + "DEC"] = torch.cat(layers)
        tc_layers, cum = [], torch.zeros(32, dtype=torch.float64)
        for l in range(depth):
            d = f"transformer_decoder_{k}.layers.{l}"
            g2, b2n = sd[d + ".1.fn.norm.weight"].double(), sd[d + ".1.fn.norm.bias"].double()
            w1, b1 = sd[d + ".1.fn.fn.net.0.weight"].double(), sd[d + ".1.fn.fn.net.0.bias"].double()
            w2, b2 = sd[d + ".1.fn.fn.net.3.weight"].double(), sd[d + ".1.fn.fn.net.3.bias"].double()
            cba = cum + sd[d + ".0.fn.fn.to_out.0.bias"].double()
            cum = cba + b2
            w1h, w1l = tf32_split(w1 * g2[None, :])
            w2h, w2l = tf32_split(w2)
            tc_layers += [swizzle128(w1h), swizzle128(w2h), b1 + w1 @ b2n, cba, cum.clone(), swizzle128(w1l), swizzle128(w2l)]
        P[s + "DECTC"] = torch.cat(tc_layers)
        if variant == DH_VARIANT_LEVIR:
            pe = sd.get(f"pos_embedding_decoder_{k}")
        else:
            pe = sd.get("pos_embedding_decoder_3") if k == 5 else None
        P[s + "POS"] = None if pe is None else pe.double()[0].permute(1, 2, 0).reshape(-1, 32)
    for name, key in (("DH_W_CL4", "conv_layer4.0"), ("DH_W_CL3", "conv_layer3.0"), ("DH_W_CL2", "conv_layer2.0")):
        put_conv(name, key, None)
        pw, pb = upsample_phase_filter(sd[key + ".weight"].double(), sd[key + ".bias"].double())
        P[name + "_PSWT"], P[name + "_PSB"] = kmajor_split(pw), pb
    put_conv("DH_W_CL20A", "conv_layer2_0.0", "conv_layer2_0.1")
    put_conv("DH_W_CL20B", "conv_layer2_0.3", None)
    wc = sd["classifier.weight"].double()
    assert wc.shape[0] == out_nc
    P["DH_W_CLS_W"] = wc.permute(2, 3, 0, 1).reshape(9, out_nc, 32)
    P["DH_W_CLS_B"] = sd["classifier.bias"].double()
    return {k: (None if v is None else v.to(torch.float32).contiguous()) for k, v in P.items()}


def prepare_weights_c(sd: dict, variant: int, out_nc: int):
    lib = _lib.load()
    keep, recs = [], []
    for k, v in sd.items():
        if not torch.is_tensor(v) or not v.dtype.is_floating_point or v.dim() > 4:
            continue
        t = v.detach().cpu().contiguous()
        if t.dtype not in (torch.float32, torch.float64):
            t = t.float()
        keep.append((k.encode(), t))
    arr = (_lib.DhTensor * len(keep))()
    for i, (name, t) in enumerate(keep):
        arr[i].name, arr[i].data = name, t.data_ptr()
        arr[i].dtype, arr[i].ndim = (0 if t.dtype == torch.float32 else 1), t.dim()
        for j, d in enumerate(t.shape):
            arr[i].shape[j] = d
    n = lib.dahitra_prepare_weights(arr, len(keep), variant, out_nc, None, 0, None)
    if n <= 0:
        _lib.check(int(n), "dahitra_prepare_weights")
    flat = torch.zeros(n, dtype=torch.float32)
    offs = (C.c_longlong * len(slot_names()))()
    n2 = lib.dahitra_prepare_weights(arr, len(keep), variant, out_nc, flat.data_ptr(), n, offs)
    if n2 != n:
        _lib.check(int(n2) if n2 < 0 else -6, "dahitra_prepare_weights")
    return flat, list(offs)


F16_MAX = 65504.0


def _filter_absmax(flat: torch.Tensor, offs: dict):
    import bisect
    ends = sorted(offs.values()) + [flat.numel()]
    worst, where = 0.0, None
    for name, o in offs.items():
        if name.endswith(("_W", "_DECODE", "_SQ")):
            seg = flat[o:ends[bisect.bisect_right(ends, o)]]
            m = float(seg.abs().max()) if seg.numel() else 0.0
            if not m <= worst:
                worst, where = m, name
                if m != m:
                    break
    return worst, where


class PreparedWeights:

    def __init__(self, sd, variant, out_nc, device):
        names = slot_names()
        if os.environ.get("DAHITRA_PREPARE", "c") == "py":
            host = prepare_weights(sd, variant, out_nc)
            missing = [n for n in names if n not in host]
            if missing:
                raise RuntimeError(f"weight preparation does not produce slots {missing}")
            offs, total = {}, 0
            for n in names:
                if host[n] is not None:
                    offs[n] = total
                    total += (host[n].numel() + 63) // 64 * 64
            flat = torch.zeros(total, dtype=torch.float32)
            for n, o in offs.items():
                flat[o:o + host[n].numel()] = host[n].reshape(-1)
        else:
            flat, off_list = prepare_weights_c(sd, variant, out_nc)
            offs = {n: o for n, o in zip(names, off_list) if o >= 0}
        self.filter_absmax = _filter_absmax(flat, offs)
        if not (self.filter_absmax[0] <= F16_MAX):
            import warnings
            warnings.warn(f"dahitra_b200: folded filter {self.filter_absmax[1]} has max |w| = {self.filter_absmax[0]:.4g}, outside the FP16 "
                          "operand range of the default mode (values saturate at 65504); use net.set_mode('tf32x3_tf32main') or 'fp32' "
                          "for this checkpoint (DESIGN.md, 'FP16 operand caveat')", RuntimeWarning, stacklevel=3)
        self.flat = flat.to(device)
        base = self.flat.data_ptr()
        self.table = (C.c_void_p * len(names))(*[(base + 4 * offs[n]) if n in offs else None for n in names])
        self.n = len(names)
        self.names = names
        self.offs = offs
        self.pos_positions = {}
        for k in (5, 4, 3):
            key = f"pos_embedding_decoder_{k}" if variant == DH_VARIANT_LEVIR else ("pos_embedding_decoder_3" if k == 5 else None)
            if key is not None and key in sd and f"DH_W_LV{k}_POS" in offs:
                self.pos_positions[f"DH_W_LV{k}_POS"] = int(sd[key].shape[2] * sd[key].shape[3])

    def ptr(self, name):
        return self.flat.data_ptr() + 4 * self.offs[name] if name in self.offs else None


class NativeEngine:
    def __init__(self):
        self._preps = {}
        self._tensors = None
        self._fingerprint = None
        self._ws = {}
        if "DAHITRA_FLAGS" in os.environ:
            self.flags = int(os.environ["DAHITRA_FLAGS"])
        else:
            self.flags = resolve_mode(os.environ.get("DAHITRA_MODE", DEFAULT_MODE))
        self.last_argmax = None

    def __deepcopy__(self, memo):
        e = NativeEngine.__new__(NativeEngine)
        e.__setstate__(self.__getstate__())
        return e

    def __getstate__(self):
        return {"flags": self.flags}

    def __setstate__(self, st):
        self._preps, self._tensors, self._fingerprint, self._ws, self.last_argmax = {}, None, None, {}, None
        self.flags = st.get("flags", MODES[DEFAULT_MODE])

    def set_mode(self, mode):
        self.flags = resolve_mode(mode)

    @property
    def mode(self):
        return next((k for k, v in MODES.items() if v == self.flags), f"flags{self.flags}")

    def invalidate(self):
        self._preps = {}
        self._tensors = None
        self._fingerprint = None

    def release_workspaces(self):
        self._ws = {}

    def _live_fingerprint(self, module):
        ts = self._tensors
        if ts is None:
            ts = self._tensors = [t for t in list(module.parameters()) + list(module.buffers())]
        return (tuple(t._version for t in ts), ts[0].data_ptr() if ts else 0, len(ts))

    def _prepared(self, module, device):
        fp = self._live_fingerprint(module)
        if fp != self._fingerprint:
            self._preps = {}
            self._fingerprint = fp
        key = (str(device), module.VARIANT)
        prep = self._preps.get(key)
        if prep is None:
            variant = DH_VARIANT_LEVIR if module.VARIANT == "levir" else DH_VARIANT_XBD
            prep = self._preps[key] = PreparedWeights(module.state_dict(), variant, module.output_nc, device)
        return prep

    def _workspace(self, lib, device, variant, B, H, W, nc):
        stream = torch.cuda.current_stream(device)
        capturing = torch.cuda.is_current_stream_capturing()
        nbytes = lib.dahitra_workspace_bytes(variant, B, H, W, nc, self.flags)
        if nbytes == 0:
            raise RuntimeError(f"dahitra_b200: unsupported shape B={B} H={H} W={W} (H, W must be multiples of 32)")
        key = (str(device), "capture" if capturing else stream.cuda_stream, variant, B, H, W, nc, nbytes)
        ws = self._ws.get(key)
        if ws is None:
            ws = torch.empty(nbytes, dtype=torch.uint8, device=device)
            self._ws[key] = ws
        return ws

    def run(self, module, x1, x2, batch_stride, B, H, W, want_argmax=False):
        lib = _lib.load()
        dev = x1.device
        variant = DH_VARIANT_LEVIR if module.VARIANT == "levir" else DH_VARIANT_XBD
        prep = self._prepared(module, dev)
        for name, hw in module.pos_shapes(H, W).items():
            have = prep.pos_positions.get(name)
            if have is not None and have != hw:
                raise RuntimeError(
                    f"dahitra_b200: decoder positional embedding {name} has {have} positions but the input needs {hw} "
                    f"(the {module.VARIANT} variant only runs at the resolution its embeddings were built for, like the reference)")
        nc = module.output_nc
        ws = self._workspace(lib, dev, variant, B, H, W, nc)
        logits = torch.empty((B, nc, H, W), dtype=torch.float32, device=dev)
        amax = torch.empty((B, H, W), dtype=torch.uint8, device=dev) if want_argmax else None
        stream = torch.cuda.current_stream(dev).cuda_stream
        with torch.cuda.device(dev):
            rc = lib.dahitra_forward(prep.table, prep.n, x1.data_ptr(), x2.data_ptr(), batch_stride,
                                     logits.data_ptr(), amax.data_ptr() if amax is not None else None,
                                     ws.data_ptr(), ws.numel(), variant, B, H, W, nc, self.flags, stream)
        _lib.check(rc, "dahitra_forward")
        self.last_argmax = amax
        return logits

    def profile_pair(self, module, x1, x2):
        lib = _lib.load()
        x1 = x1.float().contiguous()
        x2 = x2.float().contiguous()
        B, _, H, W = x1.shape
        dev = x1.device
        variant = DH_VARIANT_LEVIR if module.VARIANT == "levir" else DH_VARIANT_XBD
        prep = self._prepared(module, dev)
        nc = module.output_nc
        ws = self._workspace(lib, dev, variant, B, H, W, nc)
        logits = torch.empty((B, nc, H, W), dtype=torch.float32, device=dev)
        cap = 160
        ms, fl, by = (C.c_float * cap)(), (C.c_double * cap)(), (C.c_double * cap)()
        names = (C.c_char_p * cap)()
        stream = torch.cuda.current_stream(dev).cuda_stream
        with torch.cuda.device(dev):
            n = lib.dahitra_forward_profiled(prep.table, prep.n, x1.data_ptr(), x2.data_ptr(), 3 * H * W, logits.data_ptr(),
                                             None, ws.data_ptr(), ws.numel(), variant, B, H, W, nc, self.flags, stream,
                                             cap, ms, fl, by, names)
        if n <= 0:
            _lib.check(n if n > -1000 else -(n + 1000), "dahitra_forward_profiled")
        return [dict(name=names[i].decode(), ms=float(ms[i]), flops=float(fl[i]), bytes=float(by[i])) for i in range(n)]

    def forward_pair(self, module, x1, x2, want_argmax=False):
        if x1.shape != x2.shape or x1.dim() != 4 or x1.shape[1] != 3:
            raise RuntimeError(f"dahitra_b200: expected two (B,3,H,W) tensors, got {tuple(x1.shape)} and {tuple(x2.shape)}")
        x1 = x1.float().contiguous()
        x2 = x2.float().contiguous()
        B, _, H, W = x1.shape
        return self.run(module, x1, x2, 3 * H * W, B, H, W, want_argmax)

    def forward_stacked(self, module, x, want_argmax=False):
        if x.dim() != 4 or x.shape[1] != 6:
            raise RuntimeError(f"dahitra_b200: expected a (B,6,H,W) tensor, got {tuple(x.shape)}")
        x = x.float().contiguous()
        B, _, H, W = x.shape
        return self.run(module, x, x[:, 3:], 6 * H * W, B, H, W, want_argmax)
```

### include/dahitra_b200.h

```cpp
#ifndef DAHITRA_B200_H
#define DAHITRA_B200_H

#include <stddef.h>
#include <stdint.h>

#ifdef __cplusplus
extern "C" {
#endif

#define DAHITRA_ABI_VERSION 2

#define DH_E_NULL      (-1)
#define DH_E_SHAPE     (-2)
#define DH_E_ALIGN     (-3)
#define DH_E_WORKSPACE (-4)
#define DH_E_VARIANT   (-5)
#define DH_E_WEIGHTS   (-6)

#define DH_VARIANT_LEVIR 0
#define DH_VARIANT_XBD   1

#define DH_FLAG_NONE        0
#define DH_FLAG_CONV_TC     1
#define DH_FLAG_TC_3XTF32   2
#define DH_FLAG_TC_STRIDE2  4
#define DH_FLAG_DEC_TC      8
#define DH_FLAG_STEM_TC     16
#define DH_FLAG_DEC_TC_X3   32
#define DH_FLAG_CONV_TC_V1  64
#define DH_FLAG_CONV_TC_2CTA 128
#define DH_FLAG_SERIAL      256
#define DH_FLAG_TC_X3_BF16  512
#define DH_FLAG_TC_BF16     1024
#define DH_FLAG_TC_MAIN_F16 2048
#define DH_FLAG_TC_FOLD     4096
#define DH_FLAG_EARLY_HEAD  8192
#define DH_FLAG_ACT_SPLIT   16384
#define DH_FLAG_PDL         32768
#define DH_FLAG_ACT_H16     65536
#define DH_FLAGS_TF32X3     (DH_FLAG_CONV_TC | DH_FLAG_TC_3XTF32 | DH_FLAG_TC_X3_BF16 | DH_FLAG_TC_MAIN_F16 | DH_FLAG_TC_FOLD | DH_FLAG_TC_STRIDE2 | \
                             DH_FLAG_STEM_TC | DH_FLAG_DEC_TC | DH_FLAG_DEC_TC_X3 | DH_FLAG_ACT_SPLIT | DH_FLAG_PDL)
#define DH_FLAGS_TF32       (DH_FLAG_CONV_TC | DH_FLAG_TC_STRIDE2 | DH_FLAG_STEM_TC | DH_FLAG_DEC_TC | DH_FLAG_DEC_TC_X3)
#define DH_FLAGS_F16        (DH_FLAGS_TF32 | DH_FLAG_TC_MAIN_F16)
#define DH_FLAGS_BF16       (DH_FLAGS_TF32 | DH_FLAG_TC_BF16)
#define DH_FLAGS_H16        (DH_FLAGS_F16 | DH_FLAG_ACT_H16 | DH_FLAG_PDL)

enum dh_weight_slot {
  DH_W_STEM_W = 0, DH_W_STEM_B,
  DH_W_L1_0_C1_W, DH_W_L1_0_C1_B, DH_W_L1_0_C2_W, DH_W_L1_0_C2_B,
  DH_W_L1_1_C1_W, DH_W_L1_1_C1_B, DH_W_L1_1_C2_W, DH_W_L1_1_C2_B,
  DH_W_L2_0_C1_W, DH_W_L2_0_C1_B, DH_W_L2_0_C2_W, DH_W_L2_0_C2_B, DH_W_L2_0_DS_W, DH_W_L2_0_DS_B,
  DH_W_L2_1_C1_W, DH_W_L2_1_C1_B, DH_W_L2_1_C2_W, DH_W_L2_1_C2_B,
  DH_W_L3_0_C1_W, DH_W_L3_0_C1_B, DH_W_L3_0_C2_W, DH_W_L3_0_C2_B, DH_W_L3_0_DS_W, DH_W_L3_0_DS_B,
  DH_W_L3_1_C1_W, DH_W_L3_1_C1_B, DH_W_L3_1_C2_W, DH_W_L3_1_C2_B,
  DH_W_LV5_SQ, DH_W_LV5_TOK, DH_W_LV5_ENC, DH_W_LV5_DEC, DH_W_LV5_POS, DH_W_LV5_DECODE,
  DH_W_LV4_SQ, DH_W_LV4_TOK, DH_W_LV4_ENC, DH_W_LV4_DEC, DH_W_LV4_POS, DH_W_LV4_DECODE,
  DH_W_LV3_SQ, DH_W_LV3_TOK, DH_W_LV3_ENC, DH_W_LV3_DEC, DH_W_LV3_POS, DH_W_LV3_DECODE,
  DH_W_CL4_W, DH_W_CL4_B, DH_W_CL3_W, DH_W_CL3_B, DH_W_CL2_W, DH_W_CL2_B,
  DH_W_CL20A_W, DH_W_CL20A_B,
  DH_W_CL20B_W, DH_W_CL20B_B,
  DH_W_CLS_W, DH_W_CLS_B,
  DH_W_L1_0_C1_WT, DH_W_L1_0_C2_WT, DH_W_L1_1_C1_WT, DH_W_L1_1_C2_WT,
  DH_W_L2_0_C2_WT, DH_W_L2_1_C1_WT, DH_W_L2_1_C2_WT,
  DH_W_L3_0_C1_WT, DH_W_L3_0_C2_WT, DH_W_L3_0_DS_WT, DH_W_L3_1_C1_WT, DH_W_L3_1_C2_WT,
  DH_W_LV5_DECODE_WT, DH_W_LV4_DECODE_WT, DH_W_LV3_DECODE_WT,
  DH_W_CL20A_WT, DH_W_CL20B_WT,
  DH_W_L2_0_C1_WT, DH_W_L2_0_DS_WT,
  DH_W_CL4_PSWT, DH_W_CL4_PSB, DH_W_CL3_PSWT, DH_W_CL3_PSB, DH_W_CL2_PSWT, DH_W_CL2_PSB,
  DH_W_LV5_DECTC, DH_W_LV4_DECTC, DH_W_LV3_DECTC,
  DH_W_STEM_WTC,
  DH_W_LV5_SQ_WT, DH_W_LV4_SQ_WT, DH_W_LV3_SQ_WT,
  DH_W_COUNT
};

#define DH_ENC_FLOATS(H)       (8*32 + 64 + 2*(H)*1024 + 32 + 64 + 1024 + 32 + 1024 + 32)
#define DH_DEC_LAYER_FLOATS(H) (64 + 2*(H)*1024 + 32 + 1024 + 32 + 1024 + 32)

int         dahitra_version(void);
const char* dahitra_error_string(int code);
const char* dahitra_weight_slot_name(int slot);

#define DH_DTYPE_F32 0
#define DH_DTYPE_F64 1
typedef struct dh_tensor { const char* name; const void* data; int dtype; int ndim; long long shape[4]; } dh_tensor;
long long dahitra_prepare_weights(const dh_tensor* tensors, int n_tensors, int variant, int output_nc,
                                  float* out, long long out_floats, long long* slot_offsets);

size_t dahitra_workspace_bytes(int variant, int B, int H, int W, int output_nc, int flags);

int dahitra_forward(const void* const* weights, int n_weights,
                    const float* x1, const float* x2, long long x_batch_stride,
                    float* logits, unsigned char* argmax_u8,
                    void* workspace, size_t workspace_bytes,
                    int variant, int B, int H, int W, int output_nc, int flags, void* stream);

int dahitra_forward_profiled(const void* const* weights, int n_weights,
                             const float* x1, const float* x2, long long x_batch_stride,
                             float* logits, unsigned char* argmax_u8,
                             void* workspace, size_t workspace_bytes,
                             int variant, int B, int H, int W, int output_nc, int flags, void* stream,
                             int cap, float* ms, double* flops, double* bytes, const char** names);


int dahitra_conv2d(const float* in0, const float* in1, int C0, int C1, int N, int inH, int inW, int up,
                   int KH, int KW, int stride, int pad, int Cout,
                   const float* w, const float* wt, const float* bias, const float* res, int relu,
                   float* out, int flags, void* stream);

int dahitra_conv2d_up2_tc(const float* in, int N, int inH, int inW, const float* pswt, const float* psb,
                          int relu, float* out, int flags, void* stream);

int dahitra_stem(const float* x, long long x_batch_stride, int N, int H, int W,
                 const float* w, const float* bias, float* out, void* stream);

int dahitra_stem_tc(const float* x, long long x_batch_stride, int N, int H, int W,
                    const float* wtc, const float* bias, float* out, int x3, void* stream);

int dahitra_maxpool3x3s2(const float* in, int N, int H, int W, int C, float* out, void* stream);

int dahitra_squeeze_tokens(const float* feat, int N, int npix, int Cin, const float* w_sq, const float* w_tok,
                           float* xs, float* partials, void* stream);

int dahitra_token_encoder(const float* partials, int B, int nchunk, const float* enc_pack, int heads, int add_pos,
                          float* mem, void* stream);

#define DH_TAB_FLOATS(H) (32*4*(H) + 4*(H) + 4*(H)*32 + 32)
int dahitra_decoder_tables(const float* mem, int B, int first_call, int ncalls, const float* dec_pack, int heads, int depth,
                           float* tables, void* stream);

int dahitra_pixel_decoder(const float* x, const float* pos, const float* tables, const float* dec_pack,
                          int nimg, int h, int w, int heads, int depth, const float* skip, int skip_up, float* out,
                          void* stream);

#define DH_TABTC_FLOATS        (1024 + 1024 + 32 + 2048)
#define DH_DECTC_LAYER_FLOATS  (1024 + 1024 + 32 + 32 + 32 + 2048)
int dahitra_decoder_tables_tc(const float* mem, int B, int first_call, int ncalls, const float* dec_pack, int heads,
                              int depth, float* tables, void* stream);
int dahitra_pixel_decoder_tc(const float* x, const float* pos, const float* tables, const float* dectc_pack,
                             int nimg, int h, int w, int heads, int depth, const float* skip, int skip_up, int x3,
                             float* out, void* stream);

int dahitra_split_pack(const float* in, long long n, void* out_split, void* stream);
int dahitra_split_unpack(const void* in_split, long long n, float* out, void* stream);
int dahitra_maxpool3x3s2_split(const void* in_split, int N, int H, int W, int C, void* out_split, void* stream);
int dahitra_maxpool3x3s2_h16(const void* in_h16, int N, int H, int W, int C, void* out_h16, void* stream);
int dahitra_conv2d_split(const void* in0, const void* in1, int C0, int C1, long long in0_plane, long long in1_plane,
                         int N, int inH, int inW, int K, int stride, int Cout, const float* wt, const float* bias,
                         const void* res, int res_split, int relu, void* out, int out_split, int mode,
                         const float* w_tok, float* partials, void* stream);

int dahitra_classifier(const float* in, int N, int H, int W, int nc, const float* w, const float* bias,
                       float* logits, unsigned char* argmax_u8, void* stream);
int dahitra_classifier_h16(const void* in_h16, int N, int H, int W, int nc, const float* w, const float* bias,
                           float* logits, unsigned char* argmax_u8, void* stream);

#define DH_TRAIN_TAB_FLOATS(H) (65*4*(H) + 96 + 2048)
int dahitra_pixel_decoder_train_blocks(int npix);
int dahitra_pixel_decoder_train_fwd(const float* x, const float* tables, float* xs, float* out, int nimg, int npix,
                                    int heads, int depth, int pixel_major, void* stream);
int dahitra_pixel_decoder_train_bwd(const float* dout, const float* xs, const float* tables, float* dx,
                                    float* dtables_partial, int nimg, int npix, int heads, int depth, int pixel_major,
                                    void* stream);

#define DH_ACT_F32  0
#define DH_ACT_F16  1
#define DH_ACT_BF16 2
int dahitra_pixel_decoder_train_fwd_ex(const void* x, const float* tables, float* xs, void* out, int nimg, int npix,
                                       int heads, int depth, int pixel_major, int act_dtype, void* stream);
int dahitra_pixel_decoder_train_bwd_ex(const void* dout, const float* xs, const float* tables, void* dx,
                                       float* dtables_partial, int nimg, int npix, int heads, int depth, int pixel_major,
                                       int act_dtype, void* stream);

int dahitra_tokenizer_train_chunks(int npix);
int dahitra_tokenizer_train_fwd(const float* x, const float* w_tok, float* partials, float* tokens, float* stats,
                                int nimg, int npix, int pixel_major, void* stream);
int dahitra_tokenizer_train_bwd(const float* x, const float* w_tok, const float* tokens, const float* stats,
                                const float* dtokens, float* dx, float* dw_partial, int nimg, int npix, int pixel_major,
                                void* stream);
int dahitra_tokenizer_train_fwd_ex(const void* x, const float* w_tok, float* partials, float* tokens, float* stats,
                                   int nimg, int npix, int pixel_major, int act_dtype, void* stream);
int dahitra_tokenizer_train_bwd_ex(const void* x, const float* w_tok, const float* tokens, const float* stats,
                                   const float* dtokens, void* dx, float* dw_partial, int nimg, int npix, int pixel_major,
                                   int act_dtype, void* stream);


int dahitra_confusion_matrix(const unsigned char* pred, const unsigned char* gt, long long n, int nc,
                             long long* cm, void* stream);

int dahitra_prepare_input_u8(const unsigned char* hwc, int N, int H, int W, int kind, int tile, float* nchw, void* stream);

#ifdef __cplusplus
}
#endif
#endif
```

Before: 17110.

## Fuse 3x3 stride-2 maxpool into conv_layer2_0.0 via extra pooling warps on halo

Adds a pooling role of four extra warps to the tc3 conv kernel. These warps read the already-staged input halo tiles in shared memory and write the 3x3/s2 maxpool of both input images, so the standalone maxpool_2 kernel and its re-read of F2 from global memory go away. conv_layer2_0.0 is moved earlier in the forward pass (early head) to run in its place. In exchange the block gets 128 more threads, the halo-empty barrier waits on more arrivals, the resident-weights path is disabled for this conv, and the Y20 buffer must stay live longer.

```diff
diff --git a/dahitra_b200/_lib.py b/dahitra_b200/_lib.py
--- a/dahitra_b200/_lib.py
+++ b/dahitra_b200/_lib.py
@@ -155,6 +155,7 @@
     "dahitra_tokenizer_train_bwd_ex": (_I, [_P, _P, _P, _P, _P, _P, _P, _I, _I, _I, _I, _P]),
     "dahitra_conv2d_split": (_I, [_P, _P, _I, _I, _LL, _LL, _I, _I, _I, _I, _I, _I, _P, _P, _P, _I, _I, _P, _I, _I, _P, _P, _P]),
     "dahitra_maxpool3x3s2_h16": (_I, [_P, _I, _I, _I, _I, _P, _P]),
+    "dahitra_conv2d_split_pool": (_I, [_P, _P, _I, _LL, _I, _I, _I, _I, _P, _P, _I, _P, _P, _LL, _I, _P]),
     "dahitra_classifier_h16": (_I, [_P, _I, _I, _I, _I, _P, _P, _P, _P, _P]),
 }
 
diff --git a/dahitra_b200/csrc/common.cuh b/dahitra_b200/csrc/common.cuh
--- a/dahitra_b200/csrc/common.cuh
+++ b/dahitra_b200/csrc/common.cuh
@@ -65,6 +65,7 @@
   int force_stream = 0;
   int cg = 0;
   int h16 = 0;
+  void* pool = nullptr; long long pool_plane = 0;
 };
 bool dh_conv_tc3_eligible(const Conv3Args& a);
 int dh_launch_conv_tc3(const Conv3Args& a, cudaStream_t s);
diff --git a/dahitra_b200/csrc/conv_tc3.cu b/dahitra_b200/csrc/conv_tc3.cu
--- a/dahitra_b200/csrc/conv_tc3.cu
+++ b/dahitra_b200/csrc/conv_tc3.cu
@@ -23,6 +23,7 @@
   int res_split, out_split, tiles_per_img;
   int hb;
   uint32_t halo_plane_bytes;
+  void* pool; long long pool_plane;
 };
 
 template <int NT, bool RES, int CG = 1, bool P1 = false> struct T3Cfg {
@@ -95,12 +96,13 @@
 __device__ __forceinline__ uint4 ldg16(const void* p) { return __ldg(reinterpret_cast<const uint4*>(p)); }
 __device__ __forceinline__ float4 as_f4(const uint4& u) { return make_float4(__uint_as_float(u.x), __uint_as_float(u.y), __uint_as_float(u.z), __uint_as_float(u.w)); }
 
-template <int NT, int KS, int SD, int EPI, bool RES, int CG, bool P1>
-__global__ void __launch_bounds__(T3Cfg<NT, RES, CG, P1>::THREADS, 1)
+template <int NT, int KS, int SD, int EPI, bool RES, int CG, bool P1, bool POOL>
+__global__ void __launch_bounds__(T3Cfg<NT, RES, CG, P1>::THREADS + (POOL ? 128 : 0), 1)
 conv_tc3_kernel(const __grid_constant__ CUtensorMap tmA0h, const __grid_constant__ CUtensorMap tmA0l,
                 const __grid_constant__ CUtensorMap tmA1h, const __grid_constant__ CUtensorMap tmA1l,
                 const __grid_constant__ CUtensorMap tmB, const T3Args e) {
   using Cfg = T3Cfg<NT, RES, CG, P1>;
+  static_assert(!POOL || (KS == 3 && SD == 1 && CG == 1), "the pooling role needs the halo of a 3x3 stride-1 tile");
   constexpr int STAGES = Cfg::STAGES;
   extern __shared__ uint8_t t3_raw[];
   __shared__ __align__(8) uint64_t halo_full[T3_MAX_HB], halo_empty[T3_MAX_HB], b_full[STAGES], b_empty[STAGES], acc_full[2], acc_empty[2];
@@ -124,7 +126,7 @@
   const uint32_t epi_off = (uint32_t)HB * Cfg::HALO + w_bytes;
 
   if (threadIdx.x == 0) {
-    for (int i = 0; i < T3_MAX_HB; ++i) { mbar_init(smem_u32(&halo_full[i]), 1); mbar_init(smem_u32(&halo_empty[i]), 1); }
+    for (int i = 0; i < T3_MAX_HB; ++i) { mbar_init(smem_u32(&halo_full[i]), 1); mbar_init(smem_u32(&halo_empty[i]), POOL ? 129 : 1); }
     for (int i = 0; i < 2; ++i) { mbar_init(smem_u32(&acc_full[i]), 1); mbar_init(smem_u32(&acc_empty[i]), 128 * CG); }
     for (int s = 0; s < STAGES; ++s) { mbar_init(smem_u32(&b_full[s]), 1); mbar_init(smem_u32(&b_empty[s]), 1); }
     mbar_fence_init();
@@ -278,6 +280,50 @@
         if (CG == 2) umma_commit_2sm(smem_u32(&acc_full[ab])); else umma_commit(smem_u32(&acc_full[ab]));
       }
     }
+  } else if (POOL && warp >= 11) {
+    const int PH = e.OH >> 1, PW = e.OW >> 1, PC = e.cchunks0 * 32, gq = lane & 3, pg = warp - 11;
+    uint16_t* pout = reinterpret_cast<uint16_t*>(e.pool);
+    int hb = 0;
+    uint32_t hphase = 0;
+    for (int tile = w0; tile < e.ntiles; tile += wstep) {
+      const Tile3 t = tile3(tile, e);
+      for (int cc = 0; cc < e.cchunks; ++cc) {
+        mbar_wait(smem_u32(&halo_full[hb]), hphase);
+        if (t.ct == 0) {
+          const bool second = cc >= e.cchunks0;
+          const size_t img = second ? (size_t)e.N + t.n : (size_t)t.n;
+          const int c0 = (second ? cc - e.cchunks0 : cc) * 32 + gq * 8;
+          const uint8_t* hbuf = base_ptr + (size_t)hb * Cfg::HALO;
+          {
+            const int pp = pg * 8 + (lane >> 2), ri = pp >> 2, rj = pp & 3;
+            const int oy = (t.oy0 >> 1) + ri, ox = (t.ox0 >> 1) + rj;
+            uint4 mh = make_uint4(0xFC00FC00u, 0xFC00FC00u, 0xFC00FC00u, 0xFC00FC00u), ml = mh;
+#pragma unroll
+            for (int dy = -1; dy <= 1; ++dy) {
+              const int iy = 2 * oy + dy;
+              if (iy < 0 || iy >= e.OH) continue;
+#pragma unroll
+              for (int dx = -1; dx <= 1; ++dx) {
+                const int ix = 2 * ox + dx;
+                if (ix < 0 || ix >= e.OW) continue;
+                const int px = (2 * ri + dy + 1) * T3_HW + 2 * rj + dx + 1;
+                const uint8_t* src = hbuf + px * 64 + ((gq ^ ((px >> 1) & 3)) << 4);
+                const uint4 h = *reinterpret_cast<const uint4*>(src);
+                if (P1) hmax8(mh, h);
+                else    lexmax8(mh, ml, h, *reinterpret_cast<const uint4*>(src + T3_PLANE));
+              }
+            }
+            if (oy < PH && ox < PW) {
+              const size_t o = ((img * PH + oy) * PW + ox) * PC + c0;
+              *reinterpret_cast<uint4*>(pout + o) = mh;
+              if (!P1) *reinterpret_cast<uint4*>(pout + o + (size_t)e.pool_plane) = ml;
+            }
+          }
+        }
+        mbar_arrive_local(smem_u32(&halo_empty[hb]));
+        if (++hb == HB) { hb = 0; hphase ^= 1u; }
+      }
+    }
   } else {
     const int q = warp & 3, grp = warp >= 7 ? 1 : 0;
     float* stage = reinterpret_cast<float*>(base_ptr + epi_off + (size_t)(grp * 4 + q) * 4096);
@@ -523,14 +569,14 @@
 
 constexpr uint32_t T3_SMEM_MAX = 232448 - 1024;
 
-template <int NT, int KS, int SD, int EPI, bool RES, int CG, bool P1>
+template <int NT, int KS, int SD, int EPI, bool RES, int CG, bool P1, bool POOL = false>
 int launch3k(const CUtensorMap* A, const CUtensorMap& Bm, const T3Args& e, uint32_t smem, dim3 grid, cudaStream_t s) {
   using Cfg = T3Cfg<NT, RES, CG, P1>;
-  auto kern = conv_tc3_kernel<NT, KS, SD, EPI, RES, CG, P1>;
+  auto kern = conv_tc3_kernel<NT, KS, SD, EPI, RES, CG, P1, POOL>;
   cudaError_t err = cudaFuncSetAttribute(kern, cudaFuncAttributeMaxDynamicSharedMemorySize, (int)T3_SMEM_MAX);
   if (err != cudaSuccess) return (int)err;
   cudaLaunchConfig_t cfg = {};
-  cfg.gridDim = grid; cfg.blockDim = dim3(Cfg::THREADS, 1, 1); cfg.dynamicSmemBytes = smem; cfg.stream = s;
+  cfg.gridDim = grid; cfg.blockDim = dim3(Cfg::THREADS + (POOL ? 128 : 0), 1, 1); cfg.dynamicSmemBytes = smem; cfg.stream = s;
   cudaLaunchAttribute at[2];
   int na = dh_pdl_attr(at);
   if (CG == 2) {
@@ -570,6 +616,13 @@
     default: return launch3<32, RES, CG, P1>(A, Bm, e, ks, stride, epi, smem, grid, s);
   }
 }
+int launch3pool(int NT, bool p1, const CUtensorMap* A, const CUtensorMap& Bm, const T3Args& e, uint32_t smem, dim3 grid, cudaStream_t s) {
+  if (NT == 128) return p1 ? launch3k<128, 3, 1, EPI_SPLIT, false, 1, true, true>(A, Bm, e, smem, grid, s)
+                           : launch3k<128, 3, 1, EPI_SPLIT, false, 1, false, true>(A, Bm, e, smem, grid, s);
+  if (NT == 64) return p1 ? launch3k<64, 3, 1, EPI_SPLIT, false, 1, true, true>(A, Bm, e, smem, grid, s)
+                          : launch3k<64, 3, 1, EPI_SPLIT, false, 1, false, true>(A, Bm, e, smem, grid, s);
+  return DH_E_SHAPE;
+}
 template <bool RES>
 int launch3c(int cg, bool p1, int NT, const CUtensorMap* A, const CUtensorMap& Bm, const T3Args& e, int ks, int stride, int epi, uint32_t smem,
              dim3 grid, cudaStream_t s) {
@@ -586,6 +639,8 @@
   if (!base) return false;
   if (a.ps) return a.Cout == 128 && a.res == nullptr && (!a.out_split || a.h16) && a.K == 3;
   if (a.tok) return a.Cout == 32 && a.K == 1 && a.stride == 1 && a.wtok && a.partials && !a.res && !a.bias;
+  if (a.pool) return a.K == 3 && a.stride == 1 && a.in1 && a.C1 == a.C0 && a.Cout % 64 == 0 && (a.out_split || a.h16) &&
+                     a.inH % 2 == 0 && a.inW % 2 == 0;
   return true;
 }
 
@@ -594,7 +649,7 @@
 int dh_launch_conv_tc3(const Conv3Args& a, cudaStream_t s) {
   DH_REQUIRE(dh_conv_tc3_eligible(a), DH_E_SHAPE);
   DH_REQUIRE(dh_aligned16(a.in0) && dh_aligned16(a.in1) && dh_aligned16(a.wt16) && dh_aligned16(a.out) &&
-             dh_aligned16(a.bias) && dh_aligned16(a.res) && dh_aligned16(a.wtok), DH_E_ALIGN);
+             dh_aligned16(a.bias) && dh_aligned16(a.res) && dh_aligned16(a.wtok) && dh_aligned16(a.pool), DH_E_ALIGN);
   const int Cin = a.C0 + a.C1, K = a.K * a.K * Cin;
   int sms_ = 148, dev_ = 0;
   cudaGetDevice(&dev_);
@@ -622,7 +677,8 @@
   static const int env_cg = [] { const char* v = getenv("DAHITRA_TC3_CG"); return v ? atoi(v) : 0; }();
   static const bool env_stream = [] { const char* v = getenv("DAHITRA_TC3_STREAM"); return v && v[0] == '1'; }();
   const int mtiles = dh_cdiv(a.inW / a.stride, T3_TW) * dh_cdiv(a.inH / a.stride, T3_TH) * a.N;
-  int cg = a.tok ? 1 : (a.cg ? a.cg : (env_cg == 2 ? 2 : (env_cg == 1 && (NT == 128 || (a.Cout == 32 && K >= 1152)) ? 2 : 1)));
+  int cg = (a.tok || a.pool) ? 1 : (a.cg ? a.cg : (env_cg == 2 ? 2 : (env_cg == 1 && (NT == 128 || (a.Cout == 32 && K >= 1152)) ? 2 : 1)));
+  DH_REQUIRE(!(a.pool && a.cg == 2), DH_E_VARIANT);
   DH_REQUIRE(!(a.h16 && cg == 2), DH_E_VARIANT);
   if (mtiles < 2) cg = 1;
   rc = filt_map(&Bm, a.wt16, K, a.Cout, a.wt_plane_bytes, NT / cg, a.h16 ? 1 : 2);
@@ -639,6 +695,8 @@
   e.res_plane = a.res_plane ? a.res_plane : (long long)a.N * e.OH * e.OW * a.Cout;
   e.out_plane = a.out_plane ? a.out_plane : (long long)a.N * e.OH * e.OW * a.Cout;
   e.halo_plane_bytes = (uint32_t)(hw * hh * 64);
+  e.pool = a.pool;
+  e.pool_plane = a.pool_plane ? a.pool_plane : 2LL * a.N * (e.OH / 2) * (e.OW / 2) * a.C0;
   const int epi = a.tok ? EPI_TOK : ((a.out_split || a.h16) ? EPI_SPLIT : EPI_F32);
   int dev = 0, sms = 148;
   cudaGetDevice(&dev);
@@ -649,7 +707,7 @@
   const uint32_t w_bytes = (uint32_t)K * (uint32_t)a.Cout * (a.h16 ? 2u : 4u) / (uint32_t)cg;
   const uint32_t halo = a.h16 ? T3_PLANE : T3_HALO;
   const uint32_t fixed = 8 * 4096 + 1024 + (a.tok ? 512 + 2 * 2176 : 0);
-  const bool res_ok = w_bytes + 2 * halo + fixed <= T3_SMEM_MAX && !a.force_stream && !env_stream && e.ntiles >= 2 * nwork;
+  const bool res_ok = w_bytes + 2 * halo + fixed <= T3_SMEM_MAX && !a.force_stream && !env_stream && e.ntiles >= 2 * nwork && !a.pool;
   if (res_ok) {
     int hb = (int)((T3_SMEM_MAX - fixed - w_bytes) / halo);
     e.hb = hb > T3_MAX_HB ? T3_MAX_HB : hb;
@@ -660,5 +718,6 @@
   const uint32_t ring = a.h16 ? (NT == 128 ? T3Cfg<128, false, 1, true>::RING_BYTES : (NT == 64 ? T3Cfg<64, false, 1, true>::RING_BYTES : T3Cfg<32, false, 1, true>::RING_BYTES))
                               : (NT == 128 ? T3Cfg<128, false>::RING_BYTES : (NT == 64 ? T3Cfg<64, false>::RING_BYTES : T3Cfg<32, false>::RING_BYTES));
   const uint32_t smem = T3_MAX_HB * halo + ring + fixed;
+  if (a.pool) return launch3pool(NT, a.h16, A, Bm, e, smem, grid, s);
   return launch3c<false>(cg, a.h16, NT, A, Bm, e, a.K, a.stride, epi, smem, grid, s);
 }
diff --git a/dahitra_b200/csrc/forward.cu b/dahitra_b200/csrc/forward.cu
--- a/dahitra_b200/csrc/forward.cu
+++ b/dahitra_b200/csrc/forward.cu
@@ -56,7 +56,8 @@
   }
   p.c4 = b.take((size_t)B * s4 * 32);
   const size_t n_c3 = (size_t)B * s2 * 32, n_y20 = (size_t)B * s2 * 128, n_c2 = (size_t)B * H * W * 32;
-  const bool early_head = (flags & DH_FLAG_EARLY_HEAD) != 0;
+  const bool early_head = (flags & DH_FLAG_EARLY_HEAD) != 0 ||
+                          ((flags & (DH_FLAG_ACT_SPLIT | DH_FLAG_ACT_H16)) && !(flags & DH_FLAG_POOL_SEPARATE));
   p.c3 = (p.t8c - p.t8a >= n_c3) ? p.t8a : b.take(n_c3);
   p.o2 = (p.p8 - p.t8c >= n_c3) ? p.t8c : b.take(n_c3);
   p.y20 = (!early_head && p.t8a - p.p2 >= n_y20) ? p.p2 : b.take(n_y20);
@@ -223,6 +224,20 @@
   a.wt16 = wt + 3 * plane; a.wt_plane_bytes = (long long)plane * 4;
   a.bias = bias; a.res = res; a.res_split = res_split; a.relu = relu; a.out = out; a.out_split = out_split;
   a.ps = mode == 1; a.tok = mode == 2; a.wtok = w_tok; a.partials = partials;
+  return dh_launch_conv_tc3(a, (cudaStream_t)stream);
+}
+extern "C" int dahitra_conv2d_split_pool(const void* in0, const void* in1, int C, long long in_plane, int N, int inH, int inW,
+                                         int Cout, const float* wt, const float* bias, int relu, void* out, void* pool,
+                                         long long pool_plane, int mode, void* stream) {
+  DH_REQUIRE(wt && in0 && in1 && out && pool, DH_E_NULL);
+  DH_REQUIRE(mode == 0 || mode == 128, DH_E_VARIANT);
+  Conv3Args a{};
+  a.h16 = mode == 128;
+  a.in0 = in0; a.in1 = in1; a.C0 = C; a.C1 = C; a.N = N; a.inH = inH; a.inW = inW; a.in0_plane = in_plane; a.in1_plane = in_plane;
+  a.K = 3; a.stride = 1; a.Cout = Cout;
+  const size_t plane = (size_t)Cout * 9 * 2 * C;
+  a.wt16 = wt + 3 * plane; a.wt_plane_bytes = (long long)plane * 4;
+  a.bias = bias; a.relu = relu; a.out = out; a.out_split = 1; a.pool = pool; a.pool_plane = pool_plane;
   return dh_launch_conv_tc3(a, (cudaStream_t)stream);
 }
 extern "C" int dahitra_classifier(const float* in, int N, int H, int W, int nc, const float* w, const float* bias,
@@ -312,6 +327,7 @@
   const int h2 = H / 2, w2 = W / 2, h4 = H / 4, w4 = W / 4, h8 = H / 8, w8 = W / 8, h16 = H / 16, w16 = W / 16;
   const bool one = (flags & DH_FLAG_ACT_H16) != 0;
   const double eb = one ? 2.0 : 4.0;
+  void* pool_into = nullptr;
   auto conv3 = [&](const char* name, const float* in0, const float* in1, int C0, int C1, long long in_plane, int N, int inH, int inW,
                    int K, int stride, int Cout, int wts, int bslot, const float* res, int res_split, int relu, float* out,
                    int out_split, int ps) -> int {
@@ -322,13 +338,14 @@
     a.wt16 = Wt(wts) + 3 * plane; a.wt_plane_bytes = (long long)plane * 4;
     a.bias = bslot >= 0 ? Wt(bslot) : nullptr; a.res = res; a.res_split = one ? 1 : res_split; a.relu = relu; a.out = out;
     a.out_split = one ? 1 : out_split;
-    a.ps = ps; a.h16 = one;
+    a.ps = ps; a.h16 = one; a.pool = pool_into;
     const int rc = dh_launch_conv_tc3(a, s);
     if (rc != 0) return rc;
     const double OH = (double)inH / stride, OW = (double)inW / stride, Cin = C0 + C1;
     const double cout_alg = ps ? 32.0 : Cout, up = ps ? 2.0 : 1.0;
     const double fl = 2.0 * N * OH * up * OW * up * cout_alg * K * K * Cin;
-    const double by = eb * ((double)N * inH * inW * Cin + (double)N * OH * up * OW * up * cout_alg * (res ? 2 : 1) + (double)K * K * Cin * cout_alg);
+    const double pool_by = pool_into ? (double)N * (OH / 2) * (OW / 2) * Cin : 0.0;
+    const double by = eb * ((double)N * inH * inW * Cin + (double)N * OH * up * OW * up * cout_alg * (res ? 2 : 1) + (double)K * K * Cin * cout_alg + pool_by);
     prof_mark(s, name, fl, by);
     return 0;
   };
@@ -349,10 +366,18 @@
   DH_STEP("stem", 2.0 * stem_fl, 2.0 * stem_by,
           dh_launch_stem_tc(x1, x_batch_stride, B, H, W, Wt(DH_W_STEM_WTC), Wt(DH_W_STEM_B), F2, stem_mode, s, f2_plane, x2));
   float* P2 = ws + p.p2;
+  float* Y20 = ws + p.y20;
   auto maxpool = [&](const float* in, int hh, int ww, int C, float* out) {
     return one ? dh_launch_maxpool_h16(in, N2, hh, ww, C, out, s) : dh_launch_maxpool_split(in, N2, hh, ww, C, out, s);
   };
-  DH_STEP("maxpool_2", 0.0, eb * N2 * 64 * ((double)h2 * w2 + (double)h4 * w4), maxpool(F2, h2, w2, 64, P2));
+  const bool pool_in_conv = !(flags & DH_FLAG_POOL_SEPARATE);
+  if (pool_in_conv) {
+    pool_into = P2;
+    DH_CONV3("conv_layer2_0.0", F2, F2post, 64, 64, f2_plane, B, h2, w2, 3, 1, 128, DH_W_CL20A_WT, DH_W_CL20A_B, nullptr, 0, 1, Y20, 1, 0);
+    pool_into = nullptr;
+  } else {
+    DH_STEP("maxpool_2", 0.0, eb * N2 * 64 * ((double)h2 * w2 + (double)h4 * w4), maxpool(F2, h2, w2, 64, P2));
+  }
   float *T4a = ws + p.t4a, *T4b = ws + p.t4b, *F4 = ws + p.f4;
   DH_CONV3("layer1.0.conv1", P2, nullptr, 64, 0, 0, N2, h4, w4, 3, 1, 64, DH_W_L1_0_C1_WT, DH_W_L1_0_C1_B, nullptr, 0, 1, T4a, 1, 0);
   DH_CONV3("layer1.0.conv2", T4a, nullptr, 64, 0, 0, N2, h4, w4, 3, 1, 64, DH_W_L1_0_C2_WT, DH_W_L1_0_C2_B, P2, 1, 1, T4b, 1, 0);
@@ -455,10 +480,11 @@
     if (rc == 0) rc = level_post(i);
     if (rc != 0) return rc;
   }
-  float *C3 = ws + p.c3, *Y20 = ws + p.y20, *O2 = ws + p.o2, *C2 = ws + p.c2;
+  float *C3 = ws + p.c3, *O2 = ws + p.o2, *C2 = ws + p.c2;
   float* OUT3 = ws + p.lv[2].out;
   DH_CONV3("conv_layer3", OUT3, nullptr, 32, 0, 0, B, h4, w4, 3, 1, 128, DH_W_CL3_PSWT, DH_W_CL3_PSB, nullptr, 0, 1, C3, 0, 1);
-  DH_CONV3("conv_layer2_0.0", F2, F2post, 64, 64, f2_plane, B, h2, w2, 3, 1, 128, DH_W_CL20A_WT, DH_W_CL20A_B, nullptr, 0, 1, Y20, 1, 0);
+  if (!pool_in_conv)
+    DH_CONV3("conv_layer2_0.0", F2, F2post, 64, 64, f2_plane, B, h2, w2, 3, 1, 128, DH_W_CL20A_WT, DH_W_CL20A_B, nullptr, 0, 1, Y20, 1, 0);
   DH_CONV3("conv_layer2_0.3", Y20, nullptr, 128, 0, 0, B, h2, w2, 3, 1, 32, DH_W_CL20B_WT, DH_W_CL20B_B, C3, 0, 0, O2, 1, 0);
   DH_CONV3("conv_layer2", O2, nullptr, 32, 0, 0, B, h2, w2, 3, 1, 128, DH_W_CL2_PSWT, DH_W_CL2_PSB, nullptr, 0, 1, C2, 0, 1);
   DH_STEP("classifier", 2.0 * B * H * W * 9 * 32 * output_nc,
diff --git a/dahitra_b200/csrc/split.cu b/dahitra_b200/csrc/split.cu
--- a/dahitra_b200/csrc/split.cu
+++ b/dahitra_b200/csrc/split.cu
@@ -1,5 +1,4 @@
 #include "tc_common.cuh"
-#include <cuda_fp16.h>
 
 using namespace dhtc;
 
@@ -40,14 +39,6 @@
   }
 }
 
-__device__ __forceinline__ void lexmax2(uint32_t& mh, uint32_t& ml, uint32_t h, uint32_t l) {
-  const __half2 a = *reinterpret_cast<const __half2*>(&h), m = *reinterpret_cast<const __half2*>(&mh);
-  const uint32_t gt = __hgt2_mask(a, m), eq = __heq2_mask(a, m);
-  const __half2 lm = __hmax2(*reinterpret_cast<const __half2*>(&l), *reinterpret_cast<const __half2*>(&ml));
-  ml = (gt & l) | (eq & *reinterpret_cast<const uint32_t*>(&lm)) | (~(gt | eq) & ml);
-  mh = (gt & h) | (~gt & mh);
-}
-
 __global__ void __launch_bounds__(256)
 maxpool_split_kernel(const uint16_t* __restrict__ in, int N, int H, int W, int C, uint16_t* __restrict__ out) {
   const int OH = H / 2, OW = W / 2, C8 = C / 8;
@@ -72,7 +63,7 @@
       if (ix < 0 || ix >= W) continue;
       const size_t o = (((size_t)n * H + iy) * W + ix) * C + c8 * 8;
       const uint4 hi = __ldg(reinterpret_cast<const uint4*>(in + o)), lo = __ldg(reinterpret_cast<const uint4*>(in + plane_in + o));
-      lexmax2(mh.x, ml.x, hi.x, lo.x); lexmax2(mh.y, ml.y, hi.y, lo.y); lexmax2(mh.z, ml.z, hi.z, lo.z); lexmax2(mh.w, ml.w, hi.w, lo.w);
+      lexmax8(mh, ml, hi, lo);
     }
   }
   const size_t o = (((size_t)n * OH + oy) * OW + ox) * C + c8 * 8;
@@ -93,9 +84,7 @@
   const int ox = (int)(p % OW); p /= OW;
   const int oy = (int)(p % OH);
   const int n = (int)(p / OH);
-  __half2 m[4];
-#pragma unroll
-  for (int k = 0; k < 4; ++k) m[k] = __half2half2(__ushort_as_half((unsigned short)0xFC00u));
+  uint4 m = make_uint4(0xFC00FC00u, 0xFC00FC00u, 0xFC00FC00u, 0xFC00FC00u);
 #pragma unroll
   for (int dy = -1; dy <= 1; ++dy) {
     const int iy = 2 * oy + dy;
@@ -104,13 +93,10 @@
     for (int dx = -1; dx <= 1; ++dx) {
       const int ix = 2 * ox + dx;
       if (ix < 0 || ix >= W) continue;
-      const uint4 v = __ldg(reinterpret_cast<const uint4*>(in + (((size_t)n * H + iy) * W + ix) * C + c8 * 8));
-      const __half2* h = reinterpret_cast<const __half2*>(&v);
-#pragma unroll
-      for (int k = 0; k < 4; ++k) m[k] = __hmax2(m[k], h[k]);
+      hmax8(m, __ldg(reinterpret_cast<const uint4*>(in + (((size_t)n * H + iy) * W + ix) * C + c8 * 8)));
     }
   }
-  *reinterpret_cast<uint4*>(out + (((size_t)n * OH + oy) * OW + ox) * C + c8 * 8) = *reinterpret_cast<const uint4*>(m);
+  *reinterpret_cast<uint4*>(out + (((size_t)n * OH + oy) * OW + ox) * C + c8 * 8) = m;
 }
 
 int grid_for(size_t items) {
diff --git a/dahitra_b200/csrc/tc_common.cuh b/dahitra_b200/csrc/tc_common.cuh
--- a/dahitra_b200/csrc/tc_common.cuh
+++ b/dahitra_b200/csrc/tc_common.cuh
@@ -1,6 +1,7 @@
 #pragma once
 #include "common.cuh"
 #include <cuda.h>
+#include <cuda_fp16.h>
 #include <cstdio>
 
 int dh_encode_tiled_f32(CUtensorMap* out, const void* ptr, int rank, const unsigned long long* dims,
@@ -144,6 +145,22 @@
 }
 __device__ __forceinline__ float f16_lo(uint32_t p) { float f; asm("{ .reg .b16 l, h; mov.b32 {l, h}, %1; cvt.f32.f16 %0, l; }" : "=f"(f) : "r"(p)); return f; }
 __device__ __forceinline__ float f16_hi(uint32_t p) { float f; asm("{ .reg .b16 l, h; mov.b32 {l, h}, %1; cvt.f32.f16 %0, h; }" : "=f"(f) : "r"(p)); return f; }
+__device__ __forceinline__ void lexmax2(uint32_t& mh, uint32_t& ml, uint32_t h, uint32_t l) {
+  const __half2 a = *reinterpret_cast<const __half2*>(&h), m = *reinterpret_cast<const __half2*>(&mh);
+  const uint32_t gt = __hgt2_mask(a, m), eq = __heq2_mask(a, m);
+  const __half2 lm = __hmax2(*reinterpret_cast<const __half2*>(&l), *reinterpret_cast<const __half2*>(&ml));
+  ml = (gt & l) | (eq & *reinterpret_cast<const uint32_t*>(&lm)) | (~(gt | eq) & ml);
+  mh = (gt & h) | (~gt & mh);
+}
+__device__ __forceinline__ void lexmax8(uint4& mh, uint4& ml, const uint4& h, const uint4& l) {
+  lexmax2(mh.x, ml.x, h.x, l.x); lexmax2(mh.y, ml.y, h.y, l.y); lexmax2(mh.z, ml.z, h.z, l.z); lexmax2(mh.w, ml.w, h.w, l.w);
+}
+__device__ __forceinline__ void hmax8(uint4& m, const uint4& v) {
+  __half2* mp = reinterpret_cast<__half2*>(&m);
+  const __half2* vp = reinterpret_cast<const __half2*>(&v);
+#pragma unroll
+  for (int k = 0; k < 4; ++k) mp[k] = __hmax2(mp[k], vp[k]);
+}
 __device__ __forceinline__ uint32_t pack_bf16x2(float lo, float hi) {
   uint32_t r;
   asm("cvt.rn.bf16x2.f32 %0, %1, %2;" : "=r"(r) : "f"(hi), "f"(lo));
diff --git a/dahitra_b200/engine.py b/dahitra_b200/engine.py
--- a/dahitra_b200/engine.py
+++ b/dahitra_b200/engine.py
@@ -16,6 +16,7 @@
 DH_FLAG_CONV_TC_V1, DH_FLAG_CONV_TC_2CTA, DH_FLAG_SERIAL, DH_FLAG_TC_X3_BF16, DH_FLAG_TC_BF16 = 64, 128, 256, 512, 1024
 DH_FLAG_TC_MAIN_F16, DH_FLAG_TC_FOLD, DH_FLAG_EARLY_HEAD, DH_FLAG_ACT_SPLIT, DH_FLAG_PDL = 2048, 4096, 8192, 16384, 32768
 DH_FLAG_ACT_H16 = 65536
+DH_FLAG_POOL_SEPARATE = 131072
 MODES = {
     "fp32": 0,
     "fp32_tcdec": DH_FLAG_DEC_TC | DH_FLAG_DEC_TC_X3,
diff --git a/include/dahitra_b200.h b/include/dahitra_b200.h
--- a/include/dahitra_b200.h
+++ b/include/dahitra_b200.h
@@ -38,6 +38,7 @@
 #define DH_FLAG_ACT_SPLIT   16384
 #define DH_FLAG_PDL         32768
 #define DH_FLAG_ACT_H16     65536
+#define DH_FLAG_POOL_SEPARATE 131072
 #define DH_FLAGS_TF32X3     (DH_FLAG_CONV_TC | DH_FLAG_TC_3XTF32 | DH_FLAG_TC_X3_BF16 | DH_FLAG_TC_MAIN_F16 | DH_FLAG_TC_FOLD | DH_FLAG_TC_STRIDE2 | \
                              DH_FLAG_STEM_TC | DH_FLAG_DEC_TC | DH_FLAG_DEC_TC_X3 | DH_FLAG_ACT_SPLIT | DH_FLAG_PDL)
 #define DH_FLAGS_TF32       (DH_FLAG_CONV_TC | DH_FLAG_TC_STRIDE2 | DH_FLAG_STEM_TC | DH_FLAG_DEC_TC | DH_FLAG_DEC_TC_X3)
@@ -148,6 +149,9 @@
                          int N, int inH, int inW, int K, int stride, int Cout, const float* wt, const float* bias,
                          const void* res, int res_split, int relu, void* out, int out_split, int mode,
                          const float* w_tok, float* partials, void* stream);
+int dahitra_conv2d_split_pool(const void* in0, const void* in1, int C, long long in_plane, int N, int inH, int inW,
+                              int Cout, const float* wt, const float* bias, int relu, void* out, void* pool,
+                              long long pool_plane, int mode, void* stream);
 
 int dahitra_classifier(const float* in, int N, int H, int W, int nc, const float* w, const float* bias,
                        float* logits, unsigned char* argmax_u8, void* stream);
```

Measured after the change: 17560 (median of 6 runs). 2.7% higher.
